# arielmission-space/PAOS

Measured on AMD Instinct MI355X. Metric: wavefronts/sec (4096^2 c128, 20-surface chain) + achieved HBM GB/s, higher is better.
Workload: dtype c128 (f64); 1 GPU; SYN20 20-surface chain (SURVEY 8d: 43 2-D FFTs per wavefront as the reference runs it), 4096x4096 fp64, walked 512-wavelength sweep, 32 wavefronts/GPU/step, PSFs stay in HBM; separable pass programs + ptp identities ([24] passes/wavefront, parity 1e-15..2e-14 vs oracle); grid=4096, batch_per_gpu=32, parallelism=wavefront-sharded x1, transport=none (single process), ranks_seen=1, launcher=none

## Files before the change

### include/paos_hip.h

```cpp
#ifndef PAOS_HIP_H
#define PAOS_HIP_H

#ifdef __cplusplus
extern "C" {
#endif

typedef struct paos_ctx paos_ctx;

enum { PAOS_OK = 0, PAOS_EINVAL = 1, PAOS_EHIP = 2, PAOS_EUNSUPPORTED = 3 };
enum { PAOS_F64 = 0, PAOS_F32 = 1 };
enum { PAOS_SHAPE_ELLIPSE = 0, PAOS_SHAPE_RECT = 1 };
enum { PAOS_KERNEL_PASS_ROWS = 0, PAOS_KERNEL_PASS_COLS = 1, PAOS_KERNEL_PASS_ANY = 2 };
enum { PAOS_PW_SIGN = 1, PAOS_PW_QPHASE_CENTRED = 2, PAOS_PW_QPHASE_NATURAL = 3, PAOS_PW_SCALE = 4,
       PAOS_PW_MASK = 5 };
enum { PAOS_PWF_MUL2PI = 1,
       PAOS_PWF_X_ONLY = 2, PAOS_PWF_Y_ONLY = 4 };
enum { PAOS_MAX_PW = 6 };
enum { PAOS_NORM_SLOTS = 64 };
enum { PAOS_WHAT_FIELD = 0, PAOS_WHAT_AMPLITUDE = 1, PAOS_WHAT_PHASE = 2, PAOS_WHAT_INTENSITY = 3 };

enum { PAOS_PHASE_STRIDE = 5 };
enum { PAOS_APERTURE_STRIDE = 8 };
enum { PAOS_ZERNIKE_HEAD = 8 };

typedef struct { int kind, flags, block; } paos_pw_op;
typedef struct {
  int axis;
  int fft1, fft2;
  int n_pre, n_mid, n_post;
  paos_pw_op pre[PAOS_MAX_PW], mid[PAOS_MAX_PW], post[PAOS_MAX_PW];
} paos_pass;

typedef struct {
  const double* live_rows;
  int rows_stale;
  int final_intensity;
  int* power_ticket;
  const double* live_cols;
} paos_program_opts;

int paos_ctx_create(int device, int n, int batch, int precision, paos_ctx** out);
int paos_ctx_destroy(paos_ctx* ctx);
const char* paos_last_error(const paos_ctx* ctx);
int paos_sync(paos_ctx* ctx);
const char* paos_build_info(void);
const char* paos_source_hash(void);
void* paos_stream(paos_ctx* ctx);

int paos_profile_begin(paos_ctx* ctx, int kernel_kind, int max_launches);
int paos_profile_end(paos_ctx* ctx, int* launches, double* total_ms);
int paos_profile_end_split(paos_ctx* ctx, int* launches, double* total_ms, int* pruned_launches, double* pruned_ms);
int paos_profile_end_launches(paos_ctx* ctx, int capacity, double* ms_out, int* tag_out, int* count);
int paos_profile_planned_bytes(paos_ctx* ctx, int capacity, double* bytes_out, int* count);
int paos_profile_line_transforms(paos_ctx* ctx, int capacity, double* lines_out, int* count);

int paos_fill(paos_ctx* ctx, double re, double im);
int paos_start(paos_ctx* ctx, double re, double im, int shape, const double* aperture, const double* stop);
int paos_start_rows(paos_ctx* ctx, double re, double im, int shape, const double* aperture, const double* stop,
                    const double* write_rows);
int paos_zero_outside_rows(paos_ctx* ctx, const double* live_rows);
int paos_start_box(paos_ctx* ctx, double re, double im, int shape, const double* aperture, const double* stop,
                   const double* write_rows, const double* write_cols);
int paos_start_zernike_box(paos_ctx* ctx, double re, double im, int shape, const double* aperture, const double* stop,
                           const double* write_rows, const double* write_cols, int nmax, int kdim, const double* table,
                           const double* params, int param_stride, int* power_ticket);
int paos_zero_outside_box(paos_ctx* ctx, const double* live_rows, const double* live_cols);
int paos_import(paos_ctx* ctx, int item, const void* host_c128);
int paos_export(paos_ctx* ctx, int item, int what, void* host_out);

int paos_psf_keep(paos_ctx* ctx);
int paos_psf_keep_power(paos_ctx* ctx, int* ticket);
int paos_psf_fetch(paos_ctx* ctx, int item, double* host_out);
int paos_host_alloc(unsigned long long bytes, void** out);
int paos_host_free(void* p);
int paos_export_pinned(paos_ctx* ctx, int item, int what, void* pinned_out);

int paos_aperture(paos_ctx* ctx, int shape, const double* params);
int paos_aperture_render(paos_ctx* ctx, int shape, const double* params1, double* host_mask);
int paos_make_stop(paos_ctx* ctx, const double* enable);
int paos_stop_scale_last_power(paos_ctx* ctx, const double* enable);
int paos_stop_defer_last_power(paos_ctx* ctx, const double* enable);
int paos_norm2(paos_ctx* ctx, double* host_out);
int paos_norm2_enqueue(paos_ctx* ctx, int* ticket);
int paos_norm2_enqueue_rows(paos_ctx* ctx, const double* live_rows, int* ticket);
int paos_norm2_enqueue_rows_like(paos_ctx* ctx, const double* live_rows, const double* same_as, int* ticket);
int paos_norm2_enqueue_box(paos_ctx* ctx, const double* live_rows, const double* live_cols, const double* same_as, int* ticket);
int paos_norm2_fetch(paos_ctx* ctx, int ticket, double* host_out);
int paos_norm2_release(paos_ctx* ctx, int ticket);
int paos_psf_metrics(paos_ctx* ctx, int nr, const double* radii_px, double cx_px, double cy_px,
                     double* host_out);
int paos_phase(paos_ctx* ctx, const double* params, int mul2pi);
int paos_phase_map(paos_ctx* ctx, int item, const double* host_wfe, double wl);
int paos_phase_map_items(paos_ctx* ctx, const double* host_wfe, unsigned long long key, int n_items, const double* items,
                         const double* wl);
int paos_psd_screen(paos_ctx* ctx, const double* host_noise, const double* host_rough, const double* params,
                    unsigned long long key, double* host_out);
int paos_ptp(paos_ctx* ctx, const double* params);
int paos_stw(paos_ctx* ctx, const double* params, int inverse);
int paos_wts(paos_ctx* ctx, const double* params, int inverse);
int paos_focus_begin(paos_ctx* ctx);
int paos_focus_plane(paos_ctx* ctx, const double* params);
int paos_focus_end(paos_ctx* ctx);
enum { PAOS_OTF_MTF = 0, PAOS_OTF_COMPLEX = 1 };
int paos_otf_compute(paos_ctx* ctx);
int paos_otf_fetch(paos_ctx* ctx, int item, int what, void* host_out);
int paos_otf_cuts(paos_ctx* ctx, double* host_out);
int paos_blur_table(int n, double d, double sigma, double pixel, double* t);
enum { PAOS_BLUR_ITEM = 6 };
int paos_blur_apply(paos_ctx* ctx, const double* per_item);
enum { PAOS_EE_GIVEN = 0, PAOS_EE_CENTROID = 1, PAOS_EE_PEAK = 2 };
enum { PAOS_EE_ITEM = 4 };
enum { PAOS_EE_SUMMARY = 9 };
int paos_ee_compute(paos_ctx* ctx, int bins, int square, int centre_mode, const double* per_item);
int paos_ee_fetch(paos_ctx* ctx, double* summary, double* curves);
int paos_zoom_weights(int n, int s, double frac, double* w, int* carry);
enum { PAOS_ZOOM_PSF = 0, PAOS_ZOOM_FIELD = 1 };
int paos_zoom_compute(paos_ctx* ctx, int m, int s, const double* centres, int want_field);
int paos_zoom_tiles(int n, int batch, int m, int* pt_y, int* pt_x);
int paos_zoom_fetch(paos_ctx* ctx, int item, int what, void* host_out);
int paos_run_passes(paos_ctx* ctx, const paos_pass* passes, int n_passes, const double* blocks,
                    int n_blocks);
int paos_copy_yardstick(paos_ctx* ctx, int reps, double* ms_per_launch, double* bytes_per_launch);
int paos_record_set_stats(paos_ctx* ctx, unsigned long long* found, unsigned long long* rendered);
int paos_central_half_stats(paos_ctx* ctx, unsigned long long* central, unsigned long long* plain);
int paos_narrow_window_stats(paos_ctx* ctx, unsigned long long* narrow, unsigned long long* other);
int paos_record_block_stats(paos_ctx* ctx, unsigned long long* out);
int paos_frugal_built(int precision, int n, const int* record);
int paos_pass_builds(paos_ctx* ctx, int* records, int capacity, int* count);
int paos_deferred_stop_stats(paos_ctx* ctx, unsigned long long* rode, unsigned long long* settled);
int paos_ctx_set_pruning(paos_ctx* ctx, int on);
int paos_run_passes_live(paos_ctx* ctx, const paos_pass* passes, int n_passes, const double* blocks,
                         int n_blocks, const double* live_rows);
int paos_run_program(paos_ctx* ctx, const paos_pass* passes, int n_passes, const double* blocks, int n_blocks,
                     const paos_program_opts* opts);
int paos_zernike(paos_ctx* ctx, int nmax, int kdim, const double* table, const double* params,
                 int param_stride, double* host_wfe);
int paos_zernike_like(paos_ctx* ctx, int nmax, int kdim, const double* table, const double* params,
                      int param_stride, const double* same_as, double* host_wfe);


int paos_pupil_aperture(paos_ctx* ctx, int shape, const double* params);
int paos_pupil_upload(paos_ctx* ctx, int item, const double* host_weights);
int paos_zernike_gram(paos_ctx* ctx, int nmax, int kdim, const double* table, const double* params,
                      int param_stride, int K, const double* poly, int use_pupil, double* host_out);
int paos_zernike_pupil(paos_ctx* ctx, int nmax, int kdim, const double* table, const double* params,
                       int param_stride, double* host_wfe);

enum { PAOS_WF_UNIFORM = 0, PAOS_WF_INTENSITY = 1 };
enum { PAOS_WF_SUMMARY = 10 };
int paos_wavefront_fit(paos_ctx* ctx, int nmax, int kdim, const double* table, const double* params, int param_stride,
                       int K, const double* poly, int weight_mode, int use_pupil, const double* min_intensity);
int paos_wavefront_fetch(paos_ctx* ctx, double* summary, double* sums);

enum { PAOS_DETECTOR_GEOM = 6 };
enum { PAOS_DETECTOR_ITEM = 3 };
enum { PAOS_DETECTOR_SCRATCH_MIB = 512 };
int paos_detector_begin(paos_ctx* ctx, const double* geom);
int paos_detector_add(paos_ctx* ctx, const double* per_item);
int paos_detector_images(paos_ctx* ctx, const double* per_item, double* host_out);
int paos_detector_fetch(paos_ctx* ctx, double* host_out);
enum { PAOS_DETECTOR_PLACED_ITEM = 5 };
int paos_detector_add_placed(paos_ctx* ctx, const double* per_item);
int paos_detector_images_placed(paos_ctx* ctx, const double* per_item, double* host_out);

enum { PAOS_SERIES_ITEM = 4 };
enum { PAOS_SERIES_MAX_FRAMES = 65536, PAOS_SERIES_MAX_BOXES = 16 };
int paos_series_compute(paos_ctx* ctx, const double* geom, const double* per_item, const double* offsets, int frames,
                        int per_item_offsets, const int* boxes, int nboxes, const double* response, double* host_frames);
int paos_series_fetch(paos_ctx* ctx, double* flux);

#ifdef __cplusplus
}
#endif
#endif
```

### paos_amd/_lib.py

```python
import ctypes
import os
import threading
import weakref

import numpy as np

_HERE = os.path.dirname(os.path.abspath(__file__))
LIB_PATH = os.environ.get("PAOS_LIB") or os.path.join(_HERE, "libpaoship.so")

PAOS_F64, PAOS_F32 = 0, 1
SHAPE_ELLIPSE, SHAPE_RECT = 0, 1
WHAT_FIELD, WHAT_AMPLITUDE, WHAT_PHASE, WHAT_INTENSITY = 0, 1, 2, 3
KERNEL_PASS_ROWS, KERNEL_PASS_COLS, KERNEL_PASS_ANY = 0, 1, 2
PW_SIGN, PW_QPHASE_CENTRED, PW_QPHASE_NATURAL, PW_SCALE, PW_MASK = 1, 2, 3, 4, 5
PWF_MUL2PI = 1
PWF_X_ONLY, PWF_Y_ONLY = 2, 4
MAX_PW = 6
OTF_MTF, OTF_COMPLEX = 0, 1
EE_GIVEN, EE_CENTROID, EE_PEAK = 0, 1, 2
EE_ITEM, EE_SUMMARY, EE_MAX_BINS = 4, 9, 1024
SERIES_ITEM, SERIES_MAX_FRAMES, SERIES_MAX_BOXES = 4, 65536, 16
WF_UNIFORM, WF_INTENSITY = 0, 1
WF_SUMMARY, WF_MAX_TERMS = 10, 63
ZOOM_PSF, ZOOM_FIELD = 0, 1
ZOOM_MAX_TABLES = 256
NORM_SLOTS = 64


class PwOp(ctypes.Structure):
    _fields_ = [("kind", ctypes.c_int), ("flags", ctypes.c_int), ("block", ctypes.c_int)]


class ProgramOpts(ctypes.Structure):
    _fields_ = [("live_rows", ctypes.POINTER(ctypes.c_double)), ("rows_stale", ctypes.c_int),
                ("final_intensity", ctypes.c_int), ("power_ticket", ctypes.POINTER(ctypes.c_int)),
                ("live_cols", ctypes.POINTER(ctypes.c_double))]


class Pass(ctypes.Structure):
    _fields_ = [("axis", ctypes.c_int), ("fft1", ctypes.c_int), ("fft2", ctypes.c_int),
                ("n_pre", ctypes.c_int), ("n_mid", ctypes.c_int), ("n_post", ctypes.c_int),
                ("pre", PwOp * MAX_PW), ("mid", PwOp * MAX_PW), ("post", PwOp * MAX_PW)]

PHASE_STRIDE = 5
APERTURE_STRIDE = 8
ZERNIKE_HEAD = 8

_c_ctx = ctypes.c_void_p
_dbl_p = ctypes.POINTER(ctypes.c_double)
SYMBOLS = {
    "paos_ctx_create": (ctypes.c_int, [ctypes.c_int, ctypes.c_int, ctypes.c_int, ctypes.c_int, ctypes.POINTER(_c_ctx)]),
    "paos_ctx_destroy": (ctypes.c_int, [_c_ctx]),
    "paos_last_error": (ctypes.c_char_p, [_c_ctx]),
    "paos_sync": (ctypes.c_int, [_c_ctx]),
    "paos_build_info": (ctypes.c_char_p, []),
    "paos_stream": (ctypes.c_void_p, [_c_ctx]),
    "paos_profile_begin": (ctypes.c_int, [_c_ctx, ctypes.c_int, ctypes.c_int]),
    "paos_profile_end": (ctypes.c_int, [_c_ctx, ctypes.POINTER(ctypes.c_int), _dbl_p]),
    "paos_profile_end_split": (ctypes.c_int, [_c_ctx, ctypes.POINTER(ctypes.c_int), _dbl_p, ctypes.POINTER(ctypes.c_int), _dbl_p]),
    "paos_source_hash": (ctypes.c_char_p, []),
    "paos_profile_planned_bytes": (ctypes.c_int, [_c_ctx, ctypes.c_int, _dbl_p, ctypes.POINTER(ctypes.c_int)]),
    "paos_profile_line_transforms": (ctypes.c_int, [_c_ctx, ctypes.c_int, _dbl_p, ctypes.POINTER(ctypes.c_int)]),
    "paos_profile_end_launches": (ctypes.c_int, [_c_ctx, ctypes.c_int, _dbl_p, ctypes.POINTER(ctypes.c_int),
                                                 ctypes.POINTER(ctypes.c_int)]),
    "paos_fill": (ctypes.c_int, [_c_ctx, ctypes.c_double, ctypes.c_double]),
    "paos_import": (ctypes.c_int, [_c_ctx, ctypes.c_int, ctypes.c_void_p]),
    "paos_export": (ctypes.c_int, [_c_ctx, ctypes.c_int, ctypes.c_int, ctypes.c_void_p]),
    "paos_aperture": (ctypes.c_int, [_c_ctx, ctypes.c_int, _dbl_p]),
    "paos_aperture_render": (ctypes.c_int, [_c_ctx, ctypes.c_int, _dbl_p, _dbl_p]),
    "paos_make_stop": (ctypes.c_int, [_c_ctx, _dbl_p]),
    "paos_stop_scale_last_power": (ctypes.c_int, [_c_ctx, _dbl_p]),
    "paos_stop_defer_last_power": (ctypes.c_int, [_c_ctx, _dbl_p]),
    "paos_norm2": (ctypes.c_int, [_c_ctx, _dbl_p]),
    "paos_norm2_enqueue": (ctypes.c_int, [_c_ctx, ctypes.POINTER(ctypes.c_int)]),
    "paos_norm2_fetch": (ctypes.c_int, [_c_ctx, ctypes.c_int, _dbl_p]),
    "paos_norm2_release": (ctypes.c_int, [_c_ctx, ctypes.c_int]),
    "paos_psf_metrics": (ctypes.c_int, [_c_ctx, ctypes.c_int, _dbl_p, ctypes.c_double, ctypes.c_double, _dbl_p]),
    "paos_phase": (ctypes.c_int, [_c_ctx, _dbl_p, ctypes.c_int]),
    "paos_phase_map": (ctypes.c_int, [_c_ctx, ctypes.c_int, _dbl_p, ctypes.c_double]),
    "paos_ptp": (ctypes.c_int, [_c_ctx, _dbl_p]),
    "paos_stw": (ctypes.c_int, [_c_ctx, _dbl_p, ctypes.c_int]),
    "paos_wts": (ctypes.c_int, [_c_ctx, _dbl_p, ctypes.c_int]),
    "paos_focus_begin": (ctypes.c_int, [_c_ctx]),
    "paos_focus_plane": (ctypes.c_int, [_c_ctx, _dbl_p]),
    "paos_focus_end": (ctypes.c_int, [_c_ctx]),
    "paos_otf_compute": (ctypes.c_int, [_c_ctx]),
    "paos_otf_fetch": (ctypes.c_int, [_c_ctx, ctypes.c_int, ctypes.c_int, ctypes.c_void_p]),
    "paos_otf_cuts": (ctypes.c_int, [_c_ctx, _dbl_p]),
    "paos_blur_table": (ctypes.c_int, [ctypes.c_int, ctypes.c_double, ctypes.c_double, ctypes.c_double, _dbl_p]),
    "paos_blur_apply": (ctypes.c_int, [_c_ctx, _dbl_p]),
    "paos_ee_compute": (ctypes.c_int, [_c_ctx, ctypes.c_int, ctypes.c_int, ctypes.c_int, _dbl_p]),
    "paos_ee_fetch": (ctypes.c_int, [_c_ctx, _dbl_p, _dbl_p]),
    "paos_series_compute": (ctypes.c_int, [_c_ctx, _dbl_p, _dbl_p, _dbl_p, ctypes.c_int, ctypes.c_int, ctypes.POINTER(ctypes.c_int),
                                           ctypes.c_int, _dbl_p, _dbl_p]),
    "paos_series_fetch": (ctypes.c_int, [_c_ctx, _dbl_p]),
    "paos_wavefront_fit": (ctypes.c_int, [_c_ctx, ctypes.c_int, ctypes.c_int, _dbl_p, _dbl_p, ctypes.c_int, ctypes.c_int, _dbl_p,
                                          ctypes.c_int, ctypes.c_int, _dbl_p]),
    "paos_wavefront_fetch": (ctypes.c_int, [_c_ctx, _dbl_p, _dbl_p]),
    "paos_zoom_weights": (ctypes.c_int, [ctypes.c_int, ctypes.c_int, ctypes.c_double, _dbl_p, ctypes.POINTER(ctypes.c_int)]),
    "paos_zoom_compute": (ctypes.c_int, [_c_ctx, ctypes.c_int, ctypes.c_int, _dbl_p, ctypes.c_int]),
    "paos_zoom_fetch": (ctypes.c_int, [_c_ctx, ctypes.c_int, ctypes.c_int, ctypes.c_void_p]),
    "paos_zoom_tiles": (ctypes.c_int, [ctypes.c_int, ctypes.c_int, ctypes.c_int, ctypes.POINTER(ctypes.c_int),
                                       ctypes.POINTER(ctypes.c_int)]),
    "paos_run_passes": (ctypes.c_int, [_c_ctx, ctypes.POINTER(Pass), ctypes.c_int, _dbl_p, ctypes.c_int]),
    "paos_copy_yardstick": (ctypes.c_int, [_c_ctx, ctypes.c_int, _dbl_p, _dbl_p]),
    "paos_record_set_stats": (ctypes.c_int, [_c_ctx, ctypes.POINTER(ctypes.c_ulonglong), ctypes.POINTER(ctypes.c_ulonglong)]),
    "paos_central_half_stats": (ctypes.c_int, [_c_ctx, ctypes.POINTER(ctypes.c_ulonglong), ctypes.POINTER(ctypes.c_ulonglong)]),
    "paos_narrow_window_stats": (ctypes.c_int, [_c_ctx, ctypes.POINTER(ctypes.c_ulonglong), ctypes.POINTER(ctypes.c_ulonglong)]),
    "paos_record_block_stats": (ctypes.c_int, [_c_ctx, ctypes.POINTER(ctypes.c_ulonglong)]),
    "paos_frugal_built": (ctypes.c_int, [ctypes.c_int, ctypes.c_int, ctypes.POINTER(ctypes.c_int)]),
    "paos_pass_builds": (ctypes.c_int, [_c_ctx, ctypes.POINTER(ctypes.c_int), ctypes.c_int, ctypes.POINTER(ctypes.c_int)]),
    "paos_deferred_stop_stats": (ctypes.c_int, [_c_ctx, ctypes.POINTER(ctypes.c_ulonglong), ctypes.POINTER(ctypes.c_ulonglong)]),
    "paos_ctx_set_pruning": (ctypes.c_int, [_c_ctx, ctypes.c_int]),
    "paos_run_passes_live": (ctypes.c_int, [_c_ctx, ctypes.POINTER(Pass), ctypes.c_int, _dbl_p, ctypes.c_int, _dbl_p]),
    "paos_zernike": (ctypes.c_int, [_c_ctx, ctypes.c_int, ctypes.c_int, _dbl_p, _dbl_p, ctypes.c_int, _dbl_p]),
    "paos_psf_keep": (ctypes.c_int, [_c_ctx]),
    "paos_psf_keep_power": (ctypes.c_int, [_c_ctx, ctypes.POINTER(ctypes.c_int)]),
    "paos_psf_fetch": (ctypes.c_int, [_c_ctx, ctypes.c_int, _dbl_p]),
    "paos_host_alloc": (ctypes.c_int, [ctypes.c_ulonglong, ctypes.POINTER(ctypes.c_void_p)]),
    "paos_host_free": (ctypes.c_int, [ctypes.c_void_p]),
    "paos_export_pinned": (ctypes.c_int, [_c_ctx, ctypes.c_int, ctypes.c_int, ctypes.c_void_p]),
    "paos_start": (ctypes.c_int, [_c_ctx, ctypes.c_double, ctypes.c_double, ctypes.c_int, _dbl_p, _dbl_p]),
    "paos_pupil_aperture": (ctypes.c_int, [_c_ctx, ctypes.c_int, _dbl_p]),
    "paos_pupil_upload": (ctypes.c_int, [_c_ctx, ctypes.c_int, _dbl_p]),
    "paos_zernike_like": (ctypes.c_int, [_c_ctx, ctypes.c_int, ctypes.c_int, _dbl_p, _dbl_p, ctypes.c_int, _dbl_p, _dbl_p]),
    "paos_zernike_gram": (ctypes.c_int, [_c_ctx, ctypes.c_int, ctypes.c_int, _dbl_p, _dbl_p, ctypes.c_int,
                                         ctypes.c_int, _dbl_p, ctypes.c_int, _dbl_p]),
    "paos_zernike_pupil": (ctypes.c_int, [_c_ctx, ctypes.c_int, ctypes.c_int, _dbl_p, _dbl_p, ctypes.c_int, _dbl_p]),
    "paos_start_rows": (ctypes.c_int, [_c_ctx, ctypes.c_double, ctypes.c_double, ctypes.c_int, _dbl_p, _dbl_p, _dbl_p]),
    "paos_zero_outside_rows": (ctypes.c_int, [_c_ctx, _dbl_p]),
    "paos_phase_map_items": (ctypes.c_int, [_c_ctx, _dbl_p, ctypes.c_ulonglong, ctypes.c_int, _dbl_p, _dbl_p]),
    "paos_psd_screen": (ctypes.c_int, [_c_ctx, _dbl_p, _dbl_p, _dbl_p, ctypes.c_ulonglong, _dbl_p]),
    "paos_start_box": (ctypes.c_int, [_c_ctx, ctypes.c_double, ctypes.c_double, ctypes.c_int, _dbl_p, _dbl_p, _dbl_p, _dbl_p]),
    "paos_start_zernike_box": (ctypes.c_int, [_c_ctx, ctypes.c_double, ctypes.c_double, ctypes.c_int, _dbl_p, _dbl_p, _dbl_p, _dbl_p,
                                              ctypes.c_int, ctypes.c_int, _dbl_p, _dbl_p, ctypes.c_int, ctypes.POINTER(ctypes.c_int)]),
    "paos_zero_outside_box": (ctypes.c_int, [_c_ctx, _dbl_p, _dbl_p]),
    "paos_norm2_enqueue_box": (ctypes.c_int, [_c_ctx, _dbl_p, _dbl_p, _dbl_p, ctypes.POINTER(ctypes.c_int)]),
    "paos_norm2_enqueue_rows": (ctypes.c_int, [_c_ctx, _dbl_p, ctypes.POINTER(ctypes.c_int)]),
    "paos_norm2_enqueue_rows_like": (ctypes.c_int, [_c_ctx, _dbl_p, _dbl_p, ctypes.POINTER(ctypes.c_int)]),
    "paos_run_program": (ctypes.c_int, [_c_ctx, ctypes.POINTER(Pass), ctypes.c_int, _dbl_p, ctypes.c_int,
                                        ctypes.POINTER(ProgramOpts)]),
    "paos_detector_begin": (ctypes.c_int, [_c_ctx, _dbl_p]),
    "paos_detector_add": (ctypes.c_int, [_c_ctx, _dbl_p]),
    "paos_detector_images": (ctypes.c_int, [_c_ctx, _dbl_p, _dbl_p]),
    "paos_detector_fetch": (ctypes.c_int, [_c_ctx, _dbl_p]),
    "paos_detector_add_placed": (ctypes.c_int, [_c_ctx, _dbl_p]),
    "paos_detector_images_placed": (ctypes.c_int, [_c_ctx, _dbl_p, _dbl_p]),
}

_lib = None


class PaosHipError(RuntimeError):
    pass


def load():
    global _lib
    if _lib is not None:
        return _lib
    if not os.path.exists(LIB_PATH):
        raise PaosHipError(
            f"{LIB_PATH} not found: build it with `make` or "
            "`python -c 'import __graft_entry__ as g; g.build()'` (there is no CPU fallback)"
        )
    lib = ctypes.CDLL(LIB_PATH)
    if os.environ.get("PAOS_LIB"):
        import sys

        print(f"paos_amd: using the library variant {LIB_PATH} (PAOS_LIB)", file=sys.stderr)
    for name, (res, args) in SYMBOLS.items():
        fn = getattr(lib, name)
        fn.restype = res
        fn.argtypes = args
    _lib = lib
    return lib


def _dptr(arr):
    return arr.ctypes.data_as(_dbl_p)


def as_blocks(blocks, batch, stride):
    arr = np.ascontiguousarray(blocks, dtype=np.float64)
    if arr.shape != (batch, stride):
        raise ValueError(f"expected parameter blocks of shape {(batch, stride)}, got {arr.shape}")
    return arr


BUILD_FIELDS = ("axis", "kpre", "kmid", "nfft", "store", "tab", "fuse", "one_line", "central")


def frugal_built(precision, n, record):
    if len(record) != len(BUILD_FIELDS):
        raise ValueError("a build record has nine fields")
    rec = (ctypes.c_int * 9)(*[int(v) for v in record])
    code = {"fp64": PAOS_F64, "fp32": PAOS_F32}.get(precision, -1)
    rc = load().paos_frugal_built(code, int(n), rec)
    if rc < 0:
        raise ValueError(f"no family of pass-kernel builds for {precision} at n = {n}")
    return bool(rc)


def zoom_check(size, oversample, n):
    if isinstance(size, bool) or not isinstance(size, (int, np.integer)) or size < 16 or size > 1024 or size % 16:
        raise ValueError(f"a zoomed window's size must be an integer multiple of 16 in 16 .. 1024, got {size!r}")
    if isinstance(oversample, bool) or not isinstance(oversample, (int, np.integer)) or not 1 <= oversample <= 64:
        raise ValueError(f"a zoomed window's oversampling must be an integer in 1 .. 64, got {oversample!r}")
    if size > oversample * n:
        raise ValueError(f"a zoomed window of {size} samples at oversampling {oversample} is wider than the {n}-pixel grid")


def zoom_tiles(n, batch, size):
    pty, ptx = ctypes.c_int(0), ctypes.c_int(0)
    if load().paos_zoom_tiles(int(n), int(batch), int(size), ctypes.byref(pty), ctypes.byref(ptx)) != 0:
        raise ValueError(f"paos_zoom_tiles refused n={n!r}, batch={batch!r}, size={size!r}")
    return pty.value, ptx.value


def blur_table(n, d, sigma, pixel=0.0):
    if isinstance(n, bool) or not isinstance(n, (int, np.integer)) or n < 2:
        raise ValueError(f"paos_blur_table refused n={n!r}")
    out = np.empty(int(n) // 2 + 1, dtype=np.float64)
    if load().paos_blur_table(int(n), float(d), float(sigma), float(pixel), _dptr(out)) != 0:
        raise ValueError(f"paos_blur_table refused n={n!r}, d={d!r}, sigma={sigma!r}, pixel={pixel!r}")
    return out


def zoom_centres(centres, batch, n):
    try:
        ctr = np.ascontiguousarray(centres, dtype=np.float64)
    except (TypeError, ValueError):
        raise ValueError("zoomed-window centres must be a (batch, 2) array of pixel positions (x, y)") from None
    if ctr.shape != (batch, 2):
        raise ValueError(f"zoomed-window centres must have shape ({batch}, 2), got {ctr.shape}")
    if not np.all(np.isfinite(ctr)) or np.any(ctr < 0.0) or np.any(ctr >= n):
        raise ValueError(f"zoomed-window centres must be finite and lie in [0, {n})")
    if np.unique(ctr - np.floor(ctr)).size > ZOOM_MAX_TABLES:
        raise ValueError(f"the centres of one call may have at most {ZOOM_MAX_TABLES} distinct fractional parts")
    return ctr


PINNED_MIN_BYTES = 4 << 20
PINNED_MAX_BYTES = 32 << 20
PINNED_LIVE_BYTES = int(os.environ.get("PAOS_PINNED_BYTES", 8 << 30))
PINNED_POOL_BYTES = 2 << 30
_pin_lock = threading.Lock()
_pin_free = {}
_pin_live = 0
_pin_pooled = 0


def _pin_release(address, nbytes):
    global _pin_live, _pin_pooled
    with _pin_lock:
        _pin_live -= nbytes
        if _pin_pooled + nbytes <= PINNED_POOL_BYTES:
            _pin_free.setdefault(nbytes, []).append(address)
            _pin_pooled += nbytes
            return
    try:
# ... 645 lines not shown
```

### paos_amd/csrc/context.hip

```cpp
#include "host.h"

#include <cmath>
#include <complex>
#include <cstdio>
#include <cstring>
#include <mutex>
#include <set>
#include <utility>

namespace {

thread_local std::string g_err;

}

int fail(paos_ctx* c, int code, const std::string& msg) {
  if (c) c->err = msg;
  g_err = msg;
  return code;
}

namespace {

bool dump_arena() {
// ... 128 lines not shown
    }
  }
  HIPCHK(c, hipStreamSynchronize(c->stream));
  return PAOS_OK;
}

bool timed_launch_begin(paos_ctx* c, int kind) {
  const bool timed = (c->prof_kind == kind || c->prof_kind == PAOS_KERNEL_PASS_ANY) && (c->prof_used + 2 <= c->prof_events.size());
  return timed && hipEventRecord(c->prof_events[c->prof_used], c->stream) == hipSuccess;
}
hipError_t timed_launch_end(paos_ctx* c, int tag) {
  const hipError_t e = hipEventRecord(c->prof_events[c->prof_used + 1], c->stream);
  if (e != hipSuccess) return e;
  c->prof_tags.resize(c->prof_used / 2, 0);
  c->prof_tags.push_back(tag);
  c->prof_bytes.resize(c->prof_tags.size() - 1, 0.0);
  c->prof_bytes.push_back(c->prof_next_bytes);
  c->prof_lines.resize(c->prof_tags.size() - 1, 0.0);
  c->prof_lines.push_back(c->prof_next_lines);
  c->prof_used += 2;
  return hipSuccess;
}

int next_norm_slot(paos_ctx* c) {
  for (int k = 0; k < kNormSlots; ++k) {
    const int slot = (c->norm_slot + k) % kNormSlots;
    if (!c->norm_busy[slot]) { c->norm_slot = slot; return slot; }
  }
  return c->norm_slot;
}

int opt_in_lds(paos_ctx* c, const void* kern, size_t lds) {
  static std::mutex mu;
  static std::set<std::pair<int, const void*>> configured;
  std::lock_guard<std::mutex> lock(mu);
  const std::pair<int, const void*> key(c->device, kern);
  if (configured.count(key)) return PAOS_OK;
  HIPCHK(c, hipFuncSetAttribute(kern, hipFuncAttributeMaxDynamicSharedMemorySize, (int)lds));
  configured.insert(key);
  return PAOS_OK;
}

int check_mask_overflow(paos_ctx* c) {
  if (!c->mask_overflow) return PAOS_OK;
  int n = 0;
  HIPCHK(c, hipMemcpy(&n, c->mask_overflow, sizeof(int), hipMemcpyDeviceToHost));
  if (n != 0) {
    (void)hipMemset(c->mask_overflow, 0, sizeof(int));
    for (auto& ms : c->mask_sets) ms.key.clear();
    return fail(c, PAOS_EUNSUPPORTED, "aperture line records overflowed (partial run longer than kMaskW): results are invalid");
  }
  return PAOS_OK;
}

int check_rows(paos_ctx* c, const double* rows) {
  for (int i = 0; i < c->batch; ++i)
    if (!(rows[2 * i] >= 0.0) || !(rows[2 * i + 1] <= (double)c->n) || !(rows[2 * i] <= rows[2 * i + 1]))
      return fail(c, PAOS_EINVAL, "row range must satisfy 0 <= lo <= hi <= n");
  return PAOS_OK;
}

std::vector<double> rounded_cols(const paos_ctx* c, const double* cols) {
  std::vector<double> out((size_t)2 * c->batch);
  for (int i = 0; i < c->batch; ++i) {
    int l = (int)cols[2 * i], h = (int)cols[2 * i + 1];
    l = l < 0 ? 0 : (l / c->br) * c->br;
    h = ((h + c->br - 1) / c->br) * c->br;
    if (h > c->n) h = c->n;
    out[2 * i] = l; out[2 * i + 1] = h;
  }
  return out;
}

namespace {

template <typename T>
std::vector<std::complex<T>> twiddles(int n) {
  std::vector<std::complex<T>> tw(n);
  const long double two_pi = 6.283185307179586476925286766559005768L;
  for (int m = 0; m < n; ++m) {
    const long double a = two_pi * (long double)m / (long double)n;
    tw[m] = std::complex<T>((T)cosl(a), (T)-sinl(a));
  }
  return tw;
}


int profile_end(paos_ctx* c, int* launches, double* total_ms, int* pruned_launches, double* pruned_ms) {
  if (c) (void)hipSetDevice(c->device);
  if (!c || !launches || !total_ms) return fail(c, PAOS_EINVAL, "null argument");
  HIPCHK(c, hipStreamSynchronize(c->stream));
  double sum = 0.0, psum = 0.0;
  int pcount = 0;
  for (size_t i = 0; i + 1 < c->prof_used; i += 2) {
    float ms = 0.f;
    HIPCHK(c, hipEventElapsedTime(&ms, c->prof_events[i], c->prof_events[i + 1]));
    sum += ms;
    if (i / 2 < c->prof_tags.size() && c->prof_tags[i / 2]) { psum += ms; ++pcount; }
  }
  *launches = (int)(c->prof_used / 2);
  *total_ms = sum;
  if (pruned_launches) *pruned_launches = pcount;
  if (pruned_ms) *pruned_ms = psum;
  c->prof_kind = -1;
  c->prof_used = 0;
  return PAOS_OK;
}

}

extern "C" {

const char* paos_last_error(const paos_ctx* ctx) { return ctx ? ctx->err.c_str() : g_err.c_str(); }

const char* paos_build_info(void) {
  static const std::string info = std::string("libpaoship gfx950 layout=") + std::to_string(BR) + "(c64 at N>=2048: " + std::to_string(PAOS_F32_BR) + ")x(" +
                                  std::to_string(Lay<double>::BC) + "|" + std::to_string(Lay<float>::BC) +
                                  ") pad_blocks=" + std::to_string(PAOS_PAD_BLOCKS);
  return info.c_str();
}

void* paos_stream(paos_ctx* ctx) { return ctx ? (void*)ctx->stream : nullptr; }

int paos_ctx_create(int device, int n, int batch, int precision, paos_ctx** out) {
  if (!out) return fail(nullptr, PAOS_EINVAL, "out is null");
  *out = nullptr;
  if (n < 64 || n > 4096 || (n & (n - 1))) return fail(nullptr, PAOS_EUNSUPPORTED, "grid size must be a power of two in 64..4096");
  if (batch < 1) return fail(nullptr, PAOS_EINVAL, "batch must be >= 1");
  if (precision != PAOS_F64 && precision != PAOS_F32) return fail(nullptr, PAOS_EINVAL, "precision must be PAOS_F64 or PAOS_F32");
  int ndev = 0;
  if (hipGetDeviceCount(&ndev) != hipSuccess || ndev == 0)
    return fail(nullptr, PAOS_EHIP, "no HIP device available: libpaoship has no CPU fallback");
  if (device < 0 || device >= ndev) return fail(nullptr, PAOS_EINVAL, "device index out of range");
  paos_ctx* c = new paos_ctx();
  c->device = device; c->n = n; c->batch = batch; c->precision = precision;
  const int bc = precision == PAOS_F64 ? Lay<double>::BC : Lay<float>::BC;
  c->br = (precision == PAOS_F32 && n >= 2048) ? PAOS_F32_BR : PAOS_BR;
  c->pitch = (unsigned)n * c->br + (unsigned)PAOS_PAD_BLOCKS * c->br * bc;
  c->item_stride = c->pitch * (unsigned)(n / c->br);
  const size_t eb = elem_bytes(c);
  auto bail = [&](hipError_t e, const char* what) {
    std::string msg = std::string(what) + ": " + hipGetErrorString(e);
    paos_ctx_destroy(c);
    return fail(nullptr, PAOS_EHIP, msg);
  };
  hipError_t e;
  if ((e = hipSetDevice(device)) != hipSuccess) return bail(e, "hipSetDevice");
  if ((e = hipStreamCreateWithFlags(&c->stream, hipStreamNonBlocking)) != hipSuccess) return bail(e, "hipStreamCreate");
  if (const char* pad = getenv("PAOS_LDS_PAD")) c->lds_pad = (size_t)std::max(0, std::atoi(pad));
  if (env_is("PAOS_CENTRAL_HALF", '0')) c->central_half = false;
  if (env_is("PAOS_CENTRAL_HALF", '1')) c->central_half = true;
  if (env_is("PAOS_NARROW_WINDOWS", '0')) c->narrow_windows = false;
  if (env_is("PAOS_NARROW_WINDOWS", '1')) c->narrow_windows = true;
  if ((e = hipMalloc(&c->dyn_scale, (size_t)batch * sizeof(double))) != hipSuccess) return bail(e, "hipMalloc(dyn_scale)");
  {
    std::vector<double> ones((size_t)batch, 1.0);
    if ((e = hipMemcpy(c->dyn_scale, ones.data(), ones.size() * sizeof(double), hipMemcpyHostToDevice)) != hipSuccess) return bail(e, "hipMemcpy(dyn_scale)");
  }
  if ((e = hipMalloc(&c->field, (size_t)c->item_stride * batch * eb)) != hipSuccess) return bail(e, "hipMalloc(field)");
  if ((e = hipMemsetAsync(c->field, 0, (size_t)c->item_stride * batch * eb, c->stream)) != hipSuccess) return bail(e, "hipMemset(field)");
  if ((e = hipMalloc(&c->tw, (size_t)n * eb)) != hipSuccess) return bail(e, "hipMalloc(tw)");
  if ((e = hipMalloc(&c->staging, (size_t)n * n * 16)) != hipSuccess) return bail(e, "hipMalloc(staging)");
  c->nparts = 1024;
  if ((e = hipMalloc(&c->partial, (size_t)batch * c->nparts * sizeof(double))) != hipSuccess) return bail(e, "hipMalloc(partial)");
  if ((e = hipMalloc(&c->norm2, (size_t)batch * sizeof(double))) != hipSuccess) return bail(e, "hipMalloc(norm2)");
  if ((e = hipHostMalloc(&c->norm2_host, (size_t)kNormSlots * batch * sizeof(double))) != hipSuccess) return bail(e, "hipHostMalloc(norm2)");
  c->arena.lay.cap = (size_t)1 << 18;
  if (c->arena.lay.cap < (size_t)batch * 2048) c->arena.lay.cap = (size_t)batch * 2048;
  if (const char* cap = getenv("PAOS_ARENA_DOUBLES")) c->arena.lay.cap = arena_rounded((size_t)std::max(1LL, std::atoll(cap)));
  if ((e = hipHostMalloc(&c->arena.host, kArenaSlabs * c->arena.lay.cap * sizeof(double))) != hipSuccess) return bail(e, "hipHostMalloc(arena)");
  if ((e = hipMalloc(&c->arena.dev, kArenaSlabs * c->arena.lay.cap * sizeof(double))) != hipSuccess) return bail(e, "hipMalloc(arena)");
  for (int k = 0; k < kArenaSlabs; ++k)
    if ((e = hipEventCreateWithFlags(&c->arena.fence[k], hipEventDisableTiming)) != hipSuccess) return bail(e, "hipEventCreate(arena fence)");
  c->arena.used[0] = true;
  e = dispatch_layout(c, [&](auto t, auto) {
    auto tw = twiddles<decltype(t)>(n);
    return hipMemcpy(c->tw, tw.data(), (size_t)n * eb, hipMemcpyHostToDevice);
  });
  if (e != hipSuccess) return bail(e, "hipMemcpy(tw)");
  *out = c;
  return PAOS_OK;
}

int paos_profile_begin(paos_ctx* c, int kernel_kind, int max_launches) {
  if (c) (void)hipSetDevice(c->device);
  if (!c || max_launches < 0) return fail(c, PAOS_EINVAL, "bad profile request");
  HIPCHK(c, hipStreamSynchronize(c->stream));
  while (c->prof_events.size() < (size_t)2 * max_launches) {
    hipEvent_t e;
    HIPCHK(c, hipEventCreate(&e));
    c->prof_events.push_back(e);
  }
  c->prof_kind = kernel_kind;
  c->prof_used = 0;
  c->prof_tags.clear();
  c->prof_bytes.clear();
  c->prof_lines.clear();
  return PAOS_OK;
}

int paos_profile_end_launches(paos_ctx* c, int capacity, double* ms_out, int* tag_out, int* count) {
  if (c) (void)hipSetDevice(c->device);
  if (!c || !ms_out || !tag_out || !count || capacity < 0) return fail(c, PAOS_EINVAL, "null argument");
  HIPCHK(c, hipStreamSynchronize(c->stream));
  const int n = (int)(c->prof_used / 2);
  if (n > capacity) return fail(c, PAOS_EINVAL, "more launches were timed than the caller's arrays hold");
  for (int i = 0; i < n; ++i) {
    float ms = 0.f;
    HIPCHK(c, hipEventElapsedTime(&ms, c->prof_events[2 * i], c->prof_events[2 * i + 1]));
    ms_out[i] = ms;
    tag_out[i] = (size_t)i < c->prof_tags.size() ? c->prof_tags[i] : 0;
  }
  *count = n;
  c->prof_kind = -1;
  c->prof_used = 0;
  return PAOS_OK;
}

int paos_profile_planned_bytes(paos_ctx* c, int capacity, double* bytes_out, int* count) {
  if (!c || !bytes_out || !count || capacity < 0) return fail(c, PAOS_EINVAL, "null argument");
  const int n = (int)(c->prof_used / 2);
  if (n > capacity) return fail(c, PAOS_EINVAL, "more launches were timed than the caller's array holds");
  for (int i = 0; i < n; ++i) bytes_out[i] = (size_t)i < c->prof_bytes.size() ? c->prof_bytes[i] : 0.0;
  *count = n;
  return PAOS_OK;
}

int paos_profile_line_transforms(paos_ctx* c, int capacity, double* lines_out, int* count) {
  if (!c || !lines_out || !count || capacity < 0) return fail(c, PAOS_EINVAL, "bad profile request");
  const int n = (int)(c->prof_used / 2);
  if (n > capacity) return fail(c, PAOS_EINVAL, "profile buffer too small");
  for (int i = 0; i < n; ++i) lines_out[i] = (size_t)i < c->prof_lines.size() ? c->prof_lines[i] : 0.0;
  *count = n;
  return PAOS_OK;
}

int paos_profile_end(paos_ctx* c, int* launches, double* total_ms) {
  return profile_end(c, launches, total_ms, nullptr, nullptr);
}

int paos_profile_end_split(paos_ctx* c, int* launches, double* total_ms, int* pruned_launches, double* pruned_ms) {
  if (!pruned_launches || !pruned_ms) return fail(c, PAOS_EINVAL, "null argument");
  return profile_end(c, launches, total_ms, pruned_launches, pruned_ms);
}

int paos_ctx_destroy(paos_ctx* c) {
  if (!c) return PAOS_OK;
  (void)hipSetDevice(c->device);
  if (c->stream) (void)hipStreamSynchronize(c->stream);
  for (hipEvent_t e : c->prof_events) (void)hipEventDestroy(e);
  if (c->field) (void)hipFree(c->field);
  if (c->tw) (void)hipFree(c->tw);
  if (c->staging) (void)hipFree(c->staging);
  if (c->tables) (void)hipFree(c->tables);
  if (c->mask) (void)hipFree(c->mask);
  if (c->metric_partial) (void)hipFree(c->metric_partial);
  if (c->metric_out) (void)hipFree(c->metric_out);
  if (c->metric_host) (void)hipHostFree(c->metric_host);
  for (auto& ms : c->mask_sets) {
    if (ms.lines) (void)hipFree(ms.lines);
    if (ms.vals) (void)hipFree(ms.vals);
  }
  if (c->mask_overflow) (void)hipFree(c->mask_overflow);
  if (c->block_stats) (void)hipFree(c->block_stats);
  if (c->partial) (void)hipFree(c->partial);
  if (c->norm2) (void)hipFree(c->norm2);
  if (c->norm2_host) (void)hipHostFree(c->norm2_host);
  if (c->psf) (void)hipFree(c->psf);
  if (c->focus_spec) (void)hipFree(c->focus_spec);
  if (c->otf_spec) (void)hipFree(c->otf_spec);
  if (c->otf_cuts) (void)hipFree(c->otf_cuts);
  if (c->zoom_t) (void)hipFree(c->zoom_t);
  if (c->zoom_psf) (void)hipFree(c->zoom_psf);
  if (c->zoom_field) (void)hipFree(c->zoom_field);
  if (c->zoom_tabs) (void)hipFree(c->zoom_tabs);
  if (c->map_dev) (void)hipFree(c->map_dev);
  if (c->psd_scratch) (void)hipFree(c->psd_scratch);
  if (c->start_norm2) (void)hipFree(c->start_norm2);
  if (c->start_partial) (void)hipFree(c->start_partial);
  if (c->psd_bad) (void)hipFree(c->psd_bad);
  if (c->pow_partial) (void)hipFree(c->pow_partial);
  if (c->dyn_scale) (void)hipFree(c->dyn_scale);
  if (c->ptab) (void)hipFree(c->ptab);
  if (c->psf_partial) (void)hipFree(c->psf_partial);
  if (c->det_img) (void)hipFree(c->det_img);
  if (c->det_rows) (void)hipFree(c->det_rows);
  if (c->det_out) (void)hipFree(c->det_out);
  if (c->ee_buf) (void)hipFree(c->ee_buf);
  if (c->wf_buf) (void)hipFree(c->wf_buf);
  if (c->series_par) (void)hipFree(c->series_par);
  if (c->series_flux) (void)hipFree(c->series_flux);
  if (c->series_frames) (void)hipFree(c->series_frames);
  if (c->series_host) (void)hipHostFree(c->series_host);
  if (c->series_ev) (void)hipEventDestroy(c->series_ev);
  for (int i = 0; i < 2; ++i) {
    if (c->bounce[i]) (void)hipHostFree(c->bounce[i]);
    if (c->bounce_ev[i]) (void)hipEventDestroy(c->bounce_ev[i]);
  }
  if (c->arena.host) (void)hipHostFree(c->arena.host);
  if (c->arena.dev) (void)hipFree(c->arena.dev);
  for (int k = 0; k < kArenaSlabs; ++k)
    if (c->arena.fence[k]) (void)hipEventDestroy(c->arena.fence[k]);
  if (c->stream) (void)hipStreamDestroy(c->stream);
  delete c;
  return PAOS_OK;
}

int paos_sync(paos_ctx* c) {
  if (c) (void)hipSetDevice(c->device);
  if (!c) return fail(c, PAOS_EINVAL, "null context");
  HIPCHK(c, hipStreamSynchronize(c->stream));
  return check_mask_overflow(c);
}

int paos_host_alloc(unsigned long long bytes, void** out) {
  if (!out || bytes == 0) return fail(nullptr, PAOS_EINVAL, "null argument");
  *out = nullptr;
  const hipError_t e = hipHostMalloc(out, (size_t)bytes);
  if (e != hipSuccess) {
    *out = nullptr;
    return fail(nullptr, PAOS_EHIP, std::string("hipHostMalloc: ") + hipGetErrorString(e));
  }
  return PAOS_OK;
}

int paos_host_free(void* p) {
  if (!p) return PAOS_OK;
  const hipError_t e = hipHostFree(p);
  if (e != hipSuccess) return fail(nullptr, PAOS_EHIP, std::string("hipHostFree: ") + hipGetErrorString(e));
  return PAOS_OK;
}

int paos_norm2_fetch(paos_ctx* c, int ticket, double* host_out) {
  if (c) (void)hipSetDevice(c->device);
  if (!c || !host_out || ticket < 0 || ticket >= kNormSlots) return fail(c, PAOS_EINVAL, "bad ticket");
  if (!c->norm_busy[ticket]) return fail(c, PAOS_EINVAL, "ticket is not outstanding (already fetched, or never issued)");
  HIPCHK(c, hipStreamSynchronize(c->stream));
  c->norm_busy[ticket] = false;
  std::memcpy(host_out, c->norm2_host + (size_t)ticket * c->batch, (size_t)c->batch * sizeof(double));
  return check_mask_overflow(c);
}

int paos_norm2_release(paos_ctx* c, int ticket) {
  if (!c || ticket < 0 || ticket >= kNormSlots) return fail(c, PAOS_EINVAL, "bad ticket");
  c->norm_busy[ticket] = false;
  return PAOS_OK;
}

int paos_record_set_stats(paos_ctx* c, unsigned long long* found, unsigned long long* rendered) {
  if (!c || !found || !rendered) return fail(c, PAOS_EINVAL, "bad record-set request");
  *found = c->mask_hits;
  *rendered = c->mask_rendered;
  return PAOS_OK;
}

int paos_central_half_stats(paos_ctx* c, unsigned long long* central, unsigned long long* plain) {
  if (!c || !central || !plain) return fail(c, PAOS_EINVAL, "bad central-half request");
  *central = c->central_launches;
  *plain = c->plain_launches;
  return PAOS_OK;
}

int paos_narrow_window_stats(paos_ctx* c, unsigned long long* narrow, unsigned long long* other) {
  if (!c || !narrow || !other) return fail(c, PAOS_EINVAL, "bad narrow-window request");
  *narrow = c->narrow_launches;
  *other = c->other_launches;
  return PAOS_OK;
}

int paos_record_block_stats(paos_ctx* c, unsigned long long* out) {
  if (!c || !out) return fail(c, PAOS_EINVAL, "bad record-block request");
  out[0] = out[1] = out[2] = 0ull;
  if (!c->block_stats) return PAOS_OK;
  HIPCHK(c, hipStreamSynchronize(c->stream));
  HIPCHK(c, hipMemcpy(out, c->block_stats, 3 * sizeof(unsigned long long), hipMemcpyDeviceToHost));
  return PAOS_OK;
}

int paos_deferred_stop_stats(paos_ctx* c, unsigned long long* rode, unsigned long long* settled) {
  if (!c || !rode || !settled) return fail(c, PAOS_EINVAL, "bad deferred-stop request");
  *rode = c->deferred_rode;
  *settled = c->deferred_settled;
  return PAOS_OK;
}

int paos_ctx_set_pruning(paos_ctx* c, int on) {
  if (!c) return fail(c, PAOS_EINVAL, "null context");
  c->prune = on != 0;
  return PAOS_OK;
}

}
```

### paos_amd/csrc/focus_otf.hip

```cpp
#include "host.h"

#include <algorithm>
#include <cmath>

#include "blur_pass.h"
#include "focus_pass.h"
#include "otf_pass.h"

namespace {

template <typename T_, int N_, int AXIS_>
struct Tile {
  using T = T_;
  using C = FftCfg<T, N_>;
  static constexpr int N = N_, AXIS = AXIS_;
  static constexpr int LINES = AXIS == 0 ? C::ROW_LINES : C::COL_LINES;
  static constexpr int TILES = AXIS == 0 ? C::ROW_TILES : C::COL_TILES;
  static constexpr bool SPLIT = AXIS == 0 ? C::ROW_SPLIT : C::COL_SPLIT;
  static constexpr int PER_WG = LINES * TILES;
};
template <typename Kernel, typename Args>
int tile_pass(paos_ctx* c, int axis, int lines, double bytes, Kernel kernel, const Args& a) {
  return dispatch_layout(c, [&](auto t, auto) {
    return dispatch_n(c, [&](auto n) {
// ... 23 lines not shown
    using L = decltype(tile);
    using C = typename L::C;
    return focus_pass_kernel<typename L::T, L::N, C::E, L::LINES, L::TILES, L::AXIS, C::BR, C::BC, L::SPLIT, C::MINW>;
  }, a);
}

}

extern "C" {

int paos_focus_begin(paos_ctx* c) {
  SETTLE_SCALE(c);
  if (c) (void)hipSetDevice(c->device);
  if (!c) return fail(c, PAOS_EINVAL, "null context");
  if (c->focus_open) return fail(c, PAOS_EINVAL, "paos_focus_begin: a focus stack is already open (paos_focus_end first)");
  if (!c->focus_spec) HIPCHK(c, hipMalloc(&c->focus_spec, (size_t)c->item_stride * c->batch * elem_bytes(c)));
  int rc = focus_pass(c, 0, FOCUS_FORWARD, c->field, c->focus_spec, nullptr);
  if (rc) return rc;
  rc = focus_pass(c, 1, FOCUS_FORWARD, c->focus_spec, c->focus_spec, nullptr);
  if (rc) return rc;
  c->focus_open = true;
  return PAOS_OK;
}

int paos_focus_plane(paos_ctx* c, const double* params) {
  if (c) (void)hipSetDevice(c->device);
  if (!c || !params) return fail(c, PAOS_EINVAL, "null argument");
  if (!c->focus_open) return fail(c, PAOS_EINVAL, "paos_focus_plane: no focus stack is open (paos_focus_begin first)");
  for (int i = 0; i < c->batch; ++i)
    for (int k = 0; k < FP_STRIDE; ++k)
      if (!std::isfinite(params[(size_t)i * FP_STRIDE + k]))
        return fail(c, PAOS_EINVAL, "paos_focus_plane: non-finite parameter of item " + std::to_string(i));
  DROP_SCALE(c);
  const double* dparams = nullptr;
  int rc = arena_push(c, params, (size_t)c->batch * FP_STRIDE, &dparams);
  if (rc) return rc;
  rc = focus_pass(c, 1, FOCUS_TRANSFER, c->focus_spec, c->field, dparams);
  if (rc) return rc;
  return focus_pass(c, 0, FOCUS_INVERSE, c->field, c->field, nullptr);
}

int paos_focus_end(paos_ctx* c) {
  if (c) (void)hipSetDevice(c->device);
  if (!c) return fail(c, PAOS_EINVAL, "null context");
  if (!c->focus_open) return fail(c, PAOS_EINVAL, "paos_focus_end: no focus stack is open");
  HIPCHK(c, hipStreamSynchronize(c->stream));
  HIPCHK(c, hipFree(c->focus_spec));
  c->focus_spec = nullptr;
  c->focus_open = false;
  return PAOS_OK;
}

}

namespace {

constexpr int kThreads = 256;

int otf_pass(paos_ctx* c, int axis) {
  OtfArgs a{};
  a.psf = c->psf; a.spec = c->otf_spec; a.tw = c->tw;
  a.pitch = c->pitch; a.item_stride = c->item_stride;
  const double n = c->n, eb = (double)elem_bytes(c);
  const double bytes = axis == 0 ? c->batch * n * (n * 8.0 + c->n / 2 * eb) : c->batch * (double)(c->n / 2 + 1) * 2.0 * n * eb;
  return tile_pass(c, axis, packed_lines(c, axis), bytes, [](auto tile) {
    using L = decltype(tile);
    using C = typename L::C;
    if constexpr (L::AXIS == 0) return otf_row_kernel<typename L::T, L::N, C::E, L::LINES, L::TILES, C::BR, C::BC, L::SPLIT, C::MINW>;
    else return otf_col_kernel<typename L::T, L::N, C::E, L::LINES, L::TILES, C::BR, C::BC, L::SPLIT, C::MINW>;
  }, a);
}

int otf_ready(paos_ctx* c, const char* who) {
  if (!c->otf_spec || !c->otf_computed) return fail(c, PAOS_EINVAL, std::string(who) + ": no transfer functions computed (paos_otf_compute)");
  if (!c->otf_valid)
    return fail(c, PAOS_EINVAL, std::string(who) + ": the PSFs were stored anew since paos_otf_compute: the transfer functions are stale (compute again)");
  return PAOS_OK;
}

int blur_pass(paos_ctx* c, int axis, const BlurArgs& a) {
  const double n = c->n, eb = (double)elem_bytes(c);
  const double bytes = axis == 0 ? c->batch * n * n * 16.0 : c->batch * n * ((c->n / 2 + 1) * 2.0 * eb + n * 8.0);
  return tile_pass(c, axis, packed_lines(c, axis), bytes, [](auto tile) {
    using L = decltype(tile);
    using C = typename L::C;
    if constexpr (L::AXIS == 0) return blur_row_kernel<typename L::T, L::N, C::E, L::LINES, L::TILES, C::BR, C::BC, L::SPLIT, C::MINW>;
    else return blur_col_kernel<typename L::T, L::N, C::E, L::LINES, L::TILES, C::BR, C::BC, L::SPLIT, C::MINW>;
  }, a);
}

const char* blur_table_refusal(int n, double d, double sigma, double pixel) {
  if (n < 2 || (n & 1) || n > (1 << 20)) return "n must be even, 2 .. 2^20";
  if (!std::isfinite(d) || !(d > 0.0)) return "the pitch must be finite and positive";
  if (!std::isfinite(sigma) || sigma < 0.0) return "sigma must be finite and >= 0";
  if (!std::isfinite(pixel) || pixel < 0.0) return "the pixel width must be finite and >= 0";
  return nullptr;
}

}

extern "C" {

int paos_blur_table(int n, double d, double sigma, double pixel, double* t) {
  if (const char* why = blur_table_refusal(n, d, sigma, pixel)) return fail(nullptr, PAOS_EINVAL, std::string("paos_blur_table: ") + why);
  if (!t) return fail(nullptr, PAOS_EINVAL, "paos_blur_table: null argument");
  const long double pi = 3.141592653589793238462643383279502884L;
  const long double s = (long double)sigma, p = (long double)pixel, nd = (long double)n * (long double)d;
  for (int m = 0; m <= n / 2; ++m) {
    const long double f = (long double)m / nd;
    const long double x = pi * (p * f);
    const long double sinc = x == 0.0L ? 1.0L : sinl(x) / x;
    t[m] = (double)(expl(-2.0L * pi * pi * (s * s) * (f * f)) * sinc);
  }
  return PAOS_OK;
}

int paos_blur_apply(paos_ctx* c, const double* per_item) {
  if (c) (void)hipSetDevice(c->device);
  if (!c || !per_item) return fail(c, PAOS_EINVAL, "paos_blur_apply: null argument");
  int rc = otf_ready(c, "paos_blur_apply");
  if (rc) return rc;
  for (int i = 0; i < c->batch; ++i) {
    const double* q = per_item + (size_t)i * PAOS_BLUR_ITEM;
    for (int ax = 0; ax < 2; ++ax)
      if (const char* why = blur_table_refusal(c->n, q[ax], q[2 + ax], q[4 + ax]))
        return fail(c, PAOS_EINVAL, "paos_blur_apply: item " + std::to_string(i) + (ax ? ", y: " : ", x: ") + why);
  }
  const int len = c->n / 2 + 1;
  std::vector<double>& tabs = c->blur_tabs;
  if (tabs.empty()) {
    tabs.resize((size_t)c->batch * 2 * len);
    c->blur_key.assign((size_t)c->batch * 2 * 3, -1.0);
  }
  for (int i = 0; i < c->batch; ++i) {
    const double* q = per_item + (size_t)i * PAOS_BLUR_ITEM;
    for (int ax = 0; ax < 2; ++ax) {
      double* key = c->blur_key.data() + ((size_t)i * 2 + ax) * 3;
      if (key[0] == q[ax] && key[1] == q[2 + ax] && key[2] == q[4 + ax]) continue;
      key[0] = -1.0;
      rc = paos_blur_table(c->n, q[ax], q[2 + ax], q[4 + ax], tabs.data() + ((size_t)i * 2 + ax) * len);
      if (rc) return rc;
      key[0] = q[ax]; key[1] = q[2 + ax]; key[2] = q[4 + ax];
    }
  }
  rc = arena_reserve(c, tabs.size());
  if (rc) return rc;
  const double* dtabs = nullptr;
  rc = arena_push(c, tabs.data(), tabs.size(), &dtabs);
  if (rc) return rc;
  BlurArgs a{};
  a.psf = c->psf; a.spec = c->otf_spec; a.tw = c->tw; a.tabs = dtabs;
  a.scale = 1.0 / ((double)c->n * (double)c->n);
  a.pitch = c->pitch; a.item_stride = c->item_stride;
  c->psf_zero_axis = -1;
  c->ee_valid = false;
  for (int axis = 1; axis >= 0; --axis) {
    rc = blur_pass(c, axis, a);
    if (rc) {
      c->otf_valid = false;
      return rc;
    }
  }
  return PAOS_OK;
}

int paos_otf_compute(paos_ctx* c) {
  if (c) (void)hipSetDevice(c->device);
  if (!c) return fail(c, PAOS_EINVAL, "null context");
  if (!c->psf) return fail(c, PAOS_EINVAL, "paos_otf_compute: no PSF kept (paos_psf_keep)");
  if (!c->otf_spec) HIPCHK(c, hipMalloc(&c->otf_spec, (size_t)c->item_stride * c->batch * elem_bytes(c)));
  c->otf_valid = false;
  int rc = otf_pass(c, 0);
  if (rc) return rc;
  rc = otf_pass(c, 1);
  if (rc) return rc;
  c->otf_computed = c->otf_valid = true;
  return PAOS_OK;
}

int paos_otf_fetch(paos_ctx* c, int item, int what, void* host_out) {
  if (c) (void)hipSetDevice(c->device);
  if (!c || !host_out || item < 0 || item >= c->batch || (what != PAOS_OTF_MTF && what != PAOS_OTF_COMPLEX))
    return fail(c, PAOS_EINVAL, "paos_otf_fetch: bad item/what or null buffer");
  int rc = otf_ready(c, "paos_otf_fetch");
  if (rc) return rc;
  const int cplx = what == PAOS_OTF_COMPLEX;
  const size_t n2 = (size_t)c->n * c->n;
  const dim3 grid((unsigned)std::min<size_t>((n2 + kThreads - 1) / kThreads, 2048)), block(kThreads);
  dispatch_layout(c, [&](auto t, auto br) {
    using T = decltype(t);
    hipLaunchKernelGGL((otf_fetch_kernel<T, decltype(br)::value, Lay<T>::BC>), grid, block, 0, c->stream,
                       (const cx<T>*)c->otf_spec + (size_t)item * c->item_stride, c->staging, c->n, c->pitch, cplx);
  });
  HIPCHK(c, hipGetLastError());
  return copy_to_host(c, host_out, c->staging, n2 * (cplx ? 16 : 8));
}

int paos_otf_cuts(paos_ctx* c, double* host_out) {
  if (c) (void)hipSetDevice(c->device);
  if (!c || !host_out) return fail(c, PAOS_EINVAL, "paos_otf_cuts: null argument");
  int rc = otf_ready(c, "paos_otf_cuts");
  if (rc) return rc;
  const int len = c->n / 2 + 1;
  const size_t bytes = (size_t)c->batch * 2 * len * sizeof(double);
  if (!c->otf_cuts) HIPCHK(c, hipMalloc(&c->otf_cuts, bytes));
  const dim3 grid((2 * len + kThreads - 1) / kThreads, c->batch), block(kThreads);
  dispatch_layout(c, [&](auto t, auto br) {
    using T = decltype(t);
    hipLaunchKernelGGL((otf_cuts_kernel<T, decltype(br)::value, Lay<T>::BC>), grid, block, 0, c->stream, (const cx<T>*)c->otf_spec,
                       c->otf_cuts, c->n, c->pitch, c->item_stride);
  });
  HIPCHK(c, hipGetLastError());
  return copy_to_host(c, host_out, c->otf_cuts, bytes);
}

}
```

### paos_amd/csrc/frugal_launch.h

```cpp
#pragma once
#include "host.h"
#include "pass_records.h"


inline int frugal_not_built(paos_ctx* c, const FrugalBuild& b) {
  if (b.tab && b.fuse) {
    if (b.kpre != 1 || b.kmid != 1) return fail(c, PAOS_EINVAL, "no fused build of this pass shape");
    if (b.nfft < 2) return fail(c, PAOS_EINVAL, "a fused chain starts with a two-transform pass");
    if (b.fuse > 4) return fail(c, PAOS_EINVAL, "a launch runs at most three passes");
  }
  if (b.tab && !(b.kpre <= 1 && b.kmid <= 1 && b.kpre + b.kmid > 0)) return fail(c, PAOS_EINVAL, "no table build of this pass shape");
  if (b.store == 1 && !b.tab) return fail(c, PAOS_EUNSUPPORTED, "no PSF-storing build of this pass shape");
  if (b.store == 2 && !b.tab) return fail(c, PAOS_EUNSUPPORTED, "no power-summing build of this pass shape");
  return fail(c, PAOS_EINVAL, "no build of this pass shape");
}

template <typename T, int N, int AXIS, int KPRE, int KMID, int STORE = 0, int LONG = 0, int ONE = 0, int LINES_ = 0, int TILES_ = 0>
struct FrugalGeometry {
  using C = FftCfg<T, N>;
  static constexpr bool kLatencyBound = PAOS_LONG_ONE_LINE != 0 && (LONG != 0 || ONE != 0) && STORE == 0 && sizeof(T) == 8;
  static constexpr bool kOneLine = kLatencyBound && N == 4096;
  static constexpr int OCC = (kLatencyBound && N == 2048) ? 1 : 0;
  static constexpr int LINES = LINES_ != 0 ? LINES_ : (kOneLine ? 1 : (AXIS == 0 ? C::FR_ROW_LINES : C::COL_LINES));
  static constexpr int TILES = TILES_ != 0 ? TILES_ : (AXIS == 0 ? C::ROW_TILES : C::COL_TILES);
  static constexpr bool SPLIT = sizeof(T) == 8 || LINES > 2;
  static constexpr int GROUPS = N / LINES / TILES, THREADS = TILES * LINES * N / C::E;
  static constexpr size_t LDS = frugal_lds_bytes<T, N, LINES, TILES, SPLIT, KPRE, KMID, C::E, STORE, OCC>();
  static constexpr unsigned ALIGN = (LINES == 1 && AXIS == 0) ? 32 : 16;
};

namespace {

template <typename T, int N, int AXIS, int KPRE, int KMID, int NFFT, int STORE, int TAB, int LONG, int ONE, int CH>
int frugal_launch(paos_ctx* c, const FrugalArgs& args, bool narrow) {
  using C = FftCfg<T, N>;
  using G = FrugalGeometry<T, N, AXIS, KPRE, KMID, STORE, LONG, ONE>;
  FrugalArgs a = args;
  unsigned groups = G::GROUPS;
  a.wg0 = 0;
  static_assert(G::GROUPS % G::ALIGN == 0, "TileMap renumbers tiles inside aligned groups of workgroups");
  if (a.live_hi > a.live_lo) {
    const unsigned per = G::LINES * G::TILES;
    a.wg0 = (a.live_lo / per) / G::ALIGN * G::ALIGN;
    unsigned end = ((a.live_hi + per - 1) / per + G::ALIGN - 1) / G::ALIGN * G::ALIGN;
    if (end > groups) end = groups;
    groups = end - a.wg0;
  }
  const dim3 grid(groups, c->batch), block(G::THREADS);
  constexpr size_t kMaxPad = 8192;
  const size_t lds = G::LDS + (c->lds_pad < kMaxPad ? c->lds_pad : kMaxPad);
  auto kern = frugal_pass_kernel<T, N, C::E, G::LINES, G::TILES, AXIS, C::BR, C::BC, G::SPLIT, KPRE, KMID, NFFT, STORE, TAB, LONG, G::OCC, CH>;
  if constexpr (CH == 1) {
    if (narrow) kern = frugal_pass_kernel<T, N, C::E, G::LINES, G::TILES, AXIS, C::BR, C::BC, G::SPLIT, KPRE, KMID, NFFT, STORE, TAB, LONG, G::OCC, 2>;
  } else {
    narrow = false;
  }
  ++(CH != 0 ? c->central_launches : c->plain_launches);
  ++(narrow ? c->narrow_launches : c->other_launches);
  return TIMED_LAUNCH(c, kern, grid, block, lds, G::LDS + kMaxPad, AXIS == 0 ? PAOS_KERNEL_PASS_ROWS : PAOS_KERNEL_PASS_COLS,
                      c->prof_next_tag, PAOS_FRUGAL_PASS(a));
}

constexpr int kFrugalFieldMax[] = {1, kFrugalMaxPre, kFrugalMaxMid, 2, 2, 1, 4, 1, 1};
template <typename T, int N, int X, int... V>
int frugal_unfold(paos_ctx* c, const FrugalBuild& b, const FrugalArgs& a, bool narrow) {
  constexpr int I = sizeof...(V), kFields = sizeof(kFrugalFieldMax) / sizeof(int);
  static_assert(kFields == kBuildFields, "one maximum per field");
  int field[kBuildFields];
  build_to_ints(b, field);
  if (field[I] != X) {
    if constexpr (X < kFrugalFieldMax[I]) return frugal_unfold<T, N, X + 1, V...>(c, b, a, narrow);
    else return frugal_not_built(c, b);
  } else if constexpr (I + 1 < kFields) {
    return frugal_unfold<T, N, 0, V..., X>(c, b, a, narrow);
  } else if constexpr (frugal_built<T, N>(FrugalBuild{V..., X})) {
    return frugal_launch<T, N, V..., X>(c, a, narrow);
  } else {
    return frugal_not_built(c, b);
  }
}
template <typename T, int N>
int frugal_dispatch(paos_ctx* c, const FrugalBuild& b, const FrugalArgs& a, bool narrow = false) {
  return frugal_unfold<T, N, 0>(c, b, a, narrow);
}

}
```

### paos_amd/csrc/frugal_pass.h

```cpp
#pragma once
#include "fft_kernels.h"
#include "pass_records.h"

#ifndef PAOS_FENCE_EVERY
#define PAOS_FENCE_EVERY 2
#endif

namespace paos {


template <int N, int E>
constexpr int twiddle_lds_entries() { return E <= 16 ? 256 : (N / 4 < 1024 ? N / 4 : 1024); }

#ifndef PAOS_STAMPS
#define PAOS_STAMPS 0
#endif
constexpr int kStampSlots = 12;

struct FrugalArgs {
  void* field;
  const void* tw;
  const FrugalItem* items;
  unsigned pitch, item_stride;
  double* psf;
// ... 332 lines not shown
}

struct PhaseTableArgs {
  const FrugalItem* items;
  const cx<double>* tw;
  const PhaseSlotDesc* desc;
  int n;
  int f32;
};
template <int UNIT = 0>
__global__ void __launch_bounds__(256) phase_table_kernel(PhaseTableArgs a) {
  __shared__ cx<double> circle[kCircleLds];
  if (!a.f32) {
    const cx<double> w = a.tw[threadIdx.x * (a.n / kCircleLds)];
    circle[threadIdx.x] = {w.x, -w.y};
  }
  __syncthreads();
  const PhaseSlotDesc d = a.desc[blockIdx.z];
  const FrugalItem& it = a.items[d.item_base + blockIdx.y];
  const bool mid = d.mid != 0;
  const FrugalSlot& sl = mid ? it.mid : it.pre;
  if (it.active == 0.0 || sl.table == nullptr) return;
  const FrugalPhase* ph = mid ? it.mid_ph : it.pre_ph;
  const int K = d.k;
  const int qflip = (mid && it.fft1_on != 0.0 && it.fft1_inv != 0.0) ? (int)0x80000000 : 0;
  const int pos = blockIdx.x * blockDim.x + threadIdx.x;
  double g[kFrugalMaxMid], step[kFrugalMaxMid], across2[kFrugalMaxMid], coefq[kFrugalMaxMid], m2[kFrugalMaxMid];
#pragma unroll
  for (int j = 0; j < kFrugalMaxMid; ++j) {
    const FrugalPhase& q = ph[j < K ? j : 0];
    g[j] = (double)(q.natural != 0.0 ? (pos < a.n / 2 ? pos : pos - a.n) : pos - a.n / 2);
    step[j] = d.axis == 0 ? q.sx : q.sy;
    across2[j] = 0.0;
    coefq[j] = __hiloint2double(__double2hiint(q.coef) ^ qflip, __double2loint(q.coef));
    m2[j] = q.m2;
  }
  if (a.f32) {
    cx<float> pf = {1.0f, 0.0f};
    if (K <= 0) {}
    else if (K == 1) pf = slot_factor32<1>(g, step, across2, coefq, m2);
    else if (K == 2) pf = slot_factor32<2>(g, step, across2, coefq, m2);
    else pf = slot_factor32<3>(g, step, across2, coefq, m2);
    reinterpret_cast<cx<float>*>(const_cast<cx<double>*>(sl.table))[pos] = pf;
    return;
  }
  cx<double> p = {1.0, 0.0};
  if (K <= 0) {}
  else if (K == 1) p = slot_factor<1>(g, step, across2, coefq, m2, circle);
  else if (K == 2) p = slot_factor<2>(g, step, across2, coefq, m2, circle);
  else p = slot_factor<3>(g, step, across2, coefq, m2, circle);
  const_cast<cx<double>*>(sl.table)[pos] = p;
}

template <bool NT, typename T>
__device__ __forceinline__ cx<T> stream_load(const cx<T>* p) {
  typedef T vec2 __attribute__((ext_vector_type(2)));
  if constexpr (NT) {
    const vec2 t = __builtin_nontemporal_load(reinterpret_cast<const vec2*>(p));
    return {t.x, t.y};
  } else {
    return *p;
  }
}
template <bool NT, typename T>
__device__ __forceinline__ void stream_store(cx<T>* p, cx<T> v) {
  typedef T vec2 __attribute__((ext_vector_type(2)));
  if constexpr (NT) __builtin_nontemporal_store(vec2{v.x, v.y}, reinterpret_cast<vec2*>(p));
  else *p = v;
}

template <int E, typename T>
__device__ __forceinline__ void pin_tile(cx<T>* v) {
#pragma unroll
  for (int k = 0; k < E; ++k) asm volatile("" : "+v"(v[k].x), "+v"(v[k].y));
}

template <typename T, int N, int E, bool SPLIT, bool FLIP = true, int CH = 0>
__device__ __forceinline__ void frugal_fft(cx<T>* v, void* lds, int t, const cx<T>* tw, const cx<double>* circle,
                                           double inv, const cx<T>* w1_last = nullptr) {
  fft_stages<T, N, E, +1, SPLIT, 1, 1, CH>(v, lds, t, tw, circle, w1_last);
  unpermute_slots<N, E>(v);
  if constexpr (FLIP) {
    const unsigned mask = inv != 0.0 ? 0x80000000u : 0u;
#pragma unroll
    for (int k = 0; k < E; ++k) v[k].y = flip_sign(v[k].y, mask);
  }
  __builtin_amdgcn_sched_barrier(0);
}

constexpr size_t kStoreScratch = 16 * sizeof(double);
template <int LINES, int TILES, int KPRE>
constexpr int frugal_record_mode() {
  return (TILES * LINES == 2 && KPRE == 0) ? 2 : (TILES * LINES <= 16 ? 1 : 0);
}
template <typename T, int N, int E, int LINES, int TILES, int OCC = 0>
constexpr bool frugal_tw_in_regs() {
  return sizeof(T) == 8 && E == 16 && ((N == 4096 && TILES * LINES == 1) || (N == 2048 && OCC != 0 && TILES * LINES == 2) ||
                                       (N == 1024 && OCC != 0 && TILES * LINES == 4));
}
template <typename T, int N, int LINES, int TILES, bool SPLIT, int KPRE, int KMID, int E = 16, int STORE = 0, int OCC = 0>
constexpr size_t frugal_lds_bytes() {
  return (size_t)TILES * LINES * line_lds_bytes<T, N, SPLIT, LINES>() +
         (frugal_tw_in_regs<T, N, E, LINES, TILES, OCC>() ? 0 : twiddle_lds_entries<N, E>() * sizeof(cx<T>)) +
         (sizeof(T) == 8 ? kCircleLds * sizeof(cx<double>) : 0) + kStoreScratch +
         (frugal_record_mode<LINES, TILES, KPRE>() == 1 ? (size_t)TILES * LINES * sizeof(MaskLine) : 0);
}

#ifndef PAOS_MINW_SMALL
#define PAOS_MINW_SMALL 3
#endif
#ifndef PAOS_F32_MINW
#define PAOS_F32_MINW 4
#endif
template <typename T, int N, int THREADS, int OCC = 0>
constexpr int frugal_min_waves() {
  if (OCC != 0) return 4;
  if (sizeof(T) == 4 && THREADS >= 1024) return 8;
  if (sizeof(T) == 4 && THREADS >= 512) return PAOS_F32_MINW;
  if (sizeof(T) == 8 && N == 4096 && THREADS == 256) return 4;
  return THREADS >= 512 ? 4 : PAOS_MINW_SMALL;
}

template <int THREADS>
__device__ __forceinline__ void tile_power_out(double acc, double* scratch, double* out) {
#pragma unroll
  for (int off = 32; off > 0; off >>= 1) acc += __shfl_down(acc, off, 64);
  if ((threadIdx.x & 63) == 0) scratch[threadIdx.x >> 6] = acc;
  __syncthreads();
  if (threadIdx.x == 0) {
    double s = 0.0;
#pragma unroll
    for (int w = 0; w < THREADS / 64; ++w) s += scratch[w];
    *out = s;
  }
}

#if PAOS_STAMPS
#define PAOS_FRUGAL_PARAMS const FrugalItem *k_items, void *k_field, unsigned k_pitch, unsigned k_item_stride, unsigned k_wg0, \
                           const void *k_tw, double *k_psf, double *k_psf_partial, double *k_pow_partial, const double *k_dyn_scale, \
                           unsigned long long *k_stamps
#define PAOS_FRUGAL_PASS(a) (a).items, (a).field, (a).pitch, (a).item_stride, (a).wg0, (a).tw, (a).psf, (a).psf_partial, (a).pow_partial, (a).dyn_scale, (a).stamps
#else
#define PAOS_FRUGAL_PARAMS const FrugalItem *k_items, void *k_field, unsigned k_pitch, unsigned k_item_stride, unsigned k_wg0, \
                           const void *k_tw, double *k_psf, double *k_psf_partial, double *k_pow_partial, const double *k_dyn_scale
#define PAOS_FRUGAL_PASS(a) (a).items, (a).field, (a).pitch, (a).item_stride, (a).wg0, (a).tw, (a).psf, (a).psf_partial, (a).pow_partial, (a).dyn_scale
#endif
template <typename T, int N, int E, int LINES, int TILES, int AXIS, int BR, int BC, bool SPLIT,
          int KPRE, int KMID, int NFFT, int STORE = 0, int TAB = 0, int LONG = 0, int OCC = 0, int CH = 0>
__global__ void __launch_bounds__(TILES* LINES* N / E, (frugal_min_waves<T, N, TILES * LINES * N / E, OCC>()))
    frugal_pass_kernel(PAOS_FRUGAL_PARAMS) {
  static_assert(LONG == 0 || (TAB != 0 && NFFT == 2 && KPRE == 1 && KMID == 1), "LONG builds: see above");
  static_assert(CH == 0 || (sizeof(T) == 8 && N == 4096 && E == 16 && TAB != 0 && KPRE == 1 && NFFT <= 2), "CH builds: see above");
  static_assert(CH >= 0 && CH <= 2 && (CH != 2 || STORE == 0), "CH = 2: field-storing builds");
  FrugalArgs a;
  a.items = k_items; a.field = k_field; a.pitch = k_pitch; a.item_stride = k_item_stride; a.wg0 = k_wg0;
  a.tw = k_tw; a.psf = k_psf; a.psf_partial = k_psf_partial; a.pow_partial = k_pow_partial; a.dyn_scale = k_dyn_scale; a.live_lo = a.live_hi = 0;
#if PAOS_STAMPS
  a.stamps = k_stamps;
#endif
  const int item = blockIdx.y;
  typedef const __attribute__((address_space(4))) FrugalItem* ConstItemPtr;
  const FrugalItem& it = *(const FrugalItem*)((ConstItemPtr)a.items + item);
  constexpr int kThreads = TILES * LINES * N / E;
  constexpr int kTwiddleLds = twiddle_lds_entries<N, E>();
  constexpr int kTwIt = (kTwiddleLds + kThreads - 1) / kThreads;
  constexpr int kClIt = sizeof(T) == 8 ? (kCircleLds + kThreads - 1) / kThreads : 1;
  constexpr int kExtra = (LONG + 1) / 2;
  const FrugalItem& it_last = LONG == 0 ? it : *(const FrugalItem*)((ConstItemPtr)a.items + item + kExtra * gridDim.y);
  const double h_active = it.active, h_line_lo = it.line_lo, h_line_hi = it.line_hi, h_line_fill = it_last.line_fill,
               h_pos_lo = it.pos_lo, h_pos_hi = it.pos_hi, h_spos_lo = it_last.spos_lo, h_spos_hi = it_last.spos_hi;
  const double h_mask_on = it.mid.mask_on;
  const MaskLine* const h_lines = it.mid.lines;
  const double h_dyn = *((const __attribute__((address_space(4))) double*)a.dyn_scale + item);
  if constexpr (frugal_record_mode<LINES, TILES, KPRE>() != 0)
    asm volatile("" ::"s"(h_active), "s"(h_line_lo), "s"(h_line_hi), "s"(h_line_fill), "s"(h_pos_lo), "s"(h_pos_hi), "s"(h_spos_lo),
                 "s"(h_spos_hi), "s"(h_mask_on), "s"(h_lines), "s"(h_dyn));
  else
    asm volatile("" ::"s"(h_active), "s"(h_line_lo), "s"(h_line_hi), "s"(h_line_fill), "s"(h_pos_lo), "s"(h_pos_hi), "s"(h_spos_lo),
                 "s"(h_spos_hi), "s"(h_dyn));
  if (h_active == 0.0) return;
  extern __shared__ __attribute__((aligned(16))) unsigned char smem[];
  constexpr bool kBlockIsLine = BR * BC * sizeof(cx<T>) >= 128;
  constexpr int COLSIB = (kBlockIsLine ? 1 : (int)(128 / (BR * BC * sizeof(cx<T>)))) * (AXIS == 1 && LINES < BC ? BC / LINES : 1);
  const unsigned wg = blockIdx.x + a.wg0;
  const TileMap<N, E, LINES, TILES, AXIS, BR, BC, 1, COLSIB> m(wg, threadIdx.x, a.pitch);
  cx<T>* f = reinterpret_cast<cx<T>*>(a.field) + (size_t)item * a.item_stride;
  constexpr bool NT = kBlockIsLine && ((AXIS == 1 && LINES >= BC) || (AXIS == 0 && LINES == BR));
  const int l0 = TILES == 1 ? (AXIS == 0 ? m.row0 : m.col0) : (int)wg * (TILES * LINES);
  {
    if (l0 + TILES * LINES <= (int)h_line_lo || l0 >= (int)h_line_hi) {
      if constexpr (STORE == 1) {
        if (h_line_fill == 0.0) return;
        if (l0 + TILES * LINES <= (int)h_spos_lo || l0 >= (int)h_spos_hi) return;
        double* ps = a.psf + (size_t)item * a.item_stride;
#pragma unroll
        for (int k = 0; k < E; ++k) ps[m.base + (unsigned)k * m.stride] = 0.0;
        if (threadIdx.x == 0) a.psf_partial[(size_t)item * (N / LINES / TILES) + wg] = 0.0;
        return;
      }
      if (h_line_fill != 0.0) {
#pragma unroll
        for (int k = 0; k < E; ++k)
          stream_store<NT>(reinterpret_cast<cx<T>*>(reinterpret_cast<char*>(f) + (m.base + (unsigned)k * m.stride) * (unsigned)sizeof(cx<T>)),
                           cx<T>{(T)0, (T)0});
      }
      return;
    }
  }
  void* lds = smem + (size_t)m.lds_line * line_lds_bytes<T, N, SPLIT, LINES>();
  cx<T>* tw_lds = reinterpret_cast<cx<T>*>(smem + (size_t)TILES * LINES * line_lds_bytes<T, N, SPLIT, LINES>());
  constexpr bool kTwRegs = frugal_tw_in_regs<T, N, E, LINES, TILES, OCC>();
  const cx<T>* tw = kTwRegs ? reinterpret_cast<const cx<T>*>(a.tw) : tw_lds;
  cx<double>* cl = reinterpret_cast<cx<double>*>(tw_lds + (kTwRegs ? 0 : kTwiddleLds));
  const cx<double>* circle = sizeof(T) == 8 ? cl : nullptr;
#if PAOS_STAMPS
  if (threadIdx.x == 0) {
    unsigned long long* st = a.stamps + ((size_t)blockIdx.y * gridDim.x + blockIdx.x) * kStampSlots;
    st[8] = __builtin_amdgcn_s_memrealtime();
    st[9] = ((unsigned long long)__builtin_amdgcn_s_getreg((31 << 11) | 20) << 32) | __builtin_amdgcn_s_getreg((31 << 11) | 4);
  }
#endif
  PAOS_STAMP(0);

  const char* fb = reinterpret_cast<const char*>(f);
  const unsigned boff = m.base * (unsigned)sizeof(cx<T>);
  const size_t bstride = (size_t)(m.stride * (unsigned)sizeof(cx<T>));
  auto at = [&](int k) {
    const unsigned long long u = (unsigned long long)(fb + (size_t)k * bstride);
    const unsigned lo = (unsigned)__builtin_amdgcn_readfirstlane((int)(unsigned)u);
    const unsigned hi = (unsigned)__builtin_amdgcn_readfirstlane((int)(unsigned)(u >> 32));
    typedef __attribute__((address_space(1))) char* GlobalBytes;
    unsigned bo = boff;
    asm volatile("" : "+v"(bo));
    return (cx<T>*)((GlobalBytes)(((unsigned long long)hi << 32) | lo) + bo);
  };
  constexpr int kRecMode = frugal_record_mode<LINES, TILES, KPRE>();
  constexpr int kRecs = kRecMode == 2 ? 2 : 0;
  MaskLine mrec[kRecs > 0 ? kRecs : 1] = {};
  const int lbase = __builtin_amdgcn_readfirstlane(l0);
  if constexpr (kRecs > 0) {
    if (h_mask_on != 0.0) {
#pragma unroll
      for (int j = 0; j < kRecs; ++j) mrec[j] = h_lines[lbase + j];
    }
  }
  constexpr int kPlainPre = KPRE != 0 ? 0 : (AXIS == 1 ? PAOS_COL_PRE : PAOS_ROW_PRE);
  cx<T> v[E];
  const int plo = (int)h_pos_lo, phi = (int)h_pos_hi;
  if constexpr (CH != 0) {
#pragma unroll
    for (int k = 0; k < E; ++k) v[k] = cx<T>{(T)0, (T)0};
#pragma unroll
    for (int k = ch_first<E, CH>(); k < ch_end<E, CH>(); ++k) {
      const int pos = m.t + k * (N / E);
      if (pos >= plo && pos < phi) v[k] = stream_load<NT>(at(k));
    }
  } else if (plo <= 0 && phi >= N) {
#pragma unroll
    for (int k = 0; k < E; ++k) v[k] = stream_load<NT>(at(k));
  } else {
#pragma unroll
    for (int k = 0; k < E; ++k) {
      const int pos = m.t + k * (N / E);
      v[k] = cx<T>{(T)0, (T)0};
      if (pos >= plo && pos < phi) v[k] = stream_load<NT>(at(k));
    }
  }
  __builtin_amdgcn_sched_barrier(0);
  cx<T> tw_fetch[kTwIt], cl_fetch[kClIt];
  constexpr int kRecDwords = kRecMode == 1 ? TILES * LINES * (int)(sizeof(MaskLine) / 4) : 0;
  static_assert(kRecDwords <= 128, "the record area is filled by the first 128 threads");
  const bool stage_recs = kRecMode == 1 && h_mask_on != 0.0;
  unsigned rec_fetch = 0;
  if constexpr (kRecMode == 1) {
    if (stage_recs && (int)threadIdx.x < kRecDwords) rec_fetch = reinterpret_cast<const unsigned*>(h_lines + lbase)[threadIdx.x];
  }
  constexpr int kLastTpt = E / last_radix<N, E>();
  cx<T> w1_keep[kLastTpt];
#pragma unroll
  for (int q = 0; q < kLastTpt; ++q) w1_keep[q] = cx<T>{(T)1, (T)0};
  if constexpr (kTwRegs) {
#pragma unroll
    for (int q = 0; q < kLastTpt; ++q) w1_keep[q] = reinterpret_cast<const cx<T>*>(a.tw)[m.t + q * (N / E)];
  }
  const cx<T>* const w1_last = kTwRegs ? w1_keep : nullptr;
#pragma unroll
  for (int j = 0; j < kTwIt; ++j) {
    const int i = (int)threadIdx.x + j * kThreads;
    tw_fetch[j] = cx<T>{(T)0, (T)0};
    if (!kTwRegs && i < kTwiddleLds) tw_fetch[j] = reinterpret_cast<const cx<T>*>(a.tw)[i];
  }
  if constexpr (sizeof(T) == 8) {
#pragma unroll
    for (int j = 0; j < kClIt; ++j) {
      const int i = (int)threadIdx.x + j * kThreads;
      cl_fetch[j] = cx<T>{(T)0, (T)0};
      if (i < kCircleLds) cl_fetch[j] = reinterpret_cast<const cx<T>*>(a.tw)[i * (N / kCircleLds)];
    }
  }
#pragma unroll
  for (int j = 0; j < kTwIt; ++j) {
    const int i = (int)threadIdx.x + j * kThreads;
    if (!kTwRegs && i < kTwiddleLds) tw_lds[i] = tw_fetch[j];
  }
  if constexpr (sizeof(T) == 8) {
#pragma unroll
    for (int j = 0; j < kClIt; ++j) {
      const int i = (int)threadIdx.x + j * kThreads;
      if (i < kCircleLds) cl[i] = {(double)cl_fetch[j].x, -(double)cl_fetch[j].y};
    }
  }
  MaskLine* rec_lds = reinterpret_cast<MaskLine*>(smem + frugal_lds_bytes<T, N, LINES, TILES, SPLIT, KPRE, KMID, E, 0, OCC>() -
                                                  (kRecMode == 1 ? (size_t)TILES * LINES * sizeof(MaskLine) : 0));
  if constexpr (kRecMode == 1) {
    if (stage_recs && (int)threadIdx.x < kRecDwords) reinterpret_cast<unsigned*>(rec_lds)[threadIdx.x] = rec_fetch;
  }
  asm volatile("s_waitcnt lgkmcnt(0)\n\ts_barrier" ::: "memory");
  PAOS_STAMP_WAIT_VM();
  PAOS_STAMP(1);

  const bool ran1 = it.fft1_on != 0.0;
  const bool ran2 = NFFT == 2 && it.fft2_on != 0.0;
  const bool inv1 = ran1 && it.fft1_inv != 0.0;
  constexpr bool kShare = TAB == 0;
  frugal_slot<T, N, E, KPRE, decltype(m), kPlainPre, kShare && KMID == 0, 0, TAB, CH>(v, it.pre, it.pre_ph, m, circle, false, inv1, m.t, lds, false);
  PAOS_STAMP(2);
  if (ran1) frugal_fft<T, N, E, SPLIT, false, CH>(v, lds, m.t, tw, circle, it.fft1_inv, w1_last);
  PAOS_STAMP(3);
  constexpr bool kShareMid = kShare && KPRE == 0 && KMID < 3;
  constexpr int kNarrowMid = (CH == 2 && NFFT == 1 && LONG == 0 && KMID > 0) ? 2 : 0;
  frugal_slot<T, N, E, KMID, decltype(m), 0, kShareMid, (kRecMode == 1 ? -1 : kRecs), TAB, kNarrowMid>(
      v, it.mid, it.mid_ph, m, circle, inv1, ran2 && it.fft2_inv != 0.0, m.t, lds, ran1, kRecMode == 1 ? rec_lds : mrec, lbase, h_dyn);
  PAOS_STAMP(4);
  if constexpr (NFFT == 2) {
    if (ran2) {
      if (ran1 && !(kShareMid && KMID > 0)) __syncthreads();
      frugal_fft<T, N, E, SPLIT>(v, lds, m.t, tw, circle, it.fft2_inv, w1_last);
    }
  }
  if constexpr (LONG != 0) {
    bool busy = ran1 || ran2;
#define PAOS_EXTRA_PASS(ix, kTwo)                                                                                                    \
  {                                                                                                                                  \
    const bool ran3 = (ix).fft1_on != 0.0;                                                                                           \
    const bool ran4 = (kTwo) && (ix).fft2_on != 0.0;                                                                                 \
    const bool inv3 = ran3 && (ix).fft1_inv != 0.0;                                                                                  \
    frugal_slot<T, N, E, 1, decltype(m), 0, false, 0, TAB>(v, (ix).pre, (ix).pre_ph, m, circle, false, inv3, m.t, lds, false);       \
    if constexpr (CH == 2 && !(kTwo)) pin_tile<E>(v);                                                                                \
    if (ran3) {                                                                                                                      \
      if (busy) __syncthreads();                                                                                                     \
      frugal_fft<T, N, E, SPLIT, false>(v, lds, m.t, tw, circle, (ix).fft1_inv, w1_last);                                            \
      busy = true;                                                                                                                   \
    }                                                                                                                                \
                \
    frugal_slot<T, N, E, 1, decltype(m), 0, false, 0, TAB, (CH == 2 && !(kTwo)) ? 2 : 0>(                                            \
        v, (ix).mid, (ix).mid_ph, m, circle, inv3, ran4 && (ix).fft2_inv != 0.0, m.t, lds, ran3);                                    \
    if constexpr (CH == 2 && (kTwo)) pin_tile<E>(v);                                                                                 \
    if constexpr (kTwo) {                                                                                                            \
      if (ran4) {                                                                                                                    \
        if (busy) __syncthreads();                                                                                                   \
        frugal_fft<T, N, E, SPLIT>(v, lds, m.t, tw, circle, (ix).fft2_inv, w1_last);                                                 \
        busy = true;                                                                                                                 \
      }                                                                                                                              \
    }                                                                                                                                \
  }
    const FrugalItem& it2 = *(const FrugalItem*)((ConstItemPtr)a.items + item + gridDim.y);
    if constexpr (LONG == 1) PAOS_EXTRA_PASS(it2, false)
    else PAOS_EXTRA_PASS(it2, true)
    if constexpr (LONG == 3) PAOS_EXTRA_PASS(it_last, false)
    if constexpr (LONG == 4) PAOS_EXTRA_PASS(it_last, true)
#undef PAOS_EXTRA_PASS
  }
  PAOS_STAMP(5);
  [[maybe_unused]] double* const scratch = reinterpret_cast<double*>(
      smem + frugal_lds_bytes<T, N, LINES, TILES, SPLIT, KPRE, KMID, E, 0, OCC>() - kStoreScratch - (kRecMode == 1 ? (size_t)TILES * LINES * sizeof(MaskLine) : 0));
  if constexpr (STORE == 1) {
    double* ps = a.psf + (size_t)item * a.item_stride;
    double acc = 0.0;
#pragma unroll
    for (int k = 0; k < E; ++k) {
      const double x = (double)v[k].x, y = (double)v[k].y;
      const double w = __dadd_rn(__dmul_rn(x, x), __dmul_rn(y, y));
      ps[m.base + (unsigned)k * m.stride] = w;
      acc += w;
    }
    tile_power_out<TILES * LINES * N / E>(acc, scratch, a.psf_partial + (size_t)item * (N / LINES / TILES) + wg);
    return;
  }
  const int slo = (int)h_spos_lo, shi = (int)h_spos_hi;
  if constexpr (CH == 2) {
#pragma unroll
    for (int k = ch_first<E, CH>(); k < ch_end<E, CH>(); ++k) {
      const int pos = m.t + k * (N / E);
      if (pos >= slo && pos < shi) stream_store<NT>(at(k), v[k]);
    }
  } else if (slo <= 0 && shi >= N) {
#pragma unroll
    for (int k = 0; k < E; ++k) stream_store<NT>(at(k), v[k]);
  } else {
#pragma unroll
    for (int k = 0; k < E; ++k) {
      const int pos = m.t + k * (N / E);
      if (pos >= slo && pos < shi) stream_store<NT>(at(k), v[k]);
    }
  }
  if constexpr (STORE == 2) {
    double acc = 0.0;
#pragma unroll
    for (int k = 0; k < E; ++k) {
      const double x = (double)v[k].x, y = (double)v[k].y;
      acc += __dadd_rn(__dmul_rn(x, x), __dmul_rn(y, y));
    }
    tile_power_out<TILES * LINES * N / E>(acc, scratch, a.pow_partial + (size_t)item * (N / LINES / TILES) + wg);
  }
  PAOS_STAMP(6);
  PAOS_STAMP_WAIT_VM();
  PAOS_STAMP(7);
#if PAOS_STAMPS
  if (threadIdx.x == 0)
    a.stamps[((size_t)blockIdx.y * gridDim.x + blockIdx.x) * kStampSlots + 10] = __builtin_amdgcn_s_memrealtime();
#endif
}

}
```

### paos_amd/csrc/host.h

```cpp
#pragma once
#include "../../include/paos_hip.h"

#include <hip/hip_runtime.h>

#include <cstdlib>
#include <string>
#include <type_traits>
#include <vector>

#include "arena_layout.h"
#include "frugal_pass.h"
#include "pass_records.h"

using namespace paos;

#ifndef PAOS_BR
#define PAOS_BR 4
#endif
#ifndef PAOS_PAD_BLOCKS
#define PAOS_PAD_BLOCKS 3
#endif
inline constexpr int BR = PAOS_BR;
#ifndef PAOS_F32_BR
#define PAOS_F32_BR 8
#endif
template <typename T, int N>
constexpr int block_rows() { return (sizeof(T) == 4 && N >= 2048) ? PAOS_F32_BR : PAOS_BR; }
inline constexpr int kNormSlots = PAOS_NORM_SLOTS;
template <typename T>
struct Lay {
  static constexpr int BC = 2;
};

constexpr int kArenaSlabs = 4;
struct Arena {
  double* host = nullptr;
  double* dev = nullptr;
  ArenaLayout lay;
  int cur = 0;
  int left = -1;
  hipEvent_t fence[kArenaSlabs] = {};
  bool fenced[kArenaSlabs] = {};
  bool used[kArenaSlabs] = {};
};

struct paos_ctx {
  int device = 0, n = 0, batch = 0, precision = 0;
  int br = PAOS_BR;
  unsigned pitch = 0, item_stride = 0;
  hipStream_t stream = nullptr;
  double* psf = nullptr;
  void* focus_spec = nullptr;
  bool focus_open = false;
  void* otf_spec = nullptr;
  bool otf_computed = false, otf_valid = false;
  double* otf_cuts = nullptr;
  std::vector<double> blur_tabs, blur_key;
  cx<double>* zoom_t = nullptr;
  double* zoom_psf = nullptr;
  cx<double>* zoom_field = nullptr;
  int zoom_m = 0;
  bool zoom_done = false, zoom_has_field = false;
  double* zoom_tabs = nullptr;
  int zoom_s = 0, zoom_cap = 0;
  std::vector<double> zoom_fracs;
  std::vector<std::vector<int>> zoom_carry;
  double* map_dev = nullptr;
  unsigned long long map_key = 0;
  double map_max = 0.0;
  std::vector<double> start_key;
  double* start_norm2 = nullptr;
  std::vector<double> start_partial_key;
  double* start_partial = nullptr;
  cx<double>* psd_scratch = nullptr;
  int* psd_bad = nullptr;
  double* psf_partial = nullptr;
  int psf_nparts = 0;
  double* pow_partial = nullptr;
  int pow_nparts = 0;
  cx<double>* ptab = nullptr;
  int ptab_slots = 0;
  double* dyn_scale = nullptr;
  bool dyn_pending = false;
  unsigned long long deferred_rode = 0, deferred_settled = 0;
  bool norm2_of_field = false;
  int psf_zero_axis = -1;
  std::vector<double> psf_zero_lo, psf_zero_hi;
  bool det_set = false;
  int det_nx = 0, det_ny = 0;
  double det_geom[4] = {};
  double* det_img = nullptr;
  double* det_rows = nullptr;
  size_t det_rows_bytes = 0;
  double* det_out = nullptr;
  size_t det_out_bytes = 0;
  double* ee_buf = nullptr;
  size_t ee_bytes = 0;
  int ee_bins = 0, ee_curves = 0;
  bool ee_computed = false, ee_valid = false;
  double* wf_buf = nullptr;
  size_t wf_bytes = 0;
  int wf_pairs = 0;
  bool wf_fitted = false;
  double* series_par = nullptr;
  size_t series_par_bytes = 0;
  double* series_host = nullptr;
  size_t series_host_bytes = 0;
  hipEvent_t series_ev = nullptr;
  double* series_flux = nullptr;
  size_t series_flux_bytes = 0;
  double* series_frames = nullptr;
  size_t series_frames_bytes = 0;
  int series_nframes = 0, series_nboxes = 0;
  bool series_done = false;
  void* bounce[2] = {nullptr, nullptr};
  hipEvent_t bounce_ev[2] = {nullptr, nullptr};
  void* field = nullptr;
  void* tw = nullptr;
  void* staging = nullptr;
  cx<double>* tables = nullptr;
  double* mask = nullptr;
  double* metric_partial = nullptr;
  double* metric_out = nullptr;
  double* metric_host = nullptr;
  struct MaskSet {
    MaskLine* lines = nullptr;
    double* vals = nullptr;
    std::vector<double> key;
    unsigned long long used = 0;
    int line_lo = 0, line_hi = 0;
  };
  static constexpr int kMaskSets = 8;
  MaskSet mask_sets[kMaskSets];
  unsigned long long mask_clock = 0;
  unsigned long long mask_hits = 0, mask_rendered = 0;
  size_t lds_pad = 0;
  bool central_half = true;
  unsigned long long central_launches = 0, plain_launches = 0;
  bool narrow_windows = true;
  unsigned long long narrow_launches = 0, other_launches = 0;
  std::vector<int> pass_builds;
  int* mask_overflow = nullptr;
  unsigned long long* block_stats = nullptr;
  double* partial = nullptr;
  double* norm2 = nullptr;
  double* norm2_host = nullptr;
  bool prune = true;
  int norm_slot = 0;
  bool norm_busy[64] = {};
  int nparts = 0;
  Arena arena;
  std::string err;
  int prof_kind = -1;
  std::vector<hipEvent_t> prof_events;
  std::vector<int> prof_tags;
  int prof_next_tag = 0;
  double prof_next_bytes = 0.0;
  std::vector<double> prof_bytes;
  double prof_next_lines = 0.0;
  std::vector<double> prof_lines;
  size_t prof_used = 0;
};

#pragma GCC visibility push(hidden)

int fail(paos_ctx* c, int code, const std::string& msg);

#define HIPCHK(c, call)                                                                     \
  do {                                                                                      \
    hipError_t e_ = (call);                                                                 \
    if (e_ != hipSuccess)                                                                   \
      return fail((c), PAOS_EHIP,                                                           \
                  std::string(#call) + ": " + hipGetErrorString(e_) + " (" __FILE__ ":" +   \
                      std::to_string(__LINE__) + ")");                                      \
  } while (0)

inline size_t elem_bytes(const paos_ctx* c) { return c->precision == PAOS_F64 ? 16 : 8; }

inline bool env_is(const char* name, char ch) {
  const char* e = getenv(name);
  return e && e[0] == ch;
}

template <typename T, int N>
struct FftCfg {
  static constexpr int BC = Lay<T>::BC;
  static constexpr int BR = block_rows<T, N>();
  static constexpr int E = 16;
  static constexpr int ROW_LINES = (N >= 2048) ? PAOS_BR / 2 : PAOS_BR;
  static constexpr int FR_ROW_LINES = (N >= 2048) ? BR / 2 : BR;
  static constexpr int COL_LINES = BC;
  static constexpr int ROW_THREADS = ROW_LINES * N / E, COL_THREADS = COL_LINES * N / E;
  static constexpr int ROW_TILES = (ROW_THREADS >= 128) ? 1 : 128 / ROW_THREADS;
  static constexpr int COL_TILES = (COL_THREADS >= 128) ? 1 : 128 / COL_THREADS;
  static constexpr bool ROW_SPLIT = (size_t)ROW_LINES * ROW_TILES * line_lds_bytes<T, N, false>() > 144 * 1024;
  static constexpr bool COL_SPLIT = (size_t)COL_LINES * COL_TILES * line_lds_bytes<T, N, false>() > 144 * 1024;
  static constexpr int MINW = 1;
};
inline int frugal_tile_lines(const paos_ctx* c, int axis) { return axis == 0 ? (c->n >= 2048 ? c->br / 2 : c->br) : 2; }

int arena_reserve(paos_ctx* c, size_t total);
int arena_push(paos_ctx* c, const double* src, size_t count, const double** dev);
class ArenaBatch {
 public:
  explicit ArenaBatch(paos_ctx* c) : c_(c) {}
  int begin(size_t total);
  int add(const double* src, size_t count, const double** dev);
  int commit();

 private:
  paos_ctx* c_;
  ArenaBatchState st_;
};
int arena_settled(paos_ctx* c, int rc);
int copy_to_host(paos_ctx* c, void* host, const void* dev, size_t bytes);
int next_norm_slot(paos_ctx* c);
int check_mask_overflow(paos_ctx* c);
int check_rows(paos_ctx* c, const double* rows);
std::vector<double> rounded_cols(const paos_ctx* c, const double* cols);
int opt_in_lds(paos_ctx* c, const void* kern, size_t lds);
bool timed_launch_begin(paos_ctx* c, int kind);
hipError_t timed_launch_end(paos_ctx* c, int tag);

int launch_failed(paos_ctx* c, const char* call, hipError_t e, const char* file, int line);
#define TIMED_LAUNCH(c, ...) timed_launch(__FILE__, __LINE__, (c), __VA_ARGS__)
template <typename Kern, typename... Args>
int timed_launch(const char* file, int line, paos_ctx* c, Kern kern, dim3 grid, dim3 block, size_t lds, size_t lds_opt_in, int kind,
                 int tag, Args... args) {
  if (lds_opt_in) {
    int rc = opt_in_lds(c, (const void*)kern, lds_opt_in);
    if (rc) return rc;
  }
  const bool timed = timed_launch_begin(c, kind);
  hipLaunchKernelGGL(kern, grid, block, lds, c->stream, args...);
  hipError_t e = hipGetLastError();
  if (e != hipSuccess) return launch_failed(c, "hipGetLastError()", e, file, line);
  if (timed && (e = timed_launch_end(c, tag)) != hipSuccess) return launch_failed(c, "timed_launch_end(c, tag)", e, file, line);
  return PAOS_OK;
}
inline size_t generic_lds_opt_in(size_t lds) { return lds > 48 * 1024 ? lds : 0; }
// ... 65 lines not shown
```

### paos_amd/csrc/paos_hip.hip

```cpp
#include "host.h"

#include <algorithm>
#include <cmath>
#include <cstring>

#include "item_groups.h"
#include "pointwise.h"

namespace {

int pw_blocks(const paos_ctx* c) {
  const size_t total = (size_t)c->item_stride;
  size_t b = (total + kPwThreads - 1) / kPwThreads;
  return (int)(b < 2048 ? b : 2048);
}

__global__ void dyn_scale_set_kernel(double* dyn, const double* norm2, const double* enable, int batch) {
  const int i = blockIdx.x * blockDim.x + threadIdx.x;
  if (i < batch) dyn[i] = (!enable || enable[i] != 0.0) ? 1.0 / sqrt(norm2[i]) : 1.0;
}
__global__ void dyn_scale_reset_kernel(double* dyn, int batch) {
  const int i = blockIdx.x * blockDim.x + threadIdx.x;
  if (i < batch) dyn[i] = 1.0;
}
// ... 244 lines not shown
  }
  bool power_found = false;
  if (any_stop) {
    power_found = memo && c->start_norm2 && same_key(key, c->start_key);
    if (power_found) HIPCHK(c, hipMemcpyAsync(c->norm2, c->start_norm2, (size_t)batch * sizeof(double), hipMemcpyDeviceToDevice, c->stream));
    else c->start_key.clear();
  }
  bool partial_found = false;
  double* partial = c->partial;
  if (want_power && memo) {
    pkey = key;
    pkey.insert(pkey.end(), write_rows, write_rows + (size_t)2 * batch);
    pkey.insert(pkey.end(), wc.begin(), wc.end());
    pkey.insert(pkey.end(), lead.begin(), lead.end());
    pkey.insert(pkey.end(), same.begin(), same.end());
    partial_found = c->start_partial && same_key(pkey, c->start_partial_key);
    if (!partial_found) c->start_partial_key.clear();
    if (!c->start_partial) HIPCHK(c, hipMalloc(&c->start_partial, (size_t)batch * c->nparts * sizeof(double)));
    partial = c->start_partial;
  }
  const dim3 block(kPwThreads), sweep(pw_blocks(c), batch), parts(c->nparts, batch);
  dispatch_layout(c, [&](auto t, auto br) {
    using T = decltype(t);
    constexpr int BRV = decltype(br)::value, BC = Lay<T>::BC;
    dispatch_either<0, 1>(shape == PAOS_SHAPE_ELLIPSE, [&](auto s) {
      constexpr int S = decltype(s)::value;
      if (any_stop && !power_found) {
        hipLaunchKernelGGL((start_power_kernel<T, BRV, BC, S>), parts, block, 0, c->stream, dp, c->n, c->pitch, c->item_stride, re, im,
                           c->partial, dcompute);
        hipLaunchKernelGGL(norm2_final_kernel, dim3(batch), block, 0, c->stream, c->partial, c->norm2, c->nparts, ds, 1, dpower_of);
      }
      if (!zk) {
        hipLaunchKernelGGL((start_write_kernel<T, BRV, BC, S>), sweep, block, 0, c->stream, (cx<T>*)c->field, dp, c->n, c->pitch,
                           c->item_stride, re, im, (const double*)c->norm2, ds, drows, dgoff, dglen, dmembers, dcols);
        return;
      }
      dispatch_either<8, 0>(zk->nmax <= 8, [&](auto nc) {
        hipLaunchKernelGGL((zernike_start_write_kernel<T, BRV, BC, S, decltype(nc)::value>), sweep, block, 0, c->stream, (cx<T>*)c->field,
                           dp, c->n, c->pitch, c->item_stride, re, im, (const double*)c->norm2, ds, drows, dcols, dgoff, dglen, dsubs,
                           dmembers, dzt, dzp, zk->param_stride, zk->nmax, zk->kdim);
      });
      if (want_power && !partial_found)
        hipLaunchKernelGGL((start_norm2_partial_kernel<T, BRV, BC, S>), parts, block, 0, c->stream, partial, dp, c->n, c->pitch,
                           c->item_stride, re, im, (const double*)c->norm2, ds, dlead, drows, dcols);
    });
  });
  HIPCHK(c, hipGetLastError());
  if (any_stop && !power_found && memo) {
    if (!c->start_norm2) HIPCHK(c, hipMalloc(&c->start_norm2, (size_t)batch * sizeof(double)));
    HIPCHK(c, hipMemcpyAsync(c->start_norm2, c->norm2, (size_t)batch * sizeof(double), hipMemcpyDeviceToDevice, c->stream));
    c->start_key = std::move(key);
  }
  if (want_power && !partial_found && memo) c->start_partial_key = std::move(pkey);
  if (want_power) return take_power_ticket(c, partial, c->nparts, dsame, zk->power_ticket);
  return PAOS_OK;
}

static int start_impl(paos_ctx* c, double re, double im, int shape, const double* aperture, const double* stop,
                      const double* write_rows, const double* write_cols = nullptr, const StartZernike* zk = nullptr) {
  const int rc = arena_settled(c, start_body(c, re, im, shape, aperture, stop, write_rows, write_cols, zk));
  if (rc != PAOS_OK && c) start_forget(c);
  return rc;
}

int paos_start(paos_ctx* c, double re, double im, int shape, const double* aperture, const double* stop) {
  return paos_start_box(c, re, im, shape, aperture, stop, nullptr, nullptr);
}

int paos_start_rows(paos_ctx* c, double re, double im, int shape, const double* aperture, const double* stop,
                    const double* write_rows) {
  return paos_start_box(c, re, im, shape, aperture, stop, write_rows, nullptr);
}

int paos_start_box(paos_ctx* c, double re, double im, int shape, const double* aperture, const double* stop,
                   const double* write_rows, const double* write_cols) {
  DROP_SCALE(c);
  return start_impl(c, re, im, shape, aperture, stop, write_rows, write_cols);
}

int paos_start_zernike_box(paos_ctx* c, double re, double im, int shape, const double* aperture, const double* stop,
                           const double* write_rows, const double* write_cols, int nmax, int kdim, const double* table,
                           const double* params, int param_stride, int* power_ticket) {
  DROP_SCALE(c);
  if (c && (!write_rows || !write_cols)) return fail(c, PAOS_EINVAL, "paos_start_zernike_box: null window");
  const StartZernike zk{nmax, kdim, param_stride, table, params, power_ticket};
  return start_impl(c, re, im, shape, aperture, stop, write_rows, write_cols, &zk);
}

int paos_zero_outside_box(paos_ctx* c, const double* live_rows, const double* live_cols) {
  SETTLE_SCALE(c);
  if (c) (void)hipSetDevice(c->device);
  if (!c || !live_rows) return fail(c, PAOS_EINVAL, "null argument");
  int rc = check_rows(c, live_rows);
  if (rc) return rc;
  if (live_cols && (rc = check_rows(c, live_cols))) return rc;
  return arena_settled(c, zero_outside_box(c, live_rows, live_cols));
}

int paos_zero_outside_rows(paos_ctx* c, const double* live_rows) { return paos_zero_outside_box(c, live_rows, nullptr); }

int paos_import(paos_ctx* c, int item, const void* host) {
  SETTLE_SCALE(c);
  if (c) (void)hipSetDevice(c->device);
  if (!c || !host || item < 0 || item >= c->batch) return fail(c, PAOS_EINVAL, "bad item or null buffer");
  const size_t bytes = (size_t)c->n * c->n * 16;
  HIPCHK(c, hipMemcpyAsync(c->staging, host, bytes, hipMemcpyHostToDevice, c->stream));
  dispatch_layout(c, [&](auto t, auto br) {
    using T = decltype(t);
    hipLaunchKernelGGL((import_kernel<T, decltype(br)::value, Lay<T>::BC>), dim3(pw_blocks(c)), dim3(kPwThreads), 0, c->stream,
                       (cx<T>*)c->field + (size_t)item * c->item_stride, (const cx<double>*)c->staging, c->n, c->pitch);
  });
  HIPCHK(c, hipGetLastError());
  HIPCHK(c, hipStreamSynchronize(c->stream));
  return PAOS_OK;
}

static int export_impl(paos_ctx* c, int item, int what, void* host_out, bool pinned) {
  if (!c || !host_out || item < 0 || item >= c->batch || what < 0 || what > 3)
    return fail(c, PAOS_EINVAL, "bad item/what or null buffer");
  dispatch_layout(c, [&](auto t, auto br) {
    using T = decltype(t);
    hipLaunchKernelGGL((export_kernel<T, decltype(br)::value, Lay<T>::BC>), dim3(pw_blocks(c)), dim3(kPwThreads), 0, c->stream,
                       (const cx<T>*)c->field + (size_t)item * c->item_stride, (double*)c->staging, c->n, c->pitch, what);
  });
  HIPCHK(c, hipGetLastError());
  const size_t bytes = (size_t)c->n * c->n * (what == PAOS_WHAT_FIELD ? 16 : 8);
  if (pinned) {
    HIPCHK(c, hipMemcpyAsync(host_out, c->staging, bytes, hipMemcpyDeviceToHost, c->stream));
    HIPCHK(c, hipStreamSynchronize(c->stream));
  } else {
    int rc = copy_to_host(c, host_out, c->staging, bytes);
    if (rc) return rc;
  }
  return check_mask_overflow(c);
}

int paos_export(paos_ctx* c, int item, int what, void* host_out) {
  SETTLE_SCALE(c);
  if (c) (void)hipSetDevice(c->device);
  return export_impl(c, item, what, host_out, false);
}

int paos_export_pinned(paos_ctx* c, int item, int what, void* pinned_out) {
  SETTLE_SCALE(c);
  if (c) (void)hipSetDevice(c->device);
  return export_impl(c, item, what, pinned_out, true);
}

int paos_psf_keep(paos_ctx* c) {
  SETTLE_SCALE(c);
  if (c) (void)hipSetDevice(c->device);
  if (!c) return fail(c, PAOS_EINVAL, "null context");
  if (!c->psf) HIPCHK(c, hipMalloc(&c->psf, (size_t)c->batch * c->item_stride * sizeof(double)));
  c->psf_zero_axis = -1;
  c->otf_valid = c->ee_valid = false;
  const dim3 grid(pw_blocks(c), c->batch), block(kPwThreads);
  dispatch_layout(c, [&](auto t, auto br) {
    using T = decltype(t);
    hipLaunchKernelGGL((intensity_kernel<T, decltype(br)::value, Lay<T>::BC>), grid, block, 0, c->stream, (const cx<T>*)c->field,
                       c->psf, c->n, c->pitch, c->item_stride);
  });
  HIPCHK(c, hipGetLastError());
  return PAOS_OK;
}

int paos_psf_fetch(paos_ctx* c, int item, double* host_out) {
  if (c) (void)hipSetDevice(c->device);
  if (!c || !host_out || item < 0 || item >= c->batch) return fail(c, PAOS_EINVAL, "bad item or null buffer");
  if (!c->psf) return fail(c, PAOS_EINVAL, "no PSF kept (paos_psf_keep)");
  dispatch_layout(c, [&](auto t, auto br) {
    hipLaunchKernelGGL((psf_unblock_kernel<decltype(br)::value, Lay<decltype(t)>::BC>), dim3(pw_blocks(c)), dim3(kPwThreads), 0, c->stream,
                       (const double*)c->psf + (size_t)item * c->item_stride, (double*)c->staging, c->n, c->pitch);
  });
  HIPCHK(c, hipGetLastError());
  return copy_to_host(c, host_out, c->staging, (size_t)c->n * c->n * sizeof(double));
}

static int aperture_launch(paos_ctx* c, int shape, const double* dp, int nitems, double* mask_out) {
  const dim3 grid(pw_blocks(c), nitems), block(kPwThreads);
  dispatch_layout(c, [&](auto t, auto br) {
    using T = decltype(t);
    dispatch_either<0, 1>(shape == PAOS_SHAPE_ELLIPSE, [&](auto s) {
      hipLaunchKernelGGL((aperture_kernel<T, decltype(br)::value, Lay<T>::BC, decltype(s)::value>), grid, block, 0, c->stream,
                         mask_out ? (cx<T>*)nullptr : (cx<T>*)c->field, dp, (const double*)nullptr, AP_STRIDE, c->n, c->pitch,
                         c->item_stride, mask_out, 0);
    });
  });
  HIPCHK(c, hipGetLastError());
  return PAOS_OK;
}

int paos_aperture(paos_ctx* c, int shape, const double* params) {
  SETTLE_SCALE(c);
  if (c) (void)hipSetDevice(c->device);
  if (!c || !params) return fail(c, PAOS_EINVAL, "null argument");
  if (shape != PAOS_SHAPE_ELLIPSE && shape != PAOS_SHAPE_RECT) return fail(c, PAOS_EINVAL, "unknown aperture shape");
  const double* dp = nullptr;
  int rc = arena_push(c, params, (size_t)c->batch * AP_STRIDE, &dp);
  if (rc) return rc;
  return aperture_launch(c, shape, dp, c->batch, nullptr);
}

int paos_aperture_render(paos_ctx* c, int shape, const double* params1, double* host_mask) {
  if (c) (void)hipSetDevice(c->device);
  if (!c || !params1 || !host_mask) return fail(c, PAOS_EINVAL, "null argument");
  if (shape != PAOS_SHAPE_ELLIPSE && shape != PAOS_SHAPE_RECT) return fail(c, PAOS_EINVAL, "unknown aperture shape");
  const double* dp = nullptr;
  int rc = arena_push(c, params1, AP_STRIDE, &dp);
  if (rc) return rc;
  rc = aperture_launch(c, shape, dp, 1, (double*)c->staging);
  if (rc) return rc;
  return copy_to_host(c, host_mask, c->staging, (size_t)c->n * c->n * 8);
}

static int push_enable(paos_ctx* c, const double* enable, const double** den) {
  *den = nullptr;
  return enable ? arena_push(c, enable, (size_t)c->batch, den) : PAOS_OK;
}

static int norm2_launch(paos_ctx* c, const double* den) {
  norm2_partial_launch(c, den);
  HIPCHK(c, hipGetLastError());
  hipLaunchKernelGGL(norm2_final_kernel, dim3(c->batch), dim3(kPwThreads), 0, c->stream, c->partial, c->norm2, c->nparts, den, 1);
  HIPCHK(c, hipGetLastError());
  return PAOS_OK;
}

int paos_make_stop(paos_ctx* c, const double* enable) {
  SETTLE_SCALE(c);
  if (c) (void)hipSetDevice(c->device);
  if (!c) return fail(c, PAOS_EINVAL, "null context");
  const double* den;
  int rc = push_enable(c, enable, &den);
  if (rc || (rc = norm2_launch(c, den))) return rc;
  stop_scale_launch(c, den);
  HIPCHK(c, hipGetLastError());
  return PAOS_OK;
}

int paos_stop_scale_last_power(paos_ctx* c, const double* enable) {
  if (!c) return fail(c, PAOS_EINVAL, "null context");
  if (!c->norm2_of_field) return paos_make_stop(c, enable);
  SETTLE_SCALE(c);
  (void)hipSetDevice(c->device);
  const double* den;
  if (int rc = push_enable(c, enable, &den)) return rc;
  stop_scale_launch(c, den);
  HIPCHK(c, hipGetLastError());
  return PAOS_OK;
}

int paos_stop_defer_last_power(paos_ctx* c, const double* enable) {
  if (!c) return fail(c, PAOS_EINVAL, "null context");
  if (!c->norm2_of_field) return paos_make_stop(c, enable);
  (void)hipSetDevice(c->device);
  SETTLE_SCALE(c);
  const double* den;
  if (int rc = push_enable(c, enable, &den)) return rc;
  hipLaunchKernelGGL(dyn_scale_set_kernel, dim3((c->batch + 255) / 256), dim3(256), 0, c->stream, c->dyn_scale, c->norm2, den, c->batch);
  HIPCHK(c, hipGetLastError());
  c->dyn_pending = true;
  return PAOS_OK;
}

int paos_psf_metrics(paos_ctx* c, int nr, const double* radii_px, double cx_px, double cy_px, double* host_out) {
  SETTLE_SCALE(c);
  if (c) (void)hipSetDevice(c->device);
  if (!c || !host_out || nr < 0 || nr > kMaxRadii || (nr > 0 && !radii_px)) return fail(c, PAOS_EINVAL, "bad metrics request");
  for (int k = 0; k < nr; ++k)
    if (!(radii_px[k] >= 0.0) || !std::isfinite(radii_px[k])) return fail(c, PAOS_EINVAL, "radii must be finite and >= 0");
  if (!std::isfinite(cx_px) || !std::isfinite(cy_px)) return fail(c, PAOS_EINVAL, "the centre must be finite");
  const int nvals = 4 + nr, nblocks = 512;
  if (!c->metric_partial) {
    HIPCHK(c, hipMalloc(&c->metric_partial, (size_t)c->batch * nblocks * (4 + kMaxRadii) * sizeof(double)));
    HIPCHK(c, hipMalloc(&c->metric_out, (size_t)c->batch * (4 + kMaxRadii) * sizeof(double)));
    HIPCHK(c, hipHostMalloc(&c->metric_host, (size_t)c->batch * (4 + kMaxRadii) * sizeof(double)));
  }
  MetricArgs a{};
  a.field = c->field; a.partial = c->metric_partial; a.n = c->n; a.nr = nr; a.pitch = c->pitch;
  a.item_stride = c->item_stride; a.cx = cx_px; a.cy = cy_px;
  for (int k = 0; k < nr; ++k) a.r2[k] = radii_px[k] * radii_px[k];
  const dim3 grid(nblocks, c->batch), block(kPwThreads);
  dispatch_layout(c, [&](auto t, auto br) {
    hipLaunchKernelGGL((psf_metrics_kernel<decltype(t), decltype(br)::value, Lay<decltype(t)>::BC>), grid, block, 0, c->stream, a);
  });
  HIPCHK(c, hipGetLastError());
  hipLaunchKernelGGL(psf_metrics_final_kernel, dim3(c->batch), dim3(64), 0, c->stream, c->metric_partial, c->metric_out, nblocks, nvals);
  HIPCHK(c, hipGetLastError());
  HIPCHK(c, hipMemcpyAsync(c->metric_host, c->metric_out, (size_t)c->batch * nvals * sizeof(double), hipMemcpyDeviceToHost, c->stream));
  HIPCHK(c, hipStreamSynchronize(c->stream));
  std::memcpy(host_out, c->metric_host, (size_t)c->batch * nvals * sizeof(double));
  return check_mask_overflow(c);
}

int paos_norm2_enqueue(paos_ctx* c, int* ticket) {
  SETTLE_SCALE(c);
  if (c) (void)hipSetDevice(c->device);
  if (!c || !ticket) return fail(c, PAOS_EINVAL, "null argument");
  if (int rc = power_ring_full(c)) return rc;
  norm2_partial_launch(c, nullptr);
  HIPCHK(c, hipGetLastError());
  return take_power_ticket(c, c->partial, c->nparts, nullptr, ticket);
}

}

int psf_keep_power_impl(paos_ctx* c, int* ticket) {
  if (int rc = power_ring_full(c)) return rc;
  if (!c->psf) HIPCHK(c, hipMalloc(&c->psf, (size_t)c->batch * c->item_stride * sizeof(double)));
  c->psf_zero_axis = -1;
  c->otf_valid = c->ee_valid = false;
  const dim3 grid(c->nparts, c->batch), block(kPwThreads);
  dispatch_layout(c, [&](auto t, auto br) {
    using T = decltype(t);
    hipLaunchKernelGGL((intensity_power_kernel<T, decltype(br)::value, Lay<T>::BC>), grid, block, 0, c->stream, (const cx<T>*)c->field,
                       c->psf, c->partial, c->n, c->pitch, c->item_stride);
  });
  HIPCHK(c, hipGetLastError());
  return take_power_ticket(c, c->partial, c->nparts, nullptr, ticket);
}

int zero_outside_rows(paos_ctx* c, const double* live_rows) {
  const size_t eb = elem_bytes(c);
  for (int i = 0; i < c->batch; ++i) {
    const int br = c->br;
    int lo = ((int)live_rows[2 * i] / br) * br, hi = (((int)live_rows[2 * i + 1] + br - 1) / br) * br;
    if (hi > c->n) hi = c->n;
    if (lo >= hi) { lo = 0; hi = 0; }
    char* base = (char*)c->field + (size_t)i * c->item_stride * eb;
    const size_t row_bytes = (size_t)c->pitch / br * eb;
    if (lo > 0) HIPCHK(c, hipMemsetAsync(base, 0, (size_t)lo * row_bytes, c->stream));
    if (hi < c->n) HIPCHK(c, hipMemsetAsync(base + (size_t)hi * row_bytes, 0, (size_t)(c->n - hi) * row_bytes, c->stream));
  }
  return PAOS_OK;
}

int zero_outside_box(paos_ctx* c, const double* live_rows, const double* live_cols) {
  if (!live_cols) return zero_outside_rows(c, live_rows);
  const double *drows = nullptr, *dcols = nullptr;
  int rc;
  const std::vector<double> lc = rounded_cols(c, live_cols);
  ArenaBatch ab(c);
  if ((rc = ab.add(live_rows, (size_t)2 * c->batch, &drows))) return rc;
  if ((rc = ab.add(lc.data(), lc.size(), &dcols))) return rc;
  if ((rc = ab.commit())) return rc;
  const dim3 grid(pw_blocks(c), c->batch), block(kPwThreads);
  dispatch_layout(c, [&](auto t, auto br) {
    using T = decltype(t);
    hipLaunchKernelGGL((zero_outside_box_kernel<T, decltype(br)::value, Lay<T>::BC>), grid, block, 0, c->stream, (cx<T>*)c->field, c->n,
                       c->pitch, c->item_stride, drows, dcols);
  });
  HIPCHK(c, hipGetLastError());
  return PAOS_OK;
}

extern "C" {

int paos_psf_keep_power(paos_ctx* c, int* ticket) {
  SETTLE_SCALE(c);
  if (c) (void)hipSetDevice(c->device);
  if (!c || !ticket) return fail(c, PAOS_EINVAL, "null argument");
  return psf_keep_power_impl(c, ticket);
}

static int norm2_enqueue_rows_impl(paos_ctx* c, const double* live_rows, const double* same_as, int* ticket,
                                   const double* live_cols = nullptr) {
  if (c) (void)hipSetDevice(c->device);
  if (!c || !ticket || !live_rows) return fail(c, PAOS_EINVAL, "null argument");
  int rc = check_rows(c, live_rows);
  if (rc) return rc;
  if ((rc = power_ring_full(c))) return rc;
  const double *drows = nullptr, *dlead = nullptr, *dsame = nullptr, *dcols = nullptr;
  const size_t nb = (size_t)c->batch;
  ArenaBatch ab(c);
  if ((rc = ab.begin((live_cols ? 2 : 1) * arena_rounded(2 * nb) + (same_as ? 2 : 0) * arena_rounded(nb)))) return rc;
  if ((rc = ab.add(live_rows, 2 * nb, &drows))) return rc;
  if (live_cols) {
    const std::vector<double> lc = rounded_cols(c, live_cols);
    if ((rc = ab.add(lc.data(), lc.size(), &dcols))) return rc;
  }
  if (same_as) {
    if (!same_as_valid(same_as, c->batch, true)) return fail(c, PAOS_EINVAL, "same_as must name an item that stands for itself");
    std::vector<double> lead(c->batch);
    for (int i = 0; i < c->batch; ++i) {
      const int j = (int)same_as[i];
      if (live_rows[2 * i] != live_rows[2 * j] || live_rows[2 * i + 1] != live_rows[2 * j + 1] ||
          (live_cols && (live_cols[2 * i] != live_cols[2 * j] || live_cols[2 * i + 1] != live_cols[2 * j + 1])))
        return fail(c, PAOS_EINVAL, "items that share a sum must share their row (and column) window");
      lead[i] = j == i ? 1.0 : 0.0;
    }
    if ((rc = ab.add(lead.data(), lead.size(), &dlead))) return rc;
    if ((rc = ab.add(same_as, nb, &dsame))) return rc;
  }
  if ((rc = ab.commit())) return rc;
  norm2_partial_launch(c, dlead, drows, dcols);
  HIPCHK(c, hipGetLastError());
  return take_power_ticket(c, c->partial, c->nparts, dsame, ticket);
}

int paos_norm2_enqueue_box(paos_ctx* c, const double* live_rows, const double* live_cols, const double* same_as, int* ticket) {
  SETTLE_SCALE(c);
  if (c && live_cols) {
    int rc = check_rows(c, live_cols);
    if (rc) return rc;
  }
  return arena_settled(c, norm2_enqueue_rows_impl(c, live_rows, same_as, ticket, live_cols));
}

int paos_norm2_enqueue_rows(paos_ctx* c, const double* live_rows, int* ticket) {
  SETTLE_SCALE(c);
  return arena_settled(c, norm2_enqueue_rows_impl(c, live_rows, nullptr, ticket));
}

int paos_norm2_enqueue_rows_like(paos_ctx* c, const double* live_rows, const double* same_as, int* ticket) {
  SETTLE_SCALE(c);
  if (!same_as) return fail(c, PAOS_EINVAL, "null argument");
  return arena_settled(c, norm2_enqueue_rows_impl(c, live_rows, same_as, ticket));
}

int paos_norm2(paos_ctx* c, double* host_out) {
  SETTLE_SCALE(c);
  if (c) (void)hipSetDevice(c->device);
  if (!c || !host_out) return fail(c, PAOS_EINVAL, "null argument");
  int rc = norm2_launch(c, nullptr);
  if (rc) return rc;
  HIPCHK(c, hipMemcpyAsync(c->norm2_host, c->norm2, (size_t)c->batch * sizeof(double), hipMemcpyDeviceToHost, c->stream));
  HIPCHK(c, hipStreamSynchronize(c->stream));
  std::memcpy(host_out, c->norm2_host, (size_t)c->batch * sizeof(double));
  return PAOS_OK;
}

int paos_phase_map(paos_ctx* c, int item, const double* host_wfe, double wl) {
  SETTLE_SCALE(c);
  if (c) (void)hipSetDevice(c->device);
  if (!c || !host_wfe || item < 0 || item >= c->batch) return fail(c, PAOS_EINVAL, "bad item or null buffer");
  if (!(wl > 0.0) || !std::isfinite(wl)) return fail(c, PAOS_EINVAL, "wavelength must be positive and finite");
  const size_t count = (size_t)c->n * c->n;
  double wmax = 0.0;
  for (size_t i = 0; i < count; ++i) {
    if (!std::isfinite(host_wfe[i])) return fail(c, PAOS_EINVAL, "the phase map holds a non-finite value (fill masked pixels with 0)");
    wmax = std::max(wmax, std::fabs(host_wfe[i]));
  }
  if (!phase_map_argument_finite(wmax, wl)) return fail(c, PAOS_EINVAL, kPhaseMapOverflow);
  HIPCHK(c, hipMemcpyAsync(c->staging, host_wfe, count * sizeof(double), hipMemcpyHostToDevice, c->stream));
  dispatch_layout(c, [&](auto t, auto br) {
    using T = decltype(t);
    hipLaunchKernelGGL((phase_map_kernel<T, decltype(br)::value, Lay<T>::BC>), dim3(pw_blocks(c)), dim3(kPwThreads), 0, c->stream,
                       (cx<T>*)c->field + (size_t)item * c->item_stride, (const double*)c->staging, c->n, c->pitch, wl);
  });
  HIPCHK(c, hipGetLastError());
  HIPCHK(c, hipStreamSynchronize(c->stream));
  return PAOS_OK;
}

int paos_phase_map_items(paos_ctx* c, const double* host_wfe, unsigned long long key, int n_items, const double* items,
                         const double* wl) {
  SETTLE_SCALE(c);
  if (c) (void)hipSetDevice(c->device);
  if (!c || !items || !wl || n_items < 1 || n_items > c->batch) return fail(c, PAOS_EINVAL, "bad item list or null buffer");
  if (!host_wfe && (key == 0 || key != c->map_key || !c->map_dev)) return fail(c, PAOS_EINVAL, "no host map, and no map kept on the device under this key");
  for (int k = 0; k < n_items; ++k) {
    if (!(items[k] >= 0.0) || items[k] >= (double)c->batch || items[k] != (double)(int)items[k]) return fail(c, PAOS_EINVAL, "bad item index");
    if (!(wl[k] > 0.0) || !std::isfinite(wl[k])) return fail(c, PAOS_EINVAL, "wavelength must be positive and finite");
// ... 334 lines not shown
```

### paos_amd/csrc/pass_program.h

```cpp
#pragma once
#include "../../include/paos_hip.h"

#include <cmath>
#include <cstddef>
#include <cstring>
#include <vector>

#include "pass_records.h"

#pragma GCC visibility push(hidden)

using namespace paos;

struct PlanDims {
  int n, batch, br;
  int precision;
  int central_half;
  int narrow_windows = 1;
};
struct PlanSwitches {
  bool line_tables = true;
  bool fuse_pairs = true;
  bool compact_grid = true;
  bool env_prune = true;
  bool stage_program = true;
  bool batched_records = true;
  bool psf_zero_reuse = true;
  bool ctx_prune = true;
};

struct OpList {
  const paos_pw_op* ops;
  int count;
};
inline OpList op_list(const paos_pass& p, int l) {
  return l == 0 ? OpList{p.pre, p.n_pre} : (l == 1 ? OpList{p.mid, p.n_mid} : OpList{p.post, p.n_post});
}
inline bool is_phase(const paos_pw_op& op) { return op.kind == PAOS_PW_QPHASE_CENTRED || op.kind == PAOS_PW_QPHASE_NATURAL; }

enum PhaseCheck { PHASES_OK = 0, PHASE_BLOCK_OUT_OF_RANGE, PHASE_TOO_LARGE };
inline PhaseCheck check_phase_args(const PlanDims& d, const paos_pass* passes, int n_passes, const double* blocks, int n_blocks) {
  for (int i = 0; i < n_passes; ++i)
    for (int l = 0; l < 3; ++l) {
      const OpList ol = op_list(passes[i], l);
      for (int o = 0; o < ol.count && o < PAOS_MAX_PW; ++o) {
        const paos_pw_op& op = ol.ops[o];
        if (!is_phase(op)) continue;
        if (op.block < 0 || op.block >= n_blocks) return PHASE_BLOCK_OUT_OF_RANGE;
        for (int it = 0; it < d.batch; ++it) {
          const double* p = blocks + ((size_t)op.block * d.batch + it) * FP_STRIDE;
          if (p[FP_ENABLE] == 0.0) continue;
          const double hx = 0.5 * d.n * p[FP_SX], hy = 0.5 * d.n * p[FP_SY];
          double arg = std::fabs(p[FP_COEF]) * (hx * hx + hy * hy);
          if (op.flags & PAOS_PWF_MUL2PI) arg *= 6.283185307179586;
          if (!(arg < kMaxPhaseArg)) return PHASE_TOO_LARGE;
        }
      }
    }
  return PHASES_OK;
}

inline bool lower_frugal(const PlanDims& d, const paos_pass& p, const double* blocks , LoweredPass& lp) {
  std::vector<FrugalItem>& items = lp.items;
  int &kpre = lp.kpre, &kmid = lp.kmid, &nfft = lp.nfft, &mask_block = lp.mask_block, &mask_slot = lp.mask_slot;
  std::vector<double>& mask_shared = lp.mask_shared;
  std::vector<int>& mask_rep = lp.mask_rep;
  if (p.axis != 0 && p.axis != 1) return false;
  if (p.fft1 < 0 || p.n_post != 0) return false;
  const OpList lists[2] = {op_list(p, 0), op_list(p, 1)};
  int k[2] = {0, 0};
  mask_block = -1; mask_slot = -1;
  for (int l = 0; l < 2; ++l)
    for (int o = 0; o < lists[l].count; ++o) {
      const int kind = lists[l].ops[o].kind;
      if (is_phase(lists[l].ops[o])) {
        ++k[l];
        for (int it = 0; it < d.batch; ++it) {
          const double* q = blocks + ((size_t)lists[l].ops[o].block * d.batch + it) * FP_STRIDE;
          if (q[FP_ENABLE] != 0.0 && std::fabs(q[FP_SGN]) != 1.0) return false;
        }
      }
      else if (kind == PAOS_PW_MASK) {
        if (mask_block >= 0) return false;
        mask_block = lists[l].ops[o].block; mask_slot = l;
      } else if (kind != PAOS_PW_SIGN && kind != PAOS_PW_SCALE) return false;
    }
  if (k[0] > kFrugalMaxPre || k[1] > kFrugalMaxMid) return false;
  if (mask_block >= 0) {
    for (int it = 0; it < d.batch; ++it) {
      const double* q = blocks + ((size_t)mask_block * d.batch + it) * FP_STRIDE;
      const double* q2 = blocks + ((size_t)(mask_block + 1) * d.batch + it) * FP_STRIDE;
      if (q[0] == 0.0) continue;
      const double a = q[3], b = q[4], theta = q2[0], obsc = q2[1], subpix = q2[2], shape = q2[3];
      if (theta != 0.0 || !(a > 0.0) || !(b > 0.0)) return false;
      if (shape == PAOS_SHAPE_ELLIPSE) {
        const double along = p.axis == 0 ? a : b, across = p.axis == 0 ? b : a;
        if (!(across >= 2.0) || 2.0 * along * std::sqrt(3.0 / across) + 8.0 > kMaskW) return false;
      } else {
        const int sp = (int)subpix;
        if (obsc != 0.0 || sp <= 0 || (sp & (sp - 1)) != 0) return false;
      }
    }
  }
  kpre = k[0]; kmid = k[1]; nfft = p.fft2 >= 0 ? 2 : 1;
  items.assign(d.batch, FrugalItem{});
  mask_shared.assign(d.batch, 0.0);
  mask_rep.assign(d.batch, -1);
  auto blk = [&](int b, int it) { return blocks + ((size_t)b * d.batch + it) * FP_STRIDE; };
  for (int it = 0; it < d.batch; ++it) {
    FrugalItem& fi = items[it];
    const double* c1 = blk(p.fft1, it);
    fi.fft1_on = c1[FC_ENABLE] != 0.0; fi.fft1_inv = c1[FC_INVERSE] != 0.0;
    if (p.fft2 >= 0) { const double* c2 = blk(p.fft2, it); fi.fft2_on = c2[FC_ENABLE] != 0.0; fi.fft2_inv = c2[FC_INVERSE] != 0.0; }
    bool active = fi.fft1_on != 0.0 || fi.fft2_on != 0.0;
    FrugalSlot* slots[2] = {&fi.pre, &fi.mid};
    FrugalPhase* phases[2] = {fi.pre_ph, fi.mid_ph};
    int sign_bits[2] = {0, 0};
    for (int l = 0; l < 2; ++l) {
      slots[l]->sign_on = 0.0; slots[l]->scale = 1.0;
      sign_bits[l] = 0;
      slots[l]->mask_on = 0.0; slots[l]->w_in = 1.0; slots[l]->w_out = 0.0;
      slots[l]->lines = nullptr; slots[l]->vals = nullptr;
      int j = 0;
      for (int o = 0; o < lists[l].count; ++o) {
        const paos_pw_op& op = lists[l].ops[o];
        const double* q = blk(op.block, it);
        const bool on = q[FP_ENABLE] != 0.0;
        active = active || on;
        if (op.kind == PAOS_PW_MASK) {
          const double* q2 = blk(op.block + 1, it);
          slots[l]->mask_on = on ? 1.0 : 0.0;
          const bool obsc = q2[1] != 0.0 && q2[3] == PAOS_SHAPE_ELLIPSE;
          slots[l]->w_in = obsc ? 0.0 : 1.0; slots[l]->w_out = obsc ? 1.0 : 0.0;
          int rep = it;
          for (int j = 0; j < it; ++j)
            if (!std::memcmp(blk(op.block, j), q, FP_STRIDE * sizeof(double)) &&
                !std::memcmp(blk(op.block + 1, j), q2, FP_STRIDE * sizeof(double))) { rep = j; break; }
          mask_shared[it] = rep != it ? 1.0 : 0.0;
          mask_rep[it] = rep;
        } else if (op.kind == PAOS_PW_SIGN) {
          if (on) {
            const bool x_only = op.flags & PAOS_PWF_X_ONLY, y_only = op.flags & PAOS_PWF_Y_ONLY;
            const int along = p.axis == 0 ? (y_only ? 0 : 1) : (x_only ? 0 : 1);
            const int across = p.axis == 0 ? (x_only ? 0 : 1) : (y_only ? 0 : 1);
            sign_bits[l] ^= along | (across << 1);
          }
        }
        else if (op.kind == PAOS_PW_SCALE) { if (on) slots[l]->scale *= q[FP_COEF]; }
        else {
          FrugalPhase& ph = phases[l][j++];
          ph.natural = op.kind == PAOS_PW_QPHASE_NATURAL ? 1.0 : 0.0;
          if (on) { ph.sx = q[FP_SX]; ph.sy = q[FP_SY]; ph.coef = q[FP_COEF] * q[FP_SGN]; ph.sgn = 1.0; ph.m2 = (op.flags & PAOS_PWF_MUL2PI) ? 6.283185307179586 : 1.0; }
          else { ph.sx = ph.sy = 0.0; ph.coef = 0.0; ph.sgn = 1.0; ph.m2 = 1.0; }
        }
      }
      slots[l]->sign_on = sign_bits[l] == 3 ? 1.0 : (sign_bits[l] == 1 ? 2.0 : (sign_bits[l] == 2 ? 3.0 : 0.0));
    }
    fi.active = active ? 1.0 : 0.0;
    fi.line_lo = 0.0; fi.line_hi = (double)d.n; fi.line_fill = 0.0; fi.pos_lo = 0.0; fi.pos_hi = (double)d.n;
    fi.spos_lo = 0.0; fi.spos_hi = (double)d.n;
  }
  if (kpre == 0)
    for (const FrugalItem& fi : items)
      if (fi.active != 0.0 && (fi.pre.sign_on != 0.0 || fi.pre.scale != 1.0 || fi.pre.mask_on != 0.0)) { kpre = 1; break; }
  return true;
}


inline bool mask_live_range(const PlanDims& d, const double* q, const double* q2, int axis, int* lo, int* hi) {
  if (q[0] == 0.0 || q2[0] != 0.0 || q2[1] != 0.0) return false;
  const double centre = axis == 0 ? q[2] : q[1];
  double ext = axis == 0 ? q[4] : q[3];
  if (q2[3] != PAOS_SHAPE_ELLIPSE) ext = ext / 2.0;
  if (!std::isfinite(centre) || !std::isfinite(ext) || !(ext > 0.0)) return false;
  const double a = std::floor(centre - ext + 0.5) - 1.0, b = std::ceil(centre + ext + 0.5) + 1.0;
  const int n = d.n;
  int l = a < 0.0 ? 0 : (a > n ? n : (int)a), h = b < 0.0 ? 0 : (b > n ? n : (int)b);
  const int br = d.br;
  l = (l / br) * br;
  h = ((h + br - 1) / br) * br;
  if (h > n) h = n;
  if (l >= h) { l = 0; h = br; }
  *lo = l; *hi = h;
  return true;
}

struct LineRange { int lo, hi; };

inline void plan_pruning(const PlanDims& d, const paos_pass* passes, int n_passes, const double* blocks,
                         std::vector<LoweredPass>& low, const double* entry_rows, bool entry_stale, const double* entry_cols) {
  const int n = d.n, br = d.br;
  auto meet = [br](LineRange a, LineRange b) {
    LineRange r{a.lo > b.lo ? a.lo : b.lo, a.hi < b.hi ? a.hi : b.hi};
    if (r.lo >= r.hi) { r.lo = a.lo; r.hi = a.lo + br < a.hi ? a.lo + br : a.hi; }
    return r;
  };
  std::vector<int> act;
  std::vector<LineRange> lines, loads;
  for (int it = 0; it < d.batch; ++it) {
    act.clear();
    for (int q = 0; q < n_passes; ++q)
      if (low[q].items[it].active != 0.0) act.push_back(q);
    if (act.empty()) continue;
    LineRange box[2] = {{0, n}, {0, n}};
    bool clean = false;
    LineRange rows0{0, n};
    if (entry_rows) {
      int l = (int)entry_rows[2 * it], h = (int)entry_rows[2 * it + 1];
      l = l < 0 ? 0 : (l / br) * br;
      h = h > n ? n : ((h + br - 1) / br) * br;
      if (h > n) h = n;
      if (l < h && (l > 0 || h < n)) { box[0] = {l, h}; clean = !entry_stale; }
      rows0 = box[0];
    }
    if (entry_cols && entry_stale) {
      int l = (int)entry_cols[2 * it], h = (int)entry_cols[2 * it + 1];
      l = l < 0 ? 0 : (l / br) * br;
      h = h > n ? n : ((h + br - 1) / br) * br;
      if (h > n) h = n;
      if (l < h && (l > 0 || h < n)) box[1] = {l, h};
    }
    lines.assign(act.size(), LineRange{0, n});
    loads.assign(act.size(), LineRange{0, n});
    for (size_t k = 0; k < act.size(); ++k) {
      const int q = act[k], ax = passes[q].axis;
      const FrugalItem& fi = low[q].items[it];
      LineRange& L = box[ax];
      LineRange& P = box[1 - ax];
      LineRange ml{0, n}, mp{0, n};
      bool masked = false;
      if (low[q].mask_block >= 0) {
        const double* mq = blocks + ((size_t)low[q].mask_block * d.batch + it) * FP_STRIDE;
        const double* mq2 = blocks + ((size_t)(low[q].mask_block + 1) * d.batch + it) * FP_STRIDE;
        masked = mask_live_range(d, mq, mq2, ax, &ml.lo, &ml.hi) && mask_live_range(d, mq, mq2, 1 - ax, &mp.lo, &mp.hi);
      }
      if (masked) L = meet(L, ml);
      lines[k] = L;
      LineRange pos = P;
      if (masked && low[q].mask_slot == 0) pos = meet(pos, mp);
      loads[k] = pos;
      if (fi.fft1_on != 0.0) pos = {0, n};
      if (masked && low[q].mask_slot == 1) pos = meet(pos, mp);
      if (low[q].nfft >= 2 && fi.fft2_on != 0.0) pos = {0, n};
      P = pos;
    }
    LineRange want[2] = {{0, n}, {0, n}};
    for (size_t k = act.size(); k-- > 0;) {
      const int q = act[k], ax = passes[q].axis;
      FrugalItem& fi = low[q].items[it];
      const LineRange proc = meet(lines[k], want[ax]);
      fi.line_lo = proc.lo; fi.line_hi = proc.hi;
      fi.pos_lo = loads[k].lo; fi.pos_hi = loads[k].hi;
      fi.spos_lo = want[1 - ax].lo; fi.spos_hi = want[1 - ax].hi;
      want[ax] = proc;
      want[1 - ax] = loads[k];
    }
    for (size_t k = 0; k < act.size(); ++k) {
      const FrugalItem& fi = low[act[k]].items[it];
      if (passes[act[k]].axis != 0 || (int)fi.line_lo != rows0.lo || (int)fi.line_hi != rows0.hi || fi.spos_lo > 0.0 ||
          fi.spos_hi < (double)n)
        clean = false;
    }
    FrugalItem& last = low[act.back()].items[it];
    if ((last.line_lo > 0.0 || last.line_hi < (double)n) && !clean) last.line_fill = 1.0;
  }
}

inline void record_window(const PlanDims& d, LoweredPass& lp) {
  double lo = (double)d.n, hi = 0.0;
  for (const FrugalItem& fi : lp.items) {
    if (fi.active == 0.0) continue;
    lo = fi.line_lo < lo ? fi.line_lo : lo;
    hi = fi.line_hi > hi ? fi.line_hi : hi;
  }
  const bool window = hi > lo;
  lp.mask_lo = window ? (int)lo : 0;
  lp.mask_hi = window ? (int)hi : d.n;
}

inline bool entry_zero_first(const PlanDims& d, bool pruned, const std::vector<LoweredPass>& low, const double* entry_rows,
                             const double* entry_cols) {
  bool need = !pruned;
  for (int it = 0; it < d.batch && !need; ++it) {
    bool active = false;
    for (const LoweredPass& lp : low) active = active || lp.items[it].active != 0.0;
    need = !active;
  }
  const double* windows[2] = {entry_rows, entry_cols};
  for (int w = 0; w < 2 && !need; ++w)
    for (int it = 0; windows[w] && it < d.batch && !need; ++it) {
      const int br = d.br, l = ((int)windows[w][2 * it] / br) * br;
      int h = (((int)windows[w][2 * it + 1] + br - 1) / br) * br;
      if (h > d.n) h = d.n;
      need = l >= h;
    }
  return need;
}

inline int last_pass_store(const std::vector<LoweredPass>& low, int final_mode) {
  if (final_mode == 0 || low.empty()) return 0;
  const LoweredPass& last = low.back();
  bool ok = last.ok && last.kpre <= 1 && (final_mode == 2 || last.kmid <= 1);
  if (ok)
    for (const FrugalItem& fi : last.items) ok = ok && fi.active != 0.0;
  return ok ? final_mode : 0;
}

inline void psf_zero_fill(const PlanDims& d, const PlanSwitches& sw, int axis, std::vector<FrugalItem>& last, int known_axis,
                          std::vector<double>& zero_lo, std::vector<double>& zero_hi) {
  const bool known = sw.psf_zero_reuse && known_axis == axis && (int)zero_lo.size() == d.batch;
  zero_lo.resize(d.batch); zero_hi.resize(d.batch);
  for (int it = 0; it < d.batch; ++it) {
    const double old_lo = known ? zero_lo[it] : 0.0, old_hi = known ? zero_hi[it] : (double)d.n;
    const bool covered = old_lo >= last[it].line_lo && old_hi <= last[it].line_hi;
    last[it].line_fill = covered ? 0.0 : 1.0;
    last[it].spos_lo = covered ? 0.0 : old_lo;
    last[it].spos_hi = covered ? (double)d.n : old_hi;
    zero_lo[it] = last[it].line_lo; zero_hi[it] = last[it].line_hi;
  }
}

inline std::vector<int> batched_renderings(const PlanSwitches& sw, bool all_frugal, const std::vector<LoweredPass>& low) {
  std::vector<int> todo;
  bool safe = sw.batched_records && all_frugal;
  for (int q = 0; q < (int)low.size() && safe; ++q) {
    if (low[q].mask_block < 0) continue;
    if (low[q].mask_render) {
      for (int r = 0; r < q; ++r) safe = safe && !(low[r].mask_block >= 0 && low[r].mask_set == low[q].mask_set);
      todo.push_back(q);
    }
  }
  if (!safe || todo.size() <= 1) todo.clear();
  return todo;
}

inline bool phases_along_lines(const PlanSwitches& sw, int axis, const LoweredPass& lp, bool or_none = false) {
  if (!sw.line_tables || (lp.kpre + lp.kmid == 0 && !or_none)) return false;
  const int counts[2] = {lp.kpre, lp.kmid};
  for (int l = 0; l < 2; ++l)
    for (const FrugalItem& fi : lp.items) {
      if (fi.active == 0.0) continue;
      const FrugalPhase* ph = l == 0 ? fi.pre_ph : fi.mid_ph;
      for (int j = 0; j < counts[l]; ++j)
        if ((axis == 0 ? ph[j].sy : ph[j].sx) != 0.0) return false;
    }
  return true;
}

inline bool can_fuse_pair(const PlanDims& d, const PlanSwitches& sw, int axis, const LoweredPass& lp, int axis2, const LoweredPass& lp2) {
  if (!sw.fuse_pairs) return false;
  if (!lp.ok || !lp2.ok || axis != axis2 || lp.nfft != 2) return false;
  if (lp.mask_block >= 0 && lp2.mask_block >= 0 && lp.mask_set == lp2.mask_set) return false;
  if (!phases_along_lines(sw, axis, lp, true) || !phases_along_lines(sw, axis2, lp2, true)) return false;
  for (int it = 0; it < d.batch; ++it) {
    const FrugalItem &f1 = lp.items[it], &f2 = lp2.items[it];
    if ((f1.active != 0.0) != (f2.active != 0.0)) return false;
    if (f1.active != 0.0 && (f1.line_lo != f2.line_lo || f1.line_hi != f2.line_hi || f1.line_fill != 0.0)) return false;
  }
  return true;
}

struct Launch {
  LoweredPass* lp[3] = {nullptr, nullptr, nullptr};
  int q = 0, count = 1, axis = 0;
  bool tables = false;
  size_t item_base = 0;
  int store = 0;
  FrugalBuild build{};
  int narrow = 0;
  unsigned live_lo = 0, live_hi = 0;
  int tag = 0;
  double bytes = 0.0, lines = 0.0;
  const LoweredPass& last() const { return *lp[count - 1]; }
};

inline std::vector<Launch> form_launches(const PlanDims& d, const PlanSwitches& sw, const paos_pass* passes, int n_passes,
                                         std::vector<LoweredPass>& low, bool fusable, std::vector<int>& launch_of) {
  std::vector<Launch> launches;
  launch_of.assign(n_passes, -1);
  for (int q = 0; q < n_passes;) {
    Launch g;
    g.q = q; g.axis = passes[q].axis; g.lp[0] = &low[q];
    if (low[q].ok && fusable) {
      const bool pair = q + 1 < n_passes && can_fuse_pair(d, sw, passes[q].axis, low[q], passes[q + 1].axis, low[q + 1]);
      const bool triple = pair && q + 2 < n_passes && can_fuse_pair(d, sw, passes[q + 1].axis, low[q + 1], passes[q + 2].axis, low[q + 2]) &&
                          !(low[q].mask_block >= 0 && low[q + 2].mask_block >= 0 && low[q].mask_set == low[q + 2].mask_set);
      g.count = triple ? 3 : (pair ? 2 : 1);
      for (int k = 1; k < g.count; ++k) g.lp[k] = &low[q + k];
    }
    launch_of[q] = (int)launches.size();
    launches.push_back(g);
    q += g.count;
  }
  return launches;
}

inline bool stage_whole_program(const PlanDims& d, const PlanSwitches& sw, bool all_frugal, int n_passes) {
  const size_t table_bytes = (size_t)2 * n_passes * d.batch * d.n * 2 * sizeof(double);
  return all_frugal && sw.stage_program && table_bytes <= (size_t(1) << 30);
}

inline void decide_tables(const PlanDims& d, const PlanSwitches& sw, Launch& g) {
  g.tables = g.count > 1 || (d.precision == PAOS_F64 && phases_along_lines(sw, g.axis, *g.lp[0]));
  if (g.tables && g.count == 1) {
    double lines = 0.0, active = 0.0;
    for (const FrugalItem& fi : g.lp[0]->items)
      if (fi.active != 0.0) { lines += fi.line_hi - fi.line_lo; active += 1.0; }
    if (active > 0.0 && lines > 0.5 * active * d.n) g.tables = false;
  }
}

inline bool build_exists(const PlanDims& d, const FrugalBuild& b) {
  return dispatch_family(d.precision, d.n, false, [&](auto t, auto n) { return frugal_built<decltype(t), decltype(n)::value>(b); });
}

inline FrugalBuild pick_build(const PlanDims& d, const Launch& g) {
  const LoweredPass& lp = *g.lp[0];
  const LoweredPass *next = g.lp[1], *next2 = g.lp[2];
  FrugalBuild b{};
  b.axis = g.axis;
  b.kpre = next ? 1 : (g.tables && lp.kpre > 1 ? 1 : lp.kpre);
  b.kmid = next ? 1 : (g.tables && lp.kmid > 1 ? 1 : lp.kmid);
  b.nfft = lp.nfft >= 2 ? 2 : 1;
  b.store = g.store;
  b.tab = g.tables ? 1 : 0;
  b.fuse = next2 ? 2 + next2->nfft : (next ? next->nfft : 0);
  if (!g.tables || g.store != 0) return b;
  bool light = !next, central = d.central_half, any = false;
  for (const FrugalItem& fi : lp.items) {
    if (fi.active == 0.0) continue;
    any = true;
    light = light && 2.0 * (fi.pos_hi - fi.pos_lo) <= (double)d.n && 2.0 * (fi.spos_hi - fi.spos_lo) <= (double)d.n;
    central = central && 4.0 * fi.pos_lo >= (double)d.n && 4.0 * fi.pos_hi <= 3.0 * (double)d.n;
  }
  b.one_line = light ? 1 : 0;
  if (!build_exists(d, b)) b.one_line = 0;
  b.central = central && any ? 1 : 0;
  if (!build_exists(d, b)) b.central = 0;
  return b;
}

inline int pick_narrow(const PlanDims& d, const Launch& g, const FrugalBuild& b) {
  if (b.central != 1 || !d.narrow_windows) return 0;
  const double lo = 5.0 * (double)d.n, hi = 11.0 * (double)d.n;
  bool any = false;
  for (const FrugalItem& fi : g.lp[0]->items) {
    if (fi.active == 0.0) continue;
    any = true;
    if (!(16.0 * fi.pos_lo >= lo && 16.0 * fi.pos_hi <= hi)) return 0;
  }
  for (const FrugalItem& fo : g.last().items) {
    if (fo.active == 0.0) continue;
    if (!(16.0 * fo.spos_lo >= lo && 16.0 * fo.spos_hi <= hi)) return 0;
  }
  return any ? 1 : 0;
}

inline void finish_launch(const PlanDims& d, const PlanSwitches& sw, Launch& g, int store) {
  g.store = store;
  g.build = pick_build(d, g);
  g.narrow = pick_narrow(d, g, g.build);
  const bool store_psf = store == 1;
  const LoweredPass& lp = *g.lp[0];
  {
    double lo = (double)d.n, hi = 0.0;
    bool fill = false;
    for (const FrugalItem& fi : g.last().items) {
      if (fi.active == 0.0) continue;
      lo = fi.line_lo < lo ? fi.line_lo : lo;
      hi = fi.line_hi > hi ? fi.line_hi : hi;
      if (fi.line_fill != 0.0 && store_psf) {
        lo = fi.spos_lo < lo ? fi.spos_lo : lo;
        hi = fi.spos_hi > hi ? fi.spos_hi : hi;
      } else {
        fill = fill || fi.line_fill != 0.0;
      }
    }
    g.live_lo = g.live_hi = 0;
    if (sw.compact_grid && !fill && hi > lo && (lo > 0.0 || hi < (double)d.n)) {
      g.live_lo = (unsigned)lo;
      g.live_hi = (unsigned)hi;
    }
  }
  const double elem = d.precision == PAOS_F64 ? 16.0 : 8.0;
  g.tag = store_psf ? 8 : 0;
  g.bytes = 0.0;
  g.lines = 0.0;
  if (g.count > 1) g.tag |= g.count > 2 ? 32 : 16;
  for (int it = 0; it < d.batch; ++it) {
    const FrugalItem& fi = lp.items[it];
    const FrugalItem& fo = g.last().items[it];
    if (fi.active == 0.0) continue;
    if (fi.line_lo > 0.0 || fi.line_hi < (double)d.n) g.tag |= 1;
    if (fi.pos_lo > 0.0 || fi.pos_hi < (double)d.n) g.tag |= 2;
    if (!store_psf && (fo.spos_lo > 0.0 || fo.spos_hi < (double)d.n)) g.tag |= 4;
    g.bytes += (fi.line_hi - fi.line_lo) * ((fi.pos_hi - fi.pos_lo) * elem + (store_psf ? (double)d.n * 8.0 : (fo.spos_hi - fo.spos_lo) * elem));
    for (int k = 0; k < g.count; ++k) {
      const FrugalItem& fk = g.lp[k]->items[it];
      g.lines += (fi.line_hi - fi.line_lo) * ((fk.fft1_on != 0.0 ? 1.0 : 0.0) + (g.lp[k]->nfft >= 2 && fk.fft2_on != 0.0 ? 1.0 : 0.0));
    }
  }
}

#pragma GCC visibility pop
```

### paos_amd/csrc/pass_records.h

```cpp
#pragma once
#include "../../include/paos_hip.h"

#include <type_traits>
#include <vector>

namespace paos {

template <typename T>
struct cx;

enum : int { FP_ENABLE = 0, FP_SX = 1, FP_SY = 2, FP_COEF = 3, FP_SGN = 4, FP_STRIDE = 5 };
enum : int { FC_ENABLE = 0, FC_INVERSE = 1 };

constexpr double kMaxPhaseArg = 1.0e12;

constexpr int kFrugalMaxPre = 2, kFrugalMaxMid = 3;

struct FrugalPhase {
  double sx, sy, coef, sgn, m2, natural;
};
constexpr int kMaskW = 192;
struct MaskLine {
  int p0, p1, p2, p3;
  double lm;
  double pad;
};
struct FrugalSlot {
  double sign_on, scale;
  double mask_on, w_in, w_out;
  const MaskLine* lines;
  const double* vals;
  const cx<double>* table;
};
static_assert(sizeof(FrugalSlot) == 8 * sizeof(double), "record of 8-byte fields");
struct FrugalItem {
  double active;
  double fft1_on, fft1_inv, fft2_on, fft2_inv;
  double line_lo, line_hi, line_fill, pos_lo, pos_hi;
  double spos_lo, spos_hi;
  FrugalSlot pre;
  FrugalPhase pre_ph[kFrugalMaxPre];
  FrugalSlot mid;
  FrugalPhase mid_ph[kFrugalMaxMid];
};

struct PhaseSlotDesc { int item_base, mid, k, axis; };

}

#ifndef PAOS_LONG_ONE_LINE
#define PAOS_LONG_ONE_LINE 1
#endif
#ifndef PAOS_SINGLE_ONE_LINE
#define PAOS_SINGLE_ONE_LINE 1
#endif

struct FrugalBuild {
  int axis;
  int kpre;
  int kmid;
  int nfft;
  int store;
  int tab;
  int fuse;
  int one_line;
  int central;
};
constexpr int kBuildFields = 9;
static_assert(sizeof(FrugalBuild) == kBuildFields * sizeof(int), "a record of ints");
inline void build_to_ints(const FrugalBuild& b, int* rec) {
  const int v[kBuildFields] = {b.axis, b.kpre, b.kmid, b.nfft, b.store, b.tab, b.fuse, b.one_line, b.central};
  for (int k = 0; k < kBuildFields; ++k) rec[k] = v[k];
}
inline FrugalBuild build_from_ints(const int* rec) {
  return FrugalBuild{rec[0], rec[1], rec[2], rec[3], rec[4], rec[5], rec[6], rec[7], rec[8]};
}

template <typename T, int N>
constexpr bool frugal_built(const FrugalBuild& b) {
  constexpr bool kOneLineSizes = sizeof(T) == 8 && (N == 4096 || N == 2048) && PAOS_LONG_ONE_LINE != 0;
  if (b.axis < 0 || b.axis > 1 || b.kpre < 0 || b.kpre > paos::kFrugalMaxPre || b.kmid < 0 || b.kmid > paos::kFrugalMaxMid) return false;
  if (b.nfft < 1 || b.nfft > 2 || b.store < 0 || b.store > 2 || b.fuse < 0 || b.fuse > 4) return false;
  if ((b.tab | b.one_line | b.central) & ~1) return false;
  if (b.one_line && !(kOneLineSizes && PAOS_SINGLE_ONE_LINE != 0 && b.tab && !b.fuse && b.store == 0)) return false;
  if (b.central && !(kOneLineSizes && N == 4096 && b.tab && b.kpre == 1 && b.store == 0 && (b.fuse || b.one_line))) return false;
  if (b.fuse) return b.tab && b.kpre == 1 && b.kmid == 1 && b.nfft == 2;
  if (b.tab) return b.kpre <= 1 && b.kmid <= 1 && b.kpre + b.kmid > 0;
  return b.store == 0 || (b.kpre <= 1 && (b.store == 2 || b.kmid <= 1));
}

template <typename R, typename F>
R dispatch_family(int precision, int n, R none, F&& f) {
  if (precision == PAOS_F64) {
    if (n == 1024) return f(double{}, std::integral_constant<int, 1024>{});
    if (n == 2048) return f(double{}, std::integral_constant<int, 2048>{});
    if (n == 4096) return f(double{}, std::integral_constant<int, 4096>{});
  } else if (precision == PAOS_F32) {
    if (n == 2048) return f(float{}, std::integral_constant<int, 2048>{});
    if (n == 4096) return f(float{}, std::integral_constant<int, 4096>{});
  }
  return none;
}

struct LoweredPass {
  bool ok = false;
  std::vector<paos::FrugalItem> items;
  int kpre = 0, kmid = 0, nfft = 1, mask_block = -1, mask_slot = -1;
  std::vector<double> mask_shared;
  std::vector<int> mask_rep;
  int mask_set = -1;
  int mask_shapes = 3;
  int mask_lo = 0, mask_hi = 0;
  bool mask_render = false;
};
```

### paos_amd/csrc/passes.hip

```cpp
#include "frugal_launch.h"

#include <algorithm>
#include <cmath>
#include <cstdio>
#include <cstring>

#include "pass_program.h"
#include "phase_tables.h"

namespace {

int check_ops(paos_ctx* c, const paos_pw_op* ops, int count, int n_blocks) {
  if (count < 0 || count > PAOS_MAX_PW) return fail(c, PAOS_EINVAL, "too many pointwise operators in a pass");
  for (int o = 0; o < count; ++o) {
    if (ops[o].kind < PAOS_PW_SIGN || ops[o].kind > PAOS_PW_MASK) return fail(c, PAOS_EINVAL, "unknown pointwise operator");
    if (ops[o].block < 0 || ops[o].block >= n_blocks) return fail(c, PAOS_EINVAL, "operator block index out of range");
    if (ops[o].kind == PAOS_PW_MASK && ops[o].block + 1 >= n_blocks) return fail(c, PAOS_EINVAL, "an aperture operator needs two parameter blocks");
  }
  return PAOS_OK;
}

bool use_tables() {
  static const bool on = env_is("PAOS_PHASE_TABLES", '1');
  return on;
}

bool use_frugal() {
  static const bool on = !env_is("PAOS_NO_FRUGAL", '1');
  return on;
}

bool frugal_sizes(const paos_ctx* c) {
  return use_frugal() && c->n >= (c->precision == PAOS_F64 ? 1024 : 2048);
}

int ensure_mask_store(paos_ctx* c) {
  if (!c->mask_overflow) {
    HIPCHK(c, hipMalloc(&c->mask_overflow, sizeof(int)));
    HIPCHK(c, hipMemsetAsync(c->mask_overflow, 0, sizeof(int), c->stream));
  }
  if (!c->block_stats) {
    HIPCHK(c, hipMalloc(&c->block_stats, 3 * sizeof(unsigned long long)));
    HIPCHK(c, hipMemsetAsync(c->block_stats, 0, 3 * sizeof(unsigned long long), c->stream));
  }
  return PAOS_OK;
}

int assign_mask_set(paos_ctx* c, const paos_pass& p, LoweredPass& lp, const double* blocks) {
  std::vector<double> key;
  key.reserve((size_t)2 * c->batch * FP_STRIDE + c->batch + 3);
  key.push_back((double)p.axis);
  key.push_back((double)(mask_render_mode() + (mask_rect_blocks() ? 0 : 8)));
  const double* ap = blocks + (size_t)lp.mask_block * c->batch * FP_STRIDE;
  key.insert(key.end(), ap, ap + (size_t)2 * c->batch * FP_STRIDE);
  key.insert(key.end(), lp.mask_shared.begin(), lp.mask_shared.end());
  int hit = -1, victim = 0;
  for (int k = 0; k < paos_ctx::kMaskSets; ++k) {
    const paos_ctx::MaskSet& ms = c->mask_sets[k];
    if (!ms.key.empty() && ms.key.size() == key.size() && !std::memcmp(ms.key.data(), key.data(), key.size() * sizeof(double))) hit = k;
    if (ms.used < c->mask_sets[victim].used) victim = k;
  }
  const int k = hit >= 0 ? hit : victim;
  paos_ctx::MaskSet& ms = c->mask_sets[k];
  if (!ms.lines) {
    for (paos_ctx::MaskSet& m2 : c->mask_sets) {
      if (m2.lines) continue;
      HIPCHK(c, hipMalloc(&m2.lines, (size_t)c->batch * c->n * sizeof(MaskLine)));
      HIPCHK(c, hipMalloc(&m2.vals, (size_t)c->batch * c->n * 2 * kMaskW * sizeof(double)));
    }
  }
  ms.used = ++c->mask_clock;
  lp.mask_set = k;
  lp.mask_render = hit < 0;
  lp.mask_shapes = 0;
  for (int it = 0; it < c->batch; ++it) {
    const double* a1 = ap + (size_t)it * FP_STRIDE;
    const double* a2 = a1 + (size_t)c->batch * FP_STRIDE;
    if (a1[0] != 0.0 && (it >= (int)lp.mask_shared.size() || lp.mask_shared[it] == 0.0)) lp.mask_shapes |= (int)a2[3] == 0 ? 1 : 2;
  }
  if (hit < 0) { ms.key = std::move(key); ++c->mask_rendered; } else ++c->mask_hits;
  for (int it = 0; it < c->batch; ++it) {
    if (lp.mask_rep[it] < 0) continue;
    FrugalSlot& sl = lp.mask_slot == 0 ? lp.items[it].pre : lp.items[it].mid;
    sl.lines = ms.lines + (size_t)lp.mask_rep[it] * c->n;
    sl.vals = ms.vals + (size_t)lp.mask_rep[it] * c->n * 2 * kMaskW;
  }
  return PAOS_OK;
}

void forget_mask_sets(paos_ctx* c) {
  for (auto& ms : c->mask_sets) ms.key.clear();
}

MaskRender mask_job(paos_ctx* c, int axis, const LoweredPass& lp, const double* ap, const double* dshared) {
  const int line0 = lp.mask_lo, line_end = lp.mask_hi > lp.mask_lo ? lp.mask_hi : c->n;
  return MaskRender{ap, dshared, lp.mask_set, axis, line0, line_end, lp.mask_shapes};
}

PlanDims plan_dims(const paos_ctx* c) {
  return PlanDims{c->n, c->batch, c->br, c->precision, c->central_half ? 1 : 0, c->narrow_windows ? 1 : 0};
}
PlanSwitches plan_switches(const paos_ctx* c) {
  static const bool line_tables = !env_is("PAOS_LINE_TABLES", '0'), compact_grid = !env_is("PAOS_COMPACT_GRID", '0'),
                    env_prune = !env_is("PAOS_NO_PRUNE", '1'), batched_records = !env_is("PAOS_BATCHED_RECORDS", '0'),
                    psf_zero_reuse = !env_is("PAOS_PSF_ZERO_REUSE", '0');
  PlanSwitches sw;
  sw.line_tables = line_tables;
  sw.fuse_pairs = !env_is("PAOS_FUSE_PAIRS", '0');
  sw.compact_grid = compact_grid;
  sw.env_prune = env_prune;
  sw.stage_program = !env_is("PAOS_STAGE_PROGRAM", '0');
  sw.batched_records = batched_records;
  sw.psf_zero_reuse = psf_zero_reuse;
  sw.ctx_prune = c->prune;
  return sw;
}

struct StagedTables {
  const FrugalItem* items = nullptr;
  const PhaseSlotDesc* descs = nullptr;
  unsigned count = 0;
};
int stage_groups(paos_ctx* c, ArenaBatch& ab, std::vector<Launch>& groups, StagedTables* st) {
  std::vector<FrugalItem> blob;
  std::vector<PhaseSlotDesc> descs;
  int slots = 0;
  for (const Launch& g : groups)
    if (g.tables) slots += 2 * g.count;
  if (slots > c->ptab_slots) {
    if (c->ptab) { HIPCHK(c, hipStreamSynchronize(c->stream)); (void)hipFree(c->ptab); c->ptab = nullptr; c->ptab_slots = 0; }
    HIPCHK(c, hipMalloc(&c->ptab, (size_t)slots * c->batch * c->n * sizeof(cx<double>)));
    c->ptab_slots = slots;
  }
  int slot = 0;
  for (Launch& g : groups) {
    g.item_base = blob.size();
    for (int k = 0; k < g.count; ++k) {
      LoweredPass& l = *g.lp[k];
      const int counts[2] = {l.kpre, l.kmid};
      for (int s = 0; s < 2; ++s) {
        const bool has = g.tables && (counts[s] > 0 || g.count > 1);
        for (int it = 0; it < c->batch; ++it)
          (s == 0 ? l.items[it].pre : l.items[it].mid).table = has ? c->ptab + ((size_t)slot * c->batch + it) * c->n : nullptr;
        if (has) descs.push_back(PhaseSlotDesc{(int)blob.size(), s, counts[s], g.axis});
        if (g.tables) ++slot;
      }
      blob.insert(blob.end(), l.items.begin(), l.items.end());
    }
  }
  static_assert(sizeof(FrugalItem) % sizeof(double) == 0 && sizeof(PhaseSlotDesc) == 2 * sizeof(double), "records of doubles");
  const size_t item_doubles = blob.size() * sizeof(FrugalItem) / sizeof(double);
  std::vector<double> flat(item_doubles + 2 * descs.size());
  std::memcpy(flat.data(), blob.data(), item_doubles * sizeof(double));
  if (!descs.empty()) std::memcpy(flat.data() + item_doubles, descs.data(), descs.size() * sizeof(PhaseSlotDesc));
  const double* dflat = nullptr;
  int rc = ab.add(flat.data(), flat.size(), &dflat);
  if (rc) return rc;
  st->items = reinterpret_cast<const FrugalItem*>(dflat);
  st->descs = reinterpret_cast<const PhaseSlotDesc*>(dflat + item_doubles);
  st->count = (unsigned)descs.size();
  return PAOS_OK;
}
int launch_staged_tables(paos_ctx* c, const StagedTables& st) {
  if (st.count == 0) return PAOS_OK;
  const PhaseTableArgs ta{st.items, reinterpret_cast<const cx<double>*>(c->tw), st.descs, c->n, c->precision == PAOS_F64 ? 0 : 1};
  hipLaunchKernelGGL(phase_table_kernel<0>, dim3(c->n / 256, c->batch, st.count), dim3(256), 0, c->stream, ta);
  HIPCHK(c, hipGetLastError());
  return PAOS_OK;
}

int launch_lowered(paos_ctx* c, const Launch& g, const double* dblocks, const FrugalItem* staged) {
  for (int k = 0; k < g.count; ++k) {
    LoweredPass* l = g.lp[k];
    if (l->mask_block < 0 || !l->mask_render) continue;
    const double* ap = dblocks + (size_t)l->mask_block * c->batch * FP_STRIDE;
    const double* dshared = nullptr;
    int rcs = arena_push(c, l->mask_shared.data(), l->mask_shared.size(), &dshared);
    if (rcs) return rcs;
    const MaskRender job = mask_job(c, g.axis, *l, ap, dshared);
    if ((rcs = render_mask_records(c, &job, 1))) return rcs;
    l->mask_render = false;
  }
  if (!staged) {
    std::vector<Launch> one{g};
    ArenaBatch ab(c);
    StagedTables st;
    int rcg = stage_groups(c, ab, one, &st);
    if (rcg || (rcg = ab.commit()) || (rcg = launch_staged_tables(c, st))) return rcg;
    staged = st.items + one[0].item_base;
  }
  FrugalArgs a{c->field, c->tw, staged, c->pitch, c->item_stride, nullptr, nullptr, nullptr};
  if (g.store == 1) { a.psf = c->psf; a.psf_partial = c->psf_partial; }
  if (g.store == 2) a.pow_partial = c->pow_partial;
  a.dyn_scale = c->dyn_scale;
  a.live_lo = g.live_lo; a.live_hi = g.live_hi; a.wg0 = 0;
  c->prof_next_tag = g.tag;
  c->prof_next_bytes = g.bytes;
  c->prof_next_lines = g.lines;
  const FrugalBuild& b = g.build;
  {
    int rec[kBuildFields];
    build_to_ints(b, rec);
    c->pass_builds.insert(c->pass_builds.end(), rec, rec + kBuildFields);
  }
  static const bool dump = env_is("PAOS_DUMP_PASSES", '1');
  if (dump) {
    std::fprintf(stderr, "build axis %d kpre %d kmid %d nfft %d store %d tab %d fuse %d one_line %d central %d n %d %s\n", b.axis, b.kpre, b.kmid,
                 b.nfft, b.store, b.tab, b.fuse, b.one_line, b.central, c->n, c->precision == PAOS_F64 ? "fp64" : "fp32");
    for (int k = 0; k < g.count; ++k) {
      const LoweredPass* l = g.lp[k];
      if (l->items.empty()) continue;
      const FrugalItem& f = l->items[0];
      std::fprintf(stderr, "%spass axis %d kpre %d kmid %d nfft %d | pre: sign %g scale %g mask %g | fft1 on %g inv %g | mid: sign %g scale %g mask %g | "
                   "fft2 on %g inv %g | lines [%g, %g) fill %g loads [%g, %g) stores [%g, %g)\n", k == 0 ? "" : "+", g.axis, l->kpre, l->kmid, l->nfft,
                   f.pre.sign_on, f.pre.scale, f.pre.mask_on, f.fft1_on, f.fft1_inv, f.mid.sign_on, f.mid.scale, f.mid.mask_on, f.fft2_on, f.fft2_inv,
                   f.line_lo, f.line_hi, f.line_fill, f.pos_lo, f.pos_hi, f.spos_lo, f.spos_hi);
    }
  }
  return dispatch_family(c->precision, c->n, (int)PAOS_EUNSUPPORTED,
                         [&](auto t, auto n) { return frugal_family<decltype(t), decltype(n)::value>(c, b, a, g.narrow != 0); });
}

int launch_one_pass(paos_ctx* c, const paos_pass& p, const double* dblocks, int n_blocks,
                    const int* table_of_op ) {
  int rc;
  for (int l = 0; l < 3; ++l)
    if ((rc = check_ops(c, op_list(p, l).ops, op_list(p, l).count, n_blocks))) return rc;
  if (p.fft1 >= n_blocks || p.fft2 >= n_blocks) return fail(c, PAOS_EINVAL, "transform control block out of range");
  int nmask = 0;
  for (int l = 0; l < 3; ++l) {
    const OpList ol = op_list(p, l);
    for (int o = 0; o < ol.count; ++o)
      if (ol.ops[o].kind == PAOS_PW_MASK) {
        if (++nmask > 1) return fail(c, PAOS_EINVAL, "one aperture operator per pass");
        int rcm = render_mask_weights(c, dblocks + (size_t)ol.ops[o].block * c->batch * FP_STRIDE);
        if (rcm) return rcm;
      }
  }
  PassArgs a{};
  a.field = c->field; a.tw = c->tw; a.blocks = dblocks; a.tables = c->tables; a.mask = c->mask; a.batch = c->batch;
  a.fft1 = p.fft1; a.fft2 = p.fft2; a.n_pre = p.n_pre; a.n_mid = p.n_mid; a.n_post = p.n_post;
  static_assert(sizeof(PwOp) == sizeof(paos_pw_op), "ABI op layout");
  std::memcpy(a.pre, p.pre, sizeof(a.pre));
  std::memcpy(a.mid, p.mid, sizeof(a.mid));
  std::memcpy(a.post, p.post, sizeof(a.post));
  PwOp* lists[3] = {a.pre, a.mid, a.post};
  int feat = 0;
  for (int l = 0; l < 3; ++l)
    for (int o = 0; o < PAOS_MAX_PW; ++o) {
      lists[l][o].flags &= (1 << kTableShift) - 1;
      const int t = table_of_op[l * PAOS_MAX_PW + o];
      if (t >= 0) { lists[l][o].flags |= (t + 1) << kTableShift; feat = 3; }
      if (o < op_list(p, l).count && lists[l][o].kind == PWK_MASK) feat = 3;
    }
  a.pitch = c->pitch; a.item_stride = c->item_stride;
  if (p.axis == 0 || p.axis == 1) return generic_pass(c, p.axis, a, feat);
  if (p.axis != -1) return fail(c, PAOS_EINVAL, "pass axis must be 0, 1 or -1");
  if (p.fft1 >= 0 || p.fft2 >= 0 || p.n_mid || p.n_post)
    return fail(c, PAOS_EINVAL, "a transform-free pass carries its operators in the pre list");
  return pointwise_pass(c, a);
}

struct ProgramRun {
  paos_ctx* c;
  const paos_pass* passes;
  int n_passes;
  const double* blocks;
  int n_blocks;
  PlanDims d;
  PlanSwitches sw;
  ArenaBatch ab;
  const double* dblocks = nullptr;
  std::vector<LoweredPass> low;
  bool all_frugal = false, pruned = false;
  int store = 0;
  int power_groups = 0;
  std::vector<MaskRender> renderings;
  std::vector<Launch> launches;
  std::vector<int> launch_of;
  StagedTables staged;
  ProgramRun(paos_ctx* c_, const paos_pass* passes_, int n_passes_, const double* blocks_, int n_blocks_)
      : c(c_), passes(passes_), n_passes(n_passes_), blocks(blocks_), n_blocks(n_blocks_), d(plan_dims(c_)), sw(plan_switches(c_)), ab(c_) {}
};

int validate_program(paos_ctx* c, const paos_pass* passes, int n_passes, const double* blocks, int n_blocks, const int* final_ticket) {
  if (c) c->pass_builds.clear();
  if (!c || !passes || !blocks || n_passes < 0 || n_blocks < 1) return fail(c, PAOS_EINVAL, "bad pass program");
  c->norm2_of_field = false;
  if (int rcr = final_ticket ? power_ring_full(c) : PAOS_OK) return rcr;
  switch (check_phase_args(plan_dims(c), passes, n_passes, blocks, n_blocks)) {
    case PHASE_BLOCK_OUT_OF_RANGE: return fail(c, PAOS_EINVAL, "operator block index out of range");
    case PHASE_TOO_LARGE: return fail(c, PAOS_EUNSUPPORTED, "quadratic phase exceeds 1e12 rad at the grid corner (or is not finite)");
    default: return PAOS_OK;
  }
}

int open_batch(ProgramRun& r) {
  paos_ctx* c = r.c;
  const size_t per_pass = (((size_t)c->batch * sizeof(FrugalItem) / sizeof(double) + 15) & ~size_t(15)) +
                          (((size_t)c->batch + 15) & ~size_t(15)) + 16;
  int rc = r.ab.begin((size_t)r.n_blocks * c->batch * FP_STRIDE + 16 + (size_t)r.n_passes * per_pass + 2 * arena_rounded((size_t)2 * c->batch));
  if (rc) return rc;
  return r.ab.add(r.blocks, (size_t)r.n_blocks * c->batch * FP_STRIDE, &r.dblocks);
}

int lower_and_assign_sets(ProgramRun& r) {
  paos_ctx* c = r.c;
  r.low.resize(r.n_passes);
  r.all_frugal = !use_tables() && frugal_sizes(c) && r.n_passes > 0;
  if (use_tables() || !frugal_sizes(c)) return PAOS_OK;
  int rc = ensure_mask_store(c);
  if (rc) return rc;
  for (int q = 0; q < r.n_passes; ++q) {
    LoweredPass& lp = r.low[q];
    lp.ok = lower_frugal(r.d, r.passes[q], r.blocks, lp);
    if (lp.ok && lp.mask_block >= 0 && (rc = assign_mask_set(c, r.passes[q], lp, r.blocks))) return rc;
    r.all_frugal = r.all_frugal && lp.ok;
  }
  return PAOS_OK;
}

int settle_stop(ProgramRun& r) {
  paos_ctx* c = r.c;
  if (!c->dyn_pending) return PAOS_OK;
  bool ride = r.n_passes > 0 && r.low[0].ok;
  if (ride)
    for (const FrugalItem& fi : r.low[0].items) ride = ride && fi.active != 0.0;
  if (ride) ++c->deferred_rode;
  return ride ? PAOS_OK : settle_scale(c);
}

void plan_lines(ProgramRun& r, const double* entry_rows, bool entry_stale, const double* entry_cols) {
  paos_ctx* c = r.c;
  r.pruned = r.all_frugal && r.sw.env_prune && r.sw.ctx_prune;
  if (r.pruned) plan_pruning(r.d, r.passes, r.n_passes, r.blocks, r.low, entry_rows, entry_stale, entry_cols);
  for (LoweredPass& lp : r.low) {
    if (!lp.ok || lp.mask_block < 0) continue;
    record_window(r.d, lp);
    paos_ctx::MaskSet& ms = c->mask_sets[lp.mask_set];
    if (!lp.mask_render && !(ms.line_lo <= lp.mask_lo && ms.line_hi >= lp.mask_hi)) {
      lp.mask_render = true;
      --c->mask_hits; ++c->mask_rendered;
    }
    if (lp.mask_render) { ms.line_lo = lp.mask_lo; ms.line_hi = lp.mask_hi; }
  }
}

int prepare_store(ProgramRun& r, int final_mode) {
  paos_ctx* c = r.c;
  r.store = last_pass_store(r.low, final_mode);
  if (final_mode == 2 && r.store == 2) {
    r.power_groups = c->n / frugal_tile_lines(c, r.passes[r.n_passes - 1].axis);
    if (c->pow_nparts < c->n / 2) {
      if (c->pow_partial) (void)hipFree(c->pow_partial);
      c->pow_partial = nullptr; c->pow_nparts = 0;
      HIPCHK(c, hipMalloc(&c->pow_partial, (size_t)c->batch * (c->n / 2) * sizeof(double)));
      c->pow_nparts = c->n / 2;
    }
    HIPCHK(c, hipMemsetAsync(c->pow_partial, 0, (size_t)c->batch * r.power_groups * sizeof(double), c->stream));
  }
  if (final_mode != 1) return PAOS_OK;
  if (!c->psf) HIPCHK(c, hipMalloc(&c->psf, (size_t)c->batch * c->item_stride * sizeof(double)));
  c->otf_valid = c->ee_valid = false;
  if (r.store != 1) return PAOS_OK;
  const int axis = r.passes[r.n_passes - 1].axis, groups = c->n / frugal_tile_lines(c, axis);
  if (c->psf_nparts < groups) {
    if (c->psf_partial) (void)hipFree(c->psf_partial);
    c->psf_partial = nullptr; c->psf_nparts = 0;
    c->psf_zero_axis = -1;
    HIPCHK(c, hipMalloc(&c->psf_partial, (size_t)c->batch * groups * sizeof(double)));
    c->psf_nparts = groups;
  }
  psf_zero_fill(r.d, r.sw, axis, r.low[r.n_passes - 1].items, c->psf_zero_axis, c->psf_zero_lo, c->psf_zero_hi);
  c->psf_zero_axis = -1;
  return PAOS_OK;
}

int batch_renderings(ProgramRun& r) {
  for (int q : batched_renderings(r.sw, r.all_frugal, r.low)) {
    LoweredPass& lp = r.low[q];
    const double* dshared = nullptr;
    int rc = r.ab.add(lp.mask_shared.data(), lp.mask_shared.size(), &dshared);
    if (rc) return rc;
    r.renderings.push_back(mask_job(r.c, r.passes[q].axis, lp, r.dblocks + (size_t)lp.mask_block * r.c->batch * FP_STRIDE, dshared));
    lp.mask_render = false;
  }
  return PAOS_OK;
}

int plan_and_stage_launches(ProgramRun& r) {
  r.launches = form_launches(r.d, r.sw, r.passes, r.n_passes, r.low, r.all_frugal && r.pruned, r.launch_of);
  for (Launch& g : r.launches) {
    if (!g.lp[0]->ok) continue;
    decide_tables(r.d, r.sw, g);
    finish_launch(r.d, r.sw, g, g.q + g.count == r.n_passes ? r.store : 0);
  }
  if (!stage_whole_program(r.d, r.sw, r.all_frugal, r.n_passes)) return PAOS_OK;
  return stage_groups(r.c, r.ab, r.launches, &r.staged);
}

int launch_chunks(ProgramRun& r) {
  paos_ctx* c = r.c;
  int rc;
  int i = 0;
  while (i < r.n_passes) {
    TableArgs ta{};
    ta.blocks = r.dblocks; ta.tables = c->tables; ta.batch = c->batch; ta.n = c->n; ta.count = 0;
    std::vector<int> assign;
    int j = i;
    for (; j < r.n_passes; ++j) {
      const paos_pass& p = r.passes[j];
      int need = 0;
      for (int l = 0; l < 3; ++l)
        for (int o = 0; o < op_list(p, l).count && o < PAOS_MAX_PW; ++o) need += is_phase(op_list(p, l).ops[o]);
      if (use_tables() && ta.count + need > kMaxTables) {
        if (j == i) return fail(c, PAOS_EINVAL, "one pass needs more phase tables than the store holds");
        break;
      }
      const size_t base = assign.size();
      assign.resize(base + 3 * PAOS_MAX_PW, -1);
      if (!use_tables()) continue;
      for (int l = 0; l < 3; ++l)
        for (int o = 0; o < op_list(p, l).count && o < PAOS_MAX_PW; ++o) {
          const paos_pw_op& op = op_list(p, l).ops[o];
          if (!is_phase(op)) continue;
          if (op.block < 0 || op.block >= r.n_blocks) return fail(c, PAOS_EINVAL, "operator block index out of range");
          ta.jobs[ta.count] = {op.block, op.kind, op.flags & PAOS_PWF_MUL2PI};
          assign[base + l * PAOS_MAX_PW + o] = ta.count++;
        }
    }
    if (ta.count > 0) {
      if (!c->tables) {
        HIPCHK(c, hipMalloc(&c->tables, (size_t)kMaxTables * c->batch * 2 * c->n * sizeof(cx<double>)));
        ta.tables = c->tables;
      }
      const dim3 grid((2 * c->n + 255) / 256, c->batch, ta.count);
      hipLaunchKernelGGL(phase_table_kernel, grid, dim3(256), 0, c->stream, ta);
      HIPCHK(c, hipGetLastError());
    }
    for (int q = i; q < j; ++q) {
      if (!r.low[q].ok) {
        if ((rc = launch_one_pass(c, r.passes[q], r.dblocks, r.n_blocks, &assign[(size_t)(q - i) * 3 * PAOS_MAX_PW]))) return rc;
        continue;
      }
      const Launch& g = r.launches[r.launch_of[q]];
      const int last = q + g.count - 1;
      if (last >= j) return fail(c, PAOS_EINVAL, "a fused group crosses a table chunk");
      if ((rc = launch_lowered(c, g, r.dblocks, r.staged.items ? r.staged.items + g.item_base : nullptr))) return rc;
      q = last;
      if (c->dyn_pending) {
        if ((rc = dyn_scale_reset(c))) return rc;
      }
    }
    i = j;
  }
  return PAOS_OK;
}

int hand_out_ticket(ProgramRun& r, int final_mode, int* final_ticket) {
  paos_ctx* c = r.c;
  if (final_mode == 2) {
    const int rcp = r.store == 2 ? take_power_ticket(c, c->pow_partial, r.power_groups, nullptr, final_ticket) : paos_norm2_enqueue(c, final_ticket);
    if (rcp == PAOS_OK) c->norm2_of_field = true;
    return rcp;
  }
  if (r.store != 1) return psf_keep_power_impl(c, final_ticket);
  c->psf_zero_axis = r.passes[r.n_passes - 1].axis;
  return take_power_ticket(c, c->psf_partial, c->n / frugal_tile_lines(c, r.passes[r.n_passes - 1].axis), nullptr, final_ticket);
}

int run_passes_impl(paos_ctx* c, const paos_pass* passes, int n_passes, const double* blocks, int n_blocks,
                    const double* entry_rows, bool entry_stale, int* final_ticket, int final_mode, const double* entry_cols) {
  int rc = validate_program(c, passes, n_passes, blocks, n_blocks, final_ticket);
  if (rc) return rc;
  final_mode = final_ticket ? (final_mode == 2 ? 2 : 1) : 0;
  ProgramRun r(c, passes, n_passes, blocks, n_blocks);
  if ((rc = open_batch(r)) || (rc = lower_and_assign_sets(r)) || (rc = settle_stop(r))) return rc;
  plan_lines(r, entry_rows, entry_stale, entry_cols);
  if (entry_stale && entry_rows && entry_zero_first(r.d, r.pruned, r.low, entry_rows, entry_cols)) {
    if ((rc = entry_cols ? zero_outside_box(c, entry_rows, entry_cols) : zero_outside_rows(c, entry_rows))) return rc;
  }
  if ((rc = prepare_store(r, final_mode)) || (rc = batch_renderings(r)) || (rc = plan_and_stage_launches(r))) return rc;
  if ((rc = r.ab.commit())) return rc;
  for (size_t at = 0; at < r.renderings.size(); at += kMaskRenders)
    if ((rc = render_mask_records(c, r.renderings.data() + at, (int)std::min<size_t>(kMaskRenders, r.renderings.size() - at)))) return rc;
  if ((rc = launch_staged_tables(c, r.staged)) || (rc = launch_chunks(r))) return rc;
  return final_mode ? hand_out_ticket(r, final_mode, final_ticket) : PAOS_OK;
}

}

int run_passes(paos_ctx* c, const paos_pass* passes, int n_passes, const double* blocks, int n_blocks, const double* entry_rows,
               bool entry_stale, int* final_ticket, int final_mode, const double* entry_cols) {
  const int rc = arena_settled(c, run_passes_impl(c, passes, n_passes, blocks, n_blocks, entry_rows, entry_stale, final_ticket, final_mode, entry_cols));
  if (rc != PAOS_OK && c) forget_mask_sets(c);
  return rc;
}

int mask_render_mode() {
  if (env_is("PAOS_MASK_SCAN", '1')) return 0;
  if (env_is("PAOS_MASK_PAIRS", '0')) return 1;
  if (env_is("PAOS_MASK_PAIRS", '1')) return 2;
  return env_is("PAOS_MASK_BLOCKS", '0') ? 3 : 4;
}
bool mask_rect_blocks() {
  return !env_is("PAOS_MASK_RECT_BLOCKS", '0');
}

namespace {

struct Program {
  std::vector<paos_pass> passes;
  std::vector<double> blocks;
  int batch;
  explicit Program(int b) : batch(b) {}
  int add_block(const double* src, double v1, double v2, double v3, double v4, bool copy) {
    const int id = (int)(blocks.size() / ((size_t)batch * FP_STRIDE));
    for (int i = 0; i < batch; ++i) {
      const double* s = src + (size_t)i * FP_STRIDE;
      if (copy) blocks.insert(blocks.end(), s, s + FP_STRIDE);
      else blocks.insert(blocks.end(), {s[FP_ENABLE], v1, v2, v3, v4});
    }
    return id;
  }
  paos_pass& add_pass(int axis, int fft1, int fft2) {
    paos_pass p{};
// ... 113 lines not shown
```

Before: 2454 wavefronts/s.

## Window PSF stores to the live position range in fused final passes

Measured after the change: 2451 wavefronts/s. About the same (-0.1%).

```diff
diff --git a/include/paos_hip.h b/include/paos_hip.h
--- a/include/paos_hip.h
+++ b/include/paos_hip.h
@@ -124,6 +124,7 @@
 int paos_record_set_stats(paos_ctx* ctx, unsigned long long* found, unsigned long long* rendered);
 int paos_central_half_stats(paos_ctx* ctx, unsigned long long* central, unsigned long long* plain);
 int paos_narrow_window_stats(paos_ctx* ctx, unsigned long long* narrow, unsigned long long* other);
+int paos_psf_store_window_stats(paos_ctx* ctx, unsigned long long* window, unsigned long long* full);
 int paos_record_block_stats(paos_ctx* ctx, unsigned long long* out);
 int paos_frugal_built(int precision, int n, const int* record);
 int paos_pass_builds(paos_ctx* ctx, int* records, int capacity, int* count);
diff --git a/paos_amd/_lib.py b/paos_amd/_lib.py
--- a/paos_amd/_lib.py
+++ b/paos_amd/_lib.py
@@ -107,6 +107,7 @@
     "paos_record_set_stats": (ctypes.c_int, [_c_ctx, ctypes.POINTER(ctypes.c_ulonglong), ctypes.POINTER(ctypes.c_ulonglong)]),
     "paos_central_half_stats": (ctypes.c_int, [_c_ctx, ctypes.POINTER(ctypes.c_ulonglong), ctypes.POINTER(ctypes.c_ulonglong)]),
     "paos_narrow_window_stats": (ctypes.c_int, [_c_ctx, ctypes.POINTER(ctypes.c_ulonglong), ctypes.POINTER(ctypes.c_ulonglong)]),
+    "paos_psf_store_window_stats": (ctypes.c_int, [_c_ctx, ctypes.POINTER(ctypes.c_ulonglong), ctypes.POINTER(ctypes.c_ulonglong)]),
     "paos_record_block_stats": (ctypes.c_int, [_c_ctx, ctypes.POINTER(ctypes.c_ulonglong)]),
     "paos_frugal_built": (ctypes.c_int, [ctypes.c_int, ctypes.c_int, ctypes.POINTER(ctypes.c_int)]),
     "paos_pass_builds": (ctypes.c_int, [_c_ctx, ctypes.POINTER(ctypes.c_int), ctypes.c_int, ctypes.POINTER(ctypes.c_int)]),
diff --git a/paos_amd/csrc/context.hip b/paos_amd/csrc/context.hip
--- a/paos_amd/csrc/context.hip
+++ b/paos_amd/csrc/context.hip
@@ -304,6 +304,8 @@
   if (env_is("PAOS_CENTRAL_HALF", '1')) c->central_half = true;
   if (env_is("PAOS_NARROW_WINDOWS", '0')) c->narrow_windows = false;
   if (env_is("PAOS_NARROW_WINDOWS", '1')) c->narrow_windows = true;
+  if (env_is("PAOS_PSF_STORE_WINDOW", '0')) c->psf_store_window = false;
+  if (env_is("PAOS_PSF_STORE_WINDOW", '1')) c->psf_store_window = true;
   if ((e = hipMalloc(&c->dyn_scale, (size_t)batch * sizeof(double))) != hipSuccess) return bail(e, "hipMalloc(dyn_scale)");
   {
     std::vector<double> ones((size_t)batch, 1.0);
@@ -520,6 +522,13 @@
   return PAOS_OK;
 }
 
+int paos_psf_store_window_stats(paos_ctx* c, unsigned long long* window, unsigned long long* full) {
+  if (!c || !window || !full) return fail(c, PAOS_EINVAL, "bad store-window request");
+  *window = c->psf_window_launches;
+  *full = c->psf_full_launches;
+  return PAOS_OK;
+}
+
 int paos_record_block_stats(paos_ctx* c, unsigned long long* out) {
   if (!c || !out) return fail(c, PAOS_EINVAL, "bad record-block request");
   out[0] = out[1] = out[2] = 0ull;
diff --git a/paos_amd/csrc/focus_otf.hip b/paos_amd/csrc/focus_otf.hip
--- a/paos_amd/csrc/focus_otf.hip
+++ b/paos_amd/csrc/focus_otf.hip
@@ -199,7 +199,7 @@
   a.psf = c->psf; a.spec = c->otf_spec; a.tw = c->tw; a.tabs = dtabs;
   a.scale = 1.0 / ((double)c->n * (double)c->n);
   a.pitch = c->pitch; a.item_stride = c->item_stride;
-  c->psf_zero_axis = -1;
+  c->forget_psf_zeros();
   c->ee_valid = false;
   for (int axis = 1; axis >= 0; --axis) {
     rc = blur_pass(c, axis, a);
diff --git a/paos_amd/csrc/frugal_launch.h b/paos_amd/csrc/frugal_launch.h
--- a/paos_amd/csrc/frugal_launch.h
+++ b/paos_amd/csrc/frugal_launch.h
@@ -52,7 +52,12 @@
   auto kern = frugal_pass_kernel<T, N, C::E, G::LINES, G::TILES, AXIS, C::BR, C::BC, G::SPLIT, KPRE, KMID, NFFT, STORE, TAB, LONG, G::OCC, CH>;
   if constexpr (CH == 1) {
     if (narrow) kern = frugal_pass_kernel<T, N, C::E, G::LINES, G::TILES, AXIS, C::BR, C::BC, G::SPLIT, KPRE, KMID, NFFT, STORE, TAB, LONG, G::OCC, 2>;
+  } else if constexpr (psf_window_built<T, N>(FrugalBuild{AXIS, KPRE, KMID, NFFT, STORE, TAB, LONG, ONE, CH})) {
+    if (narrow) kern = frugal_pass_kernel<T, N, C::E, G::LINES, G::TILES, AXIS, C::BR, C::BC, G::SPLIT, KPRE, KMID, NFFT, 3, TAB, LONG, G::OCC, CH>;
+    ++(narrow ? c->psf_window_launches : c->psf_full_launches);
+    narrow = false;
   } else {
+    if (STORE == 1) ++c->psf_full_launches;
     narrow = false;
   }
   ++(CH != 0 ? c->central_launches : c->plain_launches);
diff --git a/paos_amd/csrc/frugal_pass.h b/paos_amd/csrc/frugal_pass.h
--- a/paos_amd/csrc/frugal_pass.h
+++ b/paos_amd/csrc/frugal_pass.h
@@ -508,6 +508,10 @@
   static_assert(LONG == 0 || (TAB != 0 && NFFT == 2 && KPRE == 1 && KMID == 1), "LONG builds: see above");
   static_assert(CH == 0 || (sizeof(T) == 8 && N == 4096 && E == 16 && TAB != 0 && KPRE == 1 && NFFT <= 2), "CH builds: see above");
   static_assert(CH >= 0 && CH <= 2 && (CH != 2 || STORE == 0), "CH = 2: field-storing builds");
+  static_assert(STORE != 3 || (sizeof(T) == 8 && N == 4096 && E == 16 && LONG != 0), "STORE = 3: PSF-storing fused builds of 4096^2 complex128");
+  constexpr bool kPsf = STORE == 1 || STORE == 3;
+  constexpr bool kPsfWindow = STORE == 3;
+  constexpr bool kNarrowStore = CH == 2 || kPsfWindow;
   FrugalArgs a;
   a.items = k_items; a.field = k_field; a.pitch = k_pitch; a.item_stride = k_item_stride; a.wg0 = k_wg0;
   a.tw = k_tw; a.psf = k_psf; a.psf_partial = k_psf_partial; a.pow_partial = k_pow_partial; a.dyn_scale = k_dyn_scale; a.live_lo = a.live_hi = 0;
@@ -528,6 +532,8 @@
   const double h_mask_on = it.mid.mask_on;
   const MaskLine* const h_lines = it.mid.lines;
   const double h_dyn = *((const __attribute__((address_space(4))) double*)a.dyn_scale + item);
+  const FrugalPhase& win_ph = it_last.mid_ph[kFrugalMaxMid - 1];
+  [[maybe_unused]] const PsfStoreWindow h_win = kPsfWindow ? PsfStoreWindow{win_ph.sx, win_ph.sy, win_ph.coef, win_ph.sgn} : PsfStoreWindow{};
   if constexpr (frugal_record_mode<LINES, TILES, KPRE>() != 0)
     asm volatile("" ::"s"(h_active), "s"(h_line_lo), "s"(h_line_hi), "s"(h_line_fill), "s"(h_pos_lo), "s"(h_pos_hi), "s"(h_spos_lo),
                  "s"(h_spos_hi), "s"(h_mask_on), "s"(h_lines), "s"(h_dyn));
@@ -545,12 +551,21 @@
   const int l0 = TILES == 1 ? (AXIS == 0 ? m.row0 : m.col0) : (int)wg * (TILES * LINES);
   {
     if (l0 + TILES * LINES <= (int)h_line_lo || l0 >= (int)h_line_hi) {
-      if constexpr (STORE == 1) {
+      if constexpr (kPsf) {
         if (h_line_fill == 0.0) return;
         if (l0 + TILES * LINES <= (int)h_spos_lo || l0 >= (int)h_spos_hi) return;
         double* ps = a.psf + (size_t)item * a.item_stride;
-#pragma unroll
-        for (int k = 0; k < E; ++k) ps[m.base + (unsigned)k * m.stride] = 0.0;
+        if constexpr (kPsfWindow) {
+          const int zlo = (int)h_win.zero_lo, zhi = (int)h_win.zero_hi;
+#pragma unroll
+          for (int k = ch_first<E, 2>(); k < ch_end<E, 2>(); ++k) {
+            const int pos = m.t + k * (N / E);
+            if (pos >= zlo && pos < zhi) ps[m.base + (unsigned)k * m.stride] = 0.0;
+          }
+        } else {
+#pragma unroll
+          for (int k = 0; k < E; ++k) ps[m.base + (unsigned)k * m.stride] = 0.0;
+        }
         if (threadIdx.x == 0) a.psf_partial[(size_t)item * (N / LINES / TILES) + wg] = 0.0;
         return;
       }
@@ -702,16 +717,16 @@
     const bool ran4 = (kTwo) && (ix).fft2_on != 0.0;                                                                                 \
     const bool inv3 = ran3 && (ix).fft1_inv != 0.0;                                                                                  \
     frugal_slot<T, N, E, 1, decltype(m), 0, false, 0, TAB>(v, (ix).pre, (ix).pre_ph, m, circle, false, inv3, m.t, lds, false);       \
-    if constexpr (CH == 2 && !(kTwo)) pin_tile<E>(v);                                                                                \
+    if constexpr (kNarrowStore && !(kTwo)) pin_tile<E>(v);                                                                            \
     if (ran3) {                                                                                                                      \
       if (busy) __syncthreads();                                                                                                     \
       frugal_fft<T, N, E, SPLIT, false>(v, lds, m.t, tw, circle, (ix).fft1_inv, w1_last);                                            \
       busy = true;                                                                                                                   \
     }                                                                                                                                \
                 \
-    frugal_slot<T, N, E, 1, decltype(m), 0, false, 0, TAB, (CH == 2 && !(kTwo)) ? 2 : 0>(                                            \
+    frugal_slot<T, N, E, 1, decltype(m), 0, false, 0, TAB, (kNarrowStore && !(kTwo)) ? 2 : 0>(                                        \
         v, (ix).mid, (ix).mid_ph, m, circle, inv3, ran4 && (ix).fft2_inv != 0.0, m.t, lds, ran3);                                    \
-    if constexpr (CH == 2 && (kTwo)) pin_tile<E>(v);                                                                                 \
+    if constexpr (kNarrowStore && (kTwo)) pin_tile<E>(v);                                                                             \
     if constexpr (kTwo) {                                                                                                            \
       if (ran4) {                                                                                                                    \
         if (busy) __syncthreads();                                                                                                   \
@@ -730,15 +745,27 @@
   PAOS_STAMP(5);
   [[maybe_unused]] double* const scratch = reinterpret_cast<double*>(
       smem + frugal_lds_bytes<T, N, LINES, TILES, SPLIT, KPRE, KMID, E, 0, OCC>() - kStoreScratch - (kRecMode == 1 ? (size_t)TILES * LINES * sizeof(MaskLine) : 0));
-  if constexpr (STORE == 1) {
+  if constexpr (kPsf) {
     double* ps = a.psf + (size_t)item * a.item_stride;
     double acc = 0.0;
-#pragma unroll
-    for (int k = 0; k < E; ++k) {
-      const double x = (double)v[k].x, y = (double)v[k].y;
-      const double w = __dadd_rn(__dmul_rn(x, x), __dmul_rn(y, y));
-      ps[m.base + (unsigned)k * m.stride] = w;
-      acc += w;
+    if constexpr (kPsfWindow) {
+      const int wlo = (int)h_win.store_lo, whi = (int)h_win.store_hi;
+#pragma unroll
+      for (int k = ch_first<E, 2>(); k < ch_end<E, 2>(); ++k) {
+        const double x = (double)v[k].x, y = (double)v[k].y;
+        const double w = __dadd_rn(__dmul_rn(x, x), __dmul_rn(y, y));
+        const int pos = m.t + k * (N / E);
+        if (pos >= wlo && pos < whi) ps[m.base + (unsigned)k * m.stride] = w;
+        acc += w;
+      }
+    } else {
+#pragma unroll
+      for (int k = 0; k < E; ++k) {
+        const double x = (double)v[k].x, y = (double)v[k].y;
+        const double w = __dadd_rn(__dmul_rn(x, x), __dmul_rn(y, y));
+        ps[m.base + (unsigned)k * m.stride] = w;
+        acc += w;
+      }
     }
     tile_power_out<TILES * LINES * N / E>(acc, scratch, a.psf_partial + (size_t)item * (N / LINES / TILES) + wg);
     return;
diff --git a/paos_amd/csrc/host.h b/paos_amd/csrc/host.h
--- a/paos_amd/csrc/host.h
+++ b/paos_amd/csrc/host.h
@@ -85,7 +85,10 @@
   unsigned long long deferred_rode = 0, deferred_settled = 0;
   bool norm2_of_field = false;
   int psf_zero_axis = -1;
-  std::vector<double> psf_zero_lo, psf_zero_hi;
+  std::vector<double> psf_zero_lo, psf_zero_hi, psf_zero_wlo, psf_zero_whi;
+  bool psf_store_window = false;
+  unsigned long long psf_window_launches = 0, psf_full_launches = 0;
+  void forget_psf_zeros() { psf_zero_axis = -1; psf_zero_wlo.clear(); psf_zero_whi.clear(); }
   bool det_set = false;
   int det_nx = 0, det_ny = 0;
   double det_geom[4] = {};
diff --git a/paos_amd/csrc/paos_hip.hip b/paos_amd/csrc/paos_hip.hip
--- a/paos_amd/csrc/paos_hip.hip
+++ b/paos_amd/csrc/paos_hip.hip
@@ -420,7 +420,7 @@
   if (c) (void)hipSetDevice(c->device);
   if (!c) return fail(c, PAOS_EINVAL, "null context");
   if (!c->psf) HIPCHK(c, hipMalloc(&c->psf, (size_t)c->batch * c->item_stride * sizeof(double)));
-  c->psf_zero_axis = -1;
+  c->forget_psf_zeros();
   c->otf_valid = c->ee_valid = false;
   const dim3 grid(pw_blocks(c), c->batch), block(kPwThreads);
   dispatch_layout(c, [&](auto t, auto br) {
@@ -576,7 +576,7 @@
 int psf_keep_power_impl(paos_ctx* c, int* ticket) {
   if (int rc = power_ring_full(c)) return rc;
   if (!c->psf) HIPCHK(c, hipMalloc(&c->psf, (size_t)c->batch * c->item_stride * sizeof(double)));
-  c->psf_zero_axis = -1;
+  c->forget_psf_zeros();
   c->otf_valid = c->ee_valid = false;
   const dim3 grid(c->nparts, c->batch), block(kPwThreads);
   dispatch_layout(c, [&](auto t, auto br) {
diff --git a/paos_amd/csrc/pass_program.h b/paos_amd/csrc/pass_program.h
--- a/paos_amd/csrc/pass_program.h
+++ b/paos_amd/csrc/pass_program.h
@@ -17,6 +17,7 @@
   int precision;
   int central_half;
   int narrow_windows = 1;
+  int psf_store_window = 1;
 };
 struct PlanSwitches {
   bool line_tables = true;
@@ -188,8 +189,10 @@
 struct LineRange { int lo, hi; };
 
 inline void plan_pruning(const PlanDims& d, const paos_pass* passes, int n_passes, const double* blocks,
-                         std::vector<LoweredPass>& low, const double* entry_rows, bool entry_stale, const double* entry_cols) {
+                         std::vector<LoweredPass>& low, const double* entry_rows, bool entry_stale, const double* entry_cols,
+                         std::vector<LineRange>* last_window = nullptr) {
   const int n = d.n, br = d.br;
+  if (last_window) last_window->assign(d.batch, LineRange{0, n});
   auto meet = [br](LineRange a, LineRange b) {
     LineRange r{a.lo > b.lo ? a.lo : b.lo, a.hi < b.hi ? a.hi : b.hi};
     if (r.lo >= r.hi) { r.lo = a.lo; r.hi = a.lo + br < a.hi ? a.lo + br : a.hi; }
@@ -244,6 +247,7 @@
       if (low[q].nfft >= 2 && fi.fft2_on != 0.0) pos = {0, n};
       P = pos;
     }
+    if (last_window) (*last_window)[it] = box[1 - passes[act.back()].axis];
     LineRange want[2] = {{0, n}, {0, n}};
     for (size_t k = act.size(); k-- > 0;) {
       const int q = act[k], ax = passes[q].axis;
@@ -317,6 +321,24 @@
     last[it].spos_lo = covered ? 0.0 : old_lo;
     last[it].spos_hi = covered ? (double)d.n : old_hi;
     zero_lo[it] = last[it].line_lo; zero_hi[it] = last[it].line_hi;
+    set_psf_store_window(last[it], PsfStoreWindow{0.0, (double)d.n, 0.0, (double)d.n});
+  }
+}
+
+inline bool psf_zero_known(const PlanDims& d, const PlanSwitches& sw, int axis, int known_axis, const std::vector<double>& zero_lo) {
+  return sw.psf_zero_reuse && known_axis == axis && (int)zero_lo.size() == d.batch;
+}
+inline void psf_window_fill(const PlanDims& d, bool known, const std::vector<LineRange>& window, std::vector<FrugalItem>& last,
+                            std::vector<double>& win_lo, std::vector<double>& win_hi) {
+  known = known && (int)win_lo.size() == d.batch && (int)win_hi.size() == d.batch;
+  win_lo.resize(d.batch); win_hi.resize(d.batch);
+  for (int it = 0; it < d.batch; ++it) {
+    const double n = (double)d.n;
+    const double old_lo = known ? win_lo[it] : 0.0, old_hi = known ? win_hi[it] : n;
+    const bool windowed = d.psf_store_window != 0 && it < (int)window.size() && window[it].lo < window[it].hi;
+    const double lo = windowed ? (double)window[it].lo : 0.0, hi = windowed ? (double)window[it].hi : n;
+    set_psf_store_window(last[it], PsfStoreWindow{lo < old_lo ? lo : old_lo, hi > old_hi ? hi : old_hi, old_lo, old_hi});
+    win_lo[it] = lo; win_hi[it] = hi;
   }
 }
 
@@ -368,6 +390,7 @@
   int store = 0;
   FrugalBuild build{};
   int narrow = 0;
+  int psf_window = 0;
   unsigned live_lo = 0, live_hi = 0;
   int tag = 0;
   double bytes = 0.0, lines = 0.0;
@@ -456,10 +479,26 @@
   return any ? 1 : 0;
 }
 
+inline int pick_psf_window(const PlanDims& d, const Launch& g, const FrugalBuild& b) {
+  if (b.store != 1 || !d.psf_store_window) return 0;
+  if (!dispatch_family(d.precision, d.n, false, [&](auto t, auto n) { return psf_window_built<decltype(t), decltype(n)::value>(b); })) return 0;
+  const double lo = 5.0 * (double)d.n, hi = 11.0 * (double)d.n;
+  bool any = false;
+  for (const FrugalItem& fo : g.last().items) {
+    if (fo.active == 0.0) continue;
+    any = true;
+    const PsfStoreWindow w = psf_store_window(fo);
+    if (!(16.0 * w.store_lo >= lo && 16.0 * w.store_hi <= hi && w.store_lo < w.store_hi)) return 0;
+    if (fo.line_fill != 0.0 && !(16.0 * w.zero_lo >= lo && 16.0 * w.zero_hi <= hi)) return 0;
+  }
+  return any ? 1 : 0;
+}
+
 inline void finish_launch(const PlanDims& d, const PlanSwitches& sw, Launch& g, int store) {
   g.store = store;
   g.build = pick_build(d, g);
   g.narrow = pick_narrow(d, g, g.build);
+  g.psf_window = store == 1 ? pick_psf_window(d, g, g.build) : 0;
   const bool store_psf = store == 1;
   const LoweredPass& lp = *g.lp[0];
   {
@@ -494,7 +533,9 @@
     if (fi.line_lo > 0.0 || fi.line_hi < (double)d.n) g.tag |= 1;
     if (fi.pos_lo > 0.0 || fi.pos_hi < (double)d.n) g.tag |= 2;
     if (!store_psf && (fo.spos_lo > 0.0 || fo.spos_hi < (double)d.n)) g.tag |= 4;
-    g.bytes += (fi.line_hi - fi.line_lo) * ((fi.pos_hi - fi.pos_lo) * elem + (store_psf ? (double)d.n * 8.0 : (fo.spos_hi - fo.spos_lo) * elem));
+    const PsfStoreWindow w = store_psf ? psf_store_window(fo) : PsfStoreWindow{};
+    const double psf_positions = g.psf_window ? w.store_hi - w.store_lo : (double)d.n;
+    g.bytes += (fi.line_hi - fi.line_lo) * ((fi.pos_hi - fi.pos_lo) * elem + (store_psf ? psf_positions * 8.0 : (fo.spos_hi - fo.spos_lo) * elem));
     for (int k = 0; k < g.count; ++k) {
       const FrugalItem& fk = g.lp[k]->items[it];
       g.lines += (fi.line_hi - fi.line_lo) * ((fk.fft1_on != 0.0 ? 1.0 : 0.0) + (g.lp[k]->nfft >= 2 && fk.fft2_on != 0.0 ? 1.0 : 0.0));
diff --git a/paos_amd/csrc/pass_records.h b/paos_amd/csrc/pass_records.h
--- a/paos_amd/csrc/pass_records.h
+++ b/paos_amd/csrc/pass_records.h
@@ -44,6 +44,17 @@
   FrugalPhase mid_ph[kFrugalMaxMid];
 };
 
+struct PsfStoreWindow { double store_lo, store_hi, zero_lo, zero_hi; };
+static_assert(kFrugalMaxMid >= 2 && sizeof(PsfStoreWindow) <= sizeof(FrugalPhase), "rides in the unused last phase record");
+inline void set_psf_store_window(FrugalItem& fi, const PsfStoreWindow& w) {
+  FrugalPhase& ph = fi.mid_ph[kFrugalMaxMid - 1];
+  ph.sx = w.store_lo; ph.sy = w.store_hi; ph.coef = w.zero_lo; ph.sgn = w.zero_hi;
+}
+inline PsfStoreWindow psf_store_window(const FrugalItem& fi) {
+  const FrugalPhase& ph = fi.mid_ph[kFrugalMaxMid - 1];
+  return PsfStoreWindow{ph.sx, ph.sy, ph.coef, ph.sgn};
+}
+
 struct PhaseSlotDesc { int item_base, mid, k, axis; };
 
 }
@@ -89,6 +100,11 @@
   return b.store == 0 || (b.kpre <= 1 && (b.store == 2 || b.kmid <= 1));
 }
 
+template <typename T, int N>
+constexpr bool psf_window_built(const FrugalBuild& b) {
+  return sizeof(T) == 8 && N == 4096 && b.store == 1 && b.tab != 0 && b.fuse != 0 && frugal_built<T, N>(b);
+}
+
 template <typename R, typename F>
 R dispatch_family(int precision, int n, R none, F&& f) {
   if (precision == PAOS_F64) {
diff --git a/paos_amd/csrc/passes.hip b/paos_amd/csrc/passes.hip
--- a/paos_amd/csrc/passes.hip
+++ b/paos_amd/csrc/passes.hip
@@ -98,7 +98,7 @@
 }
 
 PlanDims plan_dims(const paos_ctx* c) {
-  return PlanDims{c->n, c->batch, c->br, c->precision, c->central_half ? 1 : 0, c->narrow_windows ? 1 : 0};
+  return PlanDims{c->n, c->batch, c->br, c->precision, c->central_half ? 1 : 0, c->narrow_windows ? 1 : 0, c->psf_store_window ? 1 : 0};
 }
 PlanSwitches plan_switches(const paos_ctx* c) {
   static const bool line_tables = !env_is("PAOS_LINE_TABLES", '0'), compact_grid = !env_is("PAOS_COMPACT_GRID", '0'),
@@ -218,7 +218,7 @@
     }
   }
   return dispatch_family(c->precision, c->n, (int)PAOS_EUNSUPPORTED,
-                         [&](auto t, auto n) { return frugal_family<decltype(t), decltype(n)::value>(c, b, a, g.narrow != 0); });
+                         [&](auto t, auto n) { return frugal_family<decltype(t), decltype(n)::value>(c, b, a, g.narrow != 0 || g.psf_window != 0); });
 }
 
 int launch_one_pass(paos_ctx* c, const paos_pass& p, const double* dblocks, int n_blocks,
@@ -276,6 +276,7 @@
   int store = 0;
   int power_groups = 0;
   std::vector<MaskRender> renderings;
+  std::vector<LineRange> last_window;
   std::vector<Launch> launches;
   std::vector<int> launch_of;
   StagedTables staged;
@@ -333,7 +334,7 @@
 void plan_lines(ProgramRun& r, const double* entry_rows, bool entry_stale, const double* entry_cols) {
   paos_ctx* c = r.c;
   r.pruned = r.all_frugal && r.sw.env_prune && r.sw.ctx_prune;
-  if (r.pruned) plan_pruning(r.d, r.passes, r.n_passes, r.blocks, r.low, entry_rows, entry_stale, entry_cols);
+  if (r.pruned) plan_pruning(r.d, r.passes, r.n_passes, r.blocks, r.low, entry_rows, entry_stale, entry_cols, &r.last_window);
   for (LoweredPass& lp : r.low) {
     if (!lp.ok || lp.mask_block < 0) continue;
     record_window(r.d, lp);
@@ -367,11 +368,13 @@
   if (c->psf_nparts < groups) {
     if (c->psf_partial) (void)hipFree(c->psf_partial);
     c->psf_partial = nullptr; c->psf_nparts = 0;
-    c->psf_zero_axis = -1;
+    c->forget_psf_zeros();
     HIPCHK(c, hipMalloc(&c->psf_partial, (size_t)c->batch * groups * sizeof(double)));
     c->psf_nparts = groups;
   }
+  const bool known = psf_zero_known(r.d, r.sw, axis, c->psf_zero_axis, c->psf_zero_lo);
   psf_zero_fill(r.d, r.sw, axis, r.low[r.n_passes - 1].items, c->psf_zero_axis, c->psf_zero_lo, c->psf_zero_hi);
+  psf_window_fill(r.d, known, r.last_window, r.low[r.n_passes - 1].items, c->psf_zero_wlo, c->psf_zero_whi);
   c->psf_zero_axis = -1;
   return PAOS_OK;
 }
```
